# lijingzhu1/SKGHOI

Hardware: AMD Instinct MI355X
Metric: images/sec through interaction head (20x20 pairs) (higher is better)
Workload: dtype f32; 1 GPU; HICO-DET-shaped synthetic cached detections: 20 humans x 20 objects per image (G=800 grid rows, P=780 pairs, K=117 verbs), eval forward of InteractionHead from cached AdaMixer-R50 box features [40,256,7,7]/image; precision=fp32, batch_per_gpu=256, parallelism=dp1 (independent image shards, no data-path collective)

## Files before the change

include/skghoi.h:

```cpp
#ifndef SKGHOI_H
#define SKGHOI_H
#include <stdint.h>
#ifdef __cplusplus
extern "C" {
#endif

#define SKG_ABI_VERSION 19
#define SKG_E_ARG   (-1)
#define SKG_E_ALIGN (-2)
#define SKG_E_LIMIT (-3)
#define SKG_E_UNSUPPORTED (-4)
#define SKG_E_COMM  (-5)

#define SKG_MAX_DET_PER_IMAGE 1024
#define SKG_MAX_NODES         160
#define SKG_SPATIAL_LD        48
#define SKG_TRANSH_DIM        50
#define SKG_TRANSH_ENT        80

int         skg_abi_version(void);
const char* skg_build_info(void);

typedef struct {
    int32_t image;
// ... 175 lines not shown
                          const skg_image_meta* meta, int n_active, const int32_t* hum_img, const int32_t* node_img,
                          int sum_h, int sum_n, const float* T_os, const float* T_so, int64_t ldt, int cols,
                          void* U, void* V, int64_t ldu, float* adj_out, int out_dtype, void* stream);

int skg_layernorm_f32(const float* x, int64_t ldx, const float* gamma, const float* beta, int rows, int cols,
                      float eps, float* out, int64_t ldo, void* stream);
int skg_layernorm2_f32(const float* x0, int64_t ldx0, const float* gamma0, const float* beta0, int rows0, float* out0,
                       int64_t ldo0, const float* x1, int64_t ldx1, const float* gamma1, const float* beta1, int rows1,
                       float* out1, int64_t ldo1, int cols, float eps, void* stream);
int skg_layernorm2_x(const float* x0, int64_t ldx0, const float* gamma0, const float* beta0, int rows0, void* out0,
                     int64_t ldo0, const float* x1, int64_t ldx1, const float* gamma1, const float* beta1, int rows1,
                     void* out1, int64_t ldo1, int cols, float eps, int out_dtype, void* stream);

int skg_postprocess_f32(const float* logits, int64_t ld_logits, int K, const float* boxes, const float* scores,
                        const int64_t* labels, const skg_image_meta* meta, int n_active, const int64_t* x_keep,
                        const int64_t* y_keep, const int32_t* verb_off, const int32_t* verb_list, int num_obj_classes,
                        float prior_pow, int64_t L_total, const int32_t* L_total_dev, int max_pairs_per_image,
                        int64_t* out_index, int64_t* out_pred, float* out_scores, float* out_prior, float* out_weights,
                        int64_t* out_object, float* out_boxes_h, float* out_boxes_o, void* stream);

int skg_transh_draw_f32(void* torch_cpu_rng_state, int64_t state_bytes, int n_images, int K, int need_relations,
                        int fused_affine, float* ent, float* rel, float* nrm);

int skg_transh_draw_train_f32(void* torch_cpu_rng_state, int64_t state_bytes, int n_images, int K, int fused_affine,
                              const int64_t* n_neg, const int64_t* n_take, float* ent, float* rel, float* nrm,
                              int64_t* perm_out);

int skg_transh_scores_f32(const float* ent, const float* rel, const float* nrm, int K, int human_idx,
                          const skg_image_meta* meta, int n_active, float* scores, void* stream);

int skg_associate_f32(const float* boxes, const skg_image_meta* meta, int n_active, const int64_t* x_keep,
                      const int64_t* y_keep, const float* gt_h, const float* gt_o, const int64_t* gt_label,
                      const int32_t* gt_off, int K, float thresh, float* labels, int32_t* npos, void* stream);

typedef struct {
    const float* A; int64_t a_sm, a_sk;
    const float* B; int64_t b_sn, b_sk;
    int32_t b_kshift, b_nshift; int64_t b_kstride, b_nstride;
    float*  C; int64_t ldc; int32_t c_nshift, accumulate; int64_t c_nstride;
    int32_t M, N, K, relu;
    const float* bias;
    const float* mask; int64_t ldmask;
    float*  a_rowsum;
    int32_t split_k, reserved;
    float*  split_ws;
    const uint16_t* A16;
    const uint16_t* B16;
    uint16_t* C16;
    uint32_t* split_ctr;
    int64_t a16_ld, b16_ld;
} skg_gemmx_desc;
#define SKG_GEMMX_GROUP_MAX 8
int64_t skg_gemmx_ws_floats(const skg_gemmx_desc* desc_host);
int skg_gemmx_f32(const skg_gemmx_desc* descs_host, int n, void* stream);
int skg_gemmx_bf16(const skg_gemmx_desc* descs_host, int n, void* stream);
void skg_gemmx_path_counts(int64_t* out3_host, int reset);

int skg_graph_aggregate_train_f32(const float* dot_partial, int n_partial, int64_t partial_ld, float adj_bias,
                                  const skg_image_meta* meta, int n_active, const int32_t* hum_img,
                                  const int32_t* node_img, int sum_h, int sum_n, const float* T_os, const float* T_so,
                                  int64_t ldt, int cols, float* U, float* V, int64_t ldu, float* adj_out,
                                  float* alpha_out, float* beta_out, void* stream);
int skg_rowdot_f32(const float* X, int64_t ld, const float* w, int rows, int cols, float* out, void* stream);
int skg_add_layernorm_f32(const float* a, int64_t lda, const float* b, int64_t ldb, const float* gamma,
                          const float* beta, int rows, float eps, float* xsum, float* y, float* stats, void* stream);
int skg_layernorm_bwd_f32(const float* dy, int64_t lddy, const float* x, const float* stats, const float* gamma,
                          int rows, float* dx, const float* relu_src, float* dx_masked, float* dgamma, float* dbeta,
                          void* stream);
int skg_mul_bwd_f32(float* g, int64_t ldg, const float* F, const int32_t* f_idx, int64_t ldf, const float* P,
                    const int32_t* p_idx, int64_t ldp, const float* Q, const int32_t* q_idx, int64_t ldq,
                    const float* mbias, int rows, float* dF, int64_t lddf, int accumulate, void* stream);
int skg_segment_sum_f32(const float* src, int64_t ld, const skg_image_meta* meta, int n_active, const int32_t* hum_img,
                        const int32_t* node_img, int sum_h, int sum_n, int mode, float* outH, float* outN,
                        int accumulate, void* stream);
int skg_aggregate_bwd_f32(const float* dU, const float* dV, const float* Tos, const float* Tso, const float* alpha,
                          const float* beta, const int32_t* grid_h, const int32_t* grid_o, int sum_g,
                          const skg_image_meta* meta, const int32_t* hum_img, const int32_t* node_img, int sum_h,
                          int sum_n, float* dTos, float* dTso, float* da, float* db, float* dadj_h, float* dadj_n,
                          void* stream);
int skg_adjacency_bwd_f32(const float* dadj_h, const float* dadj_n, const float* w, const float* Wt, int rows,
                          float* dadj, float* dWt, void* stream);
int skg_entity_rows_bwd_f32(const float* dX, int64_t ldx, const int32_t* hum_of, const int32_t* node_of, int sum_h,
                            int n_enc, const float* enc, float* d_enc, void* stream);
#define SKG_LOSS_CHUNKS 64
int skg_hoi_loss_f32(const float* logits, int64_t ldl, int K, const skg_image_meta* meta, int n_active,
                     int64_t cells_total, const int64_t* index, const int64_t* pred, const float* scores,
                     const float* labels, float* cell_labels, float* unary, float* partial, float* dlogits,
                     void* stream);

int skg_count_positives_f32(const float* labels, int K, const float* det_scores, const int64_t* det_labels,
                            const skg_image_meta* meta, int n_active, const int64_t* x_keep, const int64_t* y_keep,
                            const int32_t* verb_off, const int32_t* verb_list, int num_obj_classes, float prior_pow,
                            float* counts, void* stream);

int skg_loss_finish_f32(const float* partial, int rows, const float* mpart, int n_img, int64_t m_pos, float margin,
                        float grad_share, const float* norm_in, float* losses, float* scale, float* counts_out,
                        void* stream);
int skg_scale_dlogits_f32(const float* dl, int64_t ld, int rows, int K, const float* scale, const float* g0,
                          const float* g1, float* out, void* stream);

int64_t skg_transh_sample_ws_ints(int n_active, int max_pos_per_image);
int skg_transh_sample_f32(const float* labels, const float* scores, int K, const skg_image_meta* meta, int n_active,
                          const int32_t* pos_off, int max_pos_per_image, const int64_t* perm, float margin, int32_t* ws,
                          int32_t* pos_cells, float* pos_scores, float* neg_scores, float* partial, void* stream);

int skg_eval_associate_f32(const float* boxes_h, const float* boxes_o, const int64_t* object, const int32_t* pair_off,
                           const int64_t* index, const int64_t* pred, const float* scores, const int32_t* cell_off,
                           int n_images, const int32_t* lut, int n_obj, int n_verb, const float* gt_h, const float* gt_o,
                           const int64_t* gt_hoi, const int32_t* gt_off, float min_iou, int32_t* hoi_out, float* labels,
                           int32_t* status, void* stream);
int skg_eval_ap11_f64(const float* labels_sorted, const int64_t* class_off, const int64_t* num_gt, int n_classes,
                      const double* thresholds11, double* ap, void* stream);

#define SKG_CHECKSUM_PARTIALS 1024
typedef struct {
    const void* ptr;
    uint32_t    count;
    uint32_t    first;
} skg_param_chunk;
int skg_param_checksum(const skg_param_chunk* chunks, int n_chunks, uint64_t* out, void* stream);

#define SKG_ADAMW_CHUNK 16384
typedef struct {
    float* p; const float* g; float* m; float* v;
    uint32_t count, reserved;
} skg_adamw_chunk;
int skg_adamw_f32(const skg_adamw_chunk* chunks, int n_chunks, double lr, double beta1, double beta2, double eps,
                  double weight_decay, double bias1, double bias2, float* steps, int n_steps, void* stream);

#define SKG_GRADNORM_PARTIALS 1024
typedef struct {
    float   total_norm;
    float   coef;
    int32_t applied;
    int32_t reserved;
    int64_t steps_applied;
    int64_t steps_skipped;
    int64_t steps_clipped;
    float   max_total_norm;
    int32_t reserved2;
    int64_t pending_skips[2];
} skg_step_status;
int skg_grad_sumsq_f32(const skg_adamw_chunk* chunks, int n_chunks, double* partials, void* stream);
int skg_adamw_guarded_f32(const skg_adamw_chunk* chunks, int n_chunks, double lr, double beta1, double beta2, double eps,
                          double weight_decay, double bias1, double bias2, int64_t t_host, double max_norm,
                          int skip_nonfinite, const double* partials, int n_partials, float* steps, int n_steps,
                          skg_step_status* status, void* stream);
int skg_sizeof_step_status(void);

enum {
    SKG_SEG_W1_0 = 0, SKG_SEG_W1_1, SKG_SEG_W1_2, SKG_SEG_W1_3, SKG_SEG_B1_0, SKG_SEG_B1_1, SKG_SEG_B1_2, SKG_SEG_B1_3,
    SKG_SEG_W3_0, SKG_SEG_W3_1, SKG_SEG_W3_2, SKG_SEG_W3_3, SKG_SEG_B3, SKG_SEG_W2, SKG_SEG_B2, SKG_SEG_CLS_W, SKG_SEG_CLS_B,
    SKG_SEG_NH_W, SKG_SEG_NH_B, SKG_SEG_NO_W, SKG_SEG_NO_B, SKG_SEG_ADJ_W, SKG_SEG_ADJ_B, SKG_SEG_SP0_W, SKG_SEG_SP0_B,
    SKG_SEG_SP2_W, SKG_SEG_SP2_B, SKG_SEG_SP4_W, SKG_SEG_SP4_B, SKG_SEG_FH_W, SKG_SEG_FH_B, SKG_SEG_FT_W, SKG_SEG_FT_B,
    SKG_SEG_BH3_W, SKG_SEG_BH3_B, SKG_SEG_BH1_W, SKG_SEG_BH1_B, SKG_TRAIN_SEGS
};
#define SKG_TRAIN_BWD_STAGES 12
typedef struct skg_train_timer skg_train_timer;
typedef struct {
    int32_t NA, Mg, Mp, Mh, Mn, A, K, Bf, Cf;
    int32_t x0_k;
    int32_t bf16;
    int32_t ld_logits;
    const float* params; float* grads;
    int64_t seg_off[SKG_TRAIN_SEGS];
    const float* x0;
// ... 80 lines not shown
```

skghoi_amd/_capi.py:

```python
import ctypes as C
import os

_HERE = os.path.dirname(os.path.abspath(__file__))
LIB_PATH = os.environ.get("SKG_LIB") or os.path.join(_HERE, "csrc", "libskghoi_hip.so")

EPI_BIAS, EPI_BIAS_RELU, EPI_MUL_RELU, EPI_RELU_DOT, EPI_BIAS_RES_RELU = range(5)
DTYPE_F32, DTYPE_F16, DTYPE_BF16 = range(3)
MAX_DET_PER_IMAGE = 1024
MAX_NODES = 160
SPATIAL_LD = 48
TRANSH_DIM = 50
TRANSH_ENT = 80
ABI_VERSION = 19
GEMM_GROUP_MAX = 4
CHECKSUM_PARTIALS = 1024
LOSS_CHUNKS = 64

_vp = C.c_void_p
_i32 = C.c_int32
_i64 = C.c_int64
_f32 = C.c_float


class GemmDesc(C.Structure):
    _fields_ = [("A", _vp), ("lda", _i64), ("W", _vp), ("ldw", _i64), ("bias", _vp), ("C", _vp), ("ldc", _i64),
                ("M", _i32), ("N", _i32), ("K", _i32), ("epilogue", _i32), ("a_rows", _vp), ("out_rows", _vp),
                ("P", _vp), ("p_idx", _vp), ("ldp", _i64), ("Q", _vp), ("q_idx", _vp), ("ldq", _i64),
                ("mbias", _vp), ("C_raw", _vp), ("ldc_raw", _i64), ("dot_w", _vp), ("dot_partial", _vp),
                ("res", _vp), ("ldres", _i64), ("split_k", _i32), ("w_scale", _f32), ("split_ws", _vp), ("w_split", _vp),
                ("a_exp", _vp)]


class GemmB16Io(C.Structure):
    _fields_ = [("w16", _vp), ("a16", _vp), ("c16", _vp), ("ldc16", _i64)]


class GemmXDesc(C.Structure):
    _fields_ = [("A", _vp), ("a_sm", _i64), ("a_sk", _i64), ("B", _vp), ("b_sn", _i64), ("b_sk", _i64),
                ("b_kshift", _i32), ("b_nshift", _i32), ("b_kstride", _i64), ("b_nstride", _i64),
                ("C", _vp), ("ldc", _i64), ("c_nshift", _i32), ("accumulate", _i32), ("c_nstride", _i64),
                ("M", _i32), ("N", _i32), ("K", _i32), ("relu", _i32), ("bias", _vp), ("mask", _vp), ("ldmask", _i64),
                ("a_rowsum", _vp), ("split_k", _i32), ("reserved", _i32), ("split_ws", _vp),
                ("A16", _vp), ("B16", _vp), ("C16", _vp), ("split_ctr", _vp),
                ("a16_ld", _i64), ("b16_ld", _i64)]


GEMMX_GROUP_MAX = 8
ADAMW_CHUNK = 16384


class GemmBf16Desc(C.Structure):
    _fields_ = [("A", _vp), ("lda", _i64), ("W", _vp), ("ldw", _i64), ("bias", _vp), ("C", _vp), ("ldc", _i64),
                ("M", _i32), ("N", _i32), ("K", _i32), ("relu", _i32), ("out_bf16", _i32), ("split_k", _i32),
                ("split_ws", _vp)]


TRAIN_SEGS = ("W1_0", "W1_1", "W1_2", "W1_3", "b1_0", "b1_1", "b1_2", "b1_3", "W3_0", "W3_1", "W3_2", "W3_3", "b3", "W2",
              "b2", "clsW", "clsb", "nh_w", "nh_b", "no_w", "no_b", "adj_w", "adj_b", "sp0_w", "sp0_b", "sp2_w", "sp2_b",
              "sp4_w", "sp4_b", "fh_w", "fh_b", "ft_w", "ft_b", "bh3_w", "bh3_b", "bh1_w", "bh1_b")
TRAIN_BWD_STAGES = 12
COMM_ID_BYTES = 128


class Exchange(C.Structure):
    _fields_ = [("comm", C.c_void_p), ("arena", C.c_void_p), ("n_chunks", C.c_int32),
                ("stage", C.c_int32 * TRAIN_BWD_STAGES), ("end", C.c_int64 * TRAIN_BWD_STAGES),
                ("adamw", C.c_void_p), ("adamw_first", C.c_int32 * (TRAIN_BWD_STAGES + 1)), ("adamw_n_steps", C.c_int32),
                ("adamw_steps", C.c_void_p)] + [(n, C.c_double) for n in ("lr", "beta1", "beta2", "eps", "weight_decay",
                                                                          "bias1", "bias2")]


GRADNORM_PARTIALS = 1024


class StepStatus(C.Structure):
    _fields_ = [("total_norm", _f32), ("coef", _f32), ("applied", _i32), ("reserved", _i32),
                ("steps_applied", _i64), ("steps_skipped", _i64), ("steps_clipped", _i64),
                ("max_total_norm", _f32), ("reserved2", _i32), ("pending_skips", _i64 * 2)]


class Tuning(C.Structure):
    _fields_ = [(n, _i32) for n in ("small_mode", "small_tiles", "route_tiles", "khalves_blocks")]


class TrainPlan(C.Structure):
    _fields_ = [(n, _i32) for n in ("NA", "Mg", "Mp", "Mh", "Mn", "A", "K", "Bf", "Cf", "x0_k", "bf16", "ld_logits")] + \
               [("params", _vp), ("grads", _vp), ("seg_off", _i64 * len(TRAIN_SEGS)),
                ("x0", _vp), ("gfeat", _vp), ("sp48", _vp), ("ent", _vp), ("meta", _vp)] + \
               [(n, _vp) for n in ("enc_row_hn", "img_hn", "ent_row_hn", "hum_img", "node_img", "grid_h", "grid_o",
                                   "grid_pair", "grid_img", "pair_grid", "pair_h", "pair_o", "pair_img", "hum_of",
                                   "node_of")] + \
               [("ws", _vp), ("ws_floats", _i64), ("pair_features", _vp), ("logits", _vp), ("dlogits", _vp),
                ("dx0", _vp), ("dgfeat", _vp), ("timer", _vp), ("ws16", _vp), ("params16", _vp), ("pf16", _vp),
                ("params_floats", _i64), ("counters", _vp), ("n_counters", _i64), ("split_target", _i32), ("split_max", _i32),
                ("two_branch", _i32), ("reserved2", _i32)]


LAYOUT_SLICES = ("meta", "node_img", "hum_img", "node_enc_row", "hum_enc_row", "node_ent_row", "hum_ent_row", "enc_row_hn",
                 "img_hn", "ent_row_hn", "hum_of", "node_of", "pair_img", "gt_off", "active")


class LayoutInfo(C.Structure):
    _fields_ = [(n, _i32) for n in ("B", "n_visit", "n_active", "index_error")] + \
               [(n, _i64) for n in ("sum_all", "sum_n", "sum_h", "sum_g", "sum_p", "sum_l", "ints")] + \
               [("off", _i32 * len(LAYOUT_SLICES)), ("len", _i32 * len(LAYOUT_SLICES))]


META_FIELDS = [("image", "i4"), ("n_h", "i4"), ("n", "i4"), ("box_off", "i4"), ("enc_off", "i4"), ("node_off", "i4"),
               ("hum_off", "i4"), ("grid_off", "i4"), ("pair_off", "i4"), ("out_off", "i4"), ("img_h", "f4"),
               ("img_w", "f4")]

PROTOTYPES = {
    "skg_abi_version": (C.c_int, []),
    "skg_build_info": (C.c_char_p, []),
    "skg_preprocess_f32": (C.c_int, [_vp, _vp, _vp, _vp, C.c_int, C.c_int, _f32, _f32, C.c_int, C.c_int, _vp, C.c_int,
                                     _f32, _vp, _vp, _vp]),
    "skg_pack_detections_f32": (C.c_int, [_vp, _vp, _vp, _vp, _vp, C.c_int, _vp, C.c_int, _vp, _vp, _vp, _vp]),
    "skg_pairs_spatial_f32": (C.c_int, [_vp, _vp, C.c_int, _vp, _vp, _vp, _vp, _vp, _vp, _vp, _vp, _vp, _vp, C.c_int,
                                        _vp]),
    "skg_pairs_spatial_padded_f32": (C.c_int, [_vp, _vp, C.c_int, _vp, _vp, _vp, _vp, _vp, _vp, _vp, _vp, _vp, _vp,
                                               C.c_int, C.c_int, C.c_int, _vp]),
    "skg_roi_align_f32": (C.c_int, [_vp, _vp, _vp, _vp, C.c_int, C.c_int, C.c_int, C.c_int, _f32, C.c_int, _vp, _vp,
                                    C.c_int, C.c_int, C.c_int, _vp, _vp]),
    "skg_roi_align_bwd_f32": (C.c_int, [_vp, _vp, _vp, _vp, C.c_int, C.c_int, C.c_int, C.c_int, _f32, C.c_int, _vp, _vp,
                                    C.c_int, C.c_int, C.c_int, _vp, _vp]),
    "skg_roi_align_x": (C.c_int, [_vp, C.c_int, _vp, _vp, _vp, C.c_int, C.c_int, C.c_int, C.c_int, _f32, C.c_int, _vp,
                                  _vp, C.c_int, C.c_int, C.c_int, _vp, C.c_int, _vp]),
    "skg_roi_align_nhwc_x": (C.c_int, [_vp, C.c_int, _vp, _vp, _vp, C.c_int, C.c_int, C.c_int, C.c_int, _f32, C.c_int,
                                       _vp, _vp, C.c_int, C.c_int, C.c_int, _vp, C.c_int, _vp]),
    "skg_roi_align_bwd_nhwc_f32": (C.c_int, [_vp, _vp, _vp, _vp, C.c_int, C.c_int, C.c_int, C.c_int, _f32, C.c_int, _vp,
                                             _vp, C.c_int, C.c_int, C.c_int, _vp, _vp]),
    "skg_roi_align_layout_counts": (None, [C.POINTER(_i64), C.c_int]),
    "skg_roi_align_bwd_det_x": (C.c_int, [_vp, C.c_int, _vp, _vp, _vp, C.c_int, C.c_int, C.c_int, C.c_int, _f32, C.c_int,
                                          _vp, _vp, C.c_int, C.c_int, C.c_int, C.c_int, _vp, _vp]),
    "skg_roi_align_bwd_det_nhwc_x": (C.c_int, [_vp, C.c_int, _vp, _vp, _vp, C.c_int, C.c_int, C.c_int, C.c_int, _f32,
                                               C.c_int, _vp, _vp, C.c_int, C.c_int, C.c_int, C.c_int, _vp, _vp]),
    "skg_roi_align_det_counts": (None, [C.POINTER(_i64), C.c_int]),
    "skg_global_avgpool_f32": (C.c_int, [_vp, C.c_int, C.c_int, C.c_int, _vp, _vp]),
    "skg_gemm_f32": (C.c_int, [C.POINTER(GemmDesc), _vp]),
    "skg_transh_draw_f32": (C.c_int, [_vp, _i64, C.c_int, C.c_int, C.c_int, C.c_int, _vp, _vp, _vp]),
    "skg_transh_draw_train_f32": (C.c_int, [_vp, _i64, C.c_int, C.c_int, C.c_int, _vp, _vp, _vp, _vp, _vp, _vp]),
    "skg_gemm_dot_partials": (C.c_int, [C.POINTER(GemmDesc)]),
    "skg_split_weights_bytes": (C.c_int64, [C.c_int, C.c_int]),
    "skg_split_weights_f16x2": (C.c_int, [_vp, C.c_int, C.c_int, _i64, _f32, _vp, _vp]),
    "skg_gemm_group_f32": (C.c_int, [C.POINTER(GemmDesc), C.c_int, _vp]),
    "skg_gemm_group_tile": (C.c_int, [C.POINTER(GemmDesc), C.c_int]),
    "skg_gemm_b16_f32": (C.c_int, [C.POINTER(GemmDesc), _vp, _vp]),
    "skg_gemm_group_b16_f32": (C.c_int, [C.POINTER(GemmDesc), C.POINTER(_vp), C.c_int, _vp]),
    "skg_gemm_path_counts": (None, [C.POINTER(_i64), C.c_int]),
    "skg_gemm_b16_a16_f32": (C.c_int, [C.POINTER(GemmDesc), _vp, _vp, _vp]),
    "skg_gemm_b16_a16_launches": (None, [C.POINTER(_i64), C.c_int]),
    "skg_gemm_b16_x": (C.c_int, [C.POINTER(GemmDesc), C.POINTER(GemmB16Io), _vp]),
    "skg_gemm_group_b16_x": (C.c_int, [C.POINTER(GemmDesc), C.POINTER(GemmB16Io), C.c_int, _vp]),
    "skg_gemm_b16_x_counts": (None, [C.POINTER(_i64), C.c_int]),
    "skg_row_exponents_f32": (C.c_int, [_vp, C.c_int64, _vp, C.c_int, C.c_int, _vp, _vp]),
    "skg_adamw_f32": (C.c_int, [_vp, C.c_int] + [C.c_double] * 7 + [_vp, C.c_int, _vp]),
    "skg_grad_sumsq_f32": (C.c_int, [_vp, C.c_int, _vp, _vp]),
    "skg_adamw_guarded_f32": (C.c_int, [_vp, C.c_int] + [C.c_double] * 7 + [_i64, C.c_double, C.c_int, _vp, C.c_int, _vp,
                                                                          C.c_int, _vp, _vp]),
    "skg_sizeof_step_status": (C.c_int, []),
    "skg_ctx_set_tuning": (C.c_int, [_vp, C.POINTER(Tuning)]),
    "skg_ctx_get_tuning": (C.c_int, [_vp, C.POINTER(Tuning)]),
    "skg_ctx_make_current": (_vp, [_vp]),
    "skg_gemmx_ws_floats": (C.c_int64, [C.POINTER(GemmXDesc)]),
    "skg_gemmx_f32": (C.c_int, [C.POINTER(GemmXDesc), C.c_int, _vp]),
    "skg_gemmx_bf16": (C.c_int, [C.POINTER(GemmXDesc), C.c_int, _vp]),
    "skg_gemmx_path_counts": (None, [C.POINTER(_i64), C.c_int]),
    "skg_gemm_bf16": (C.c_int, [C.POINTER(GemmBf16Desc), _vp]),
    "skg_transpose_bf16": (C.c_int, [_vp, _i64, C.c_int, C.c_int, _vp, _i64, _vp]),
    "skg_transpose_f32": (C.c_int, [_vp, _i64, C.c_int, C.c_int, _vp, _i64, _vp]),
    "skg_concat_entity_f32": (C.c_int, [_vp, _i64, _vp, _vp, _vp, _vp, C.c_int, _vp, _i64, _vp]),
    "skg_concat_entity_x": (C.c_int, [_vp, _i64, _vp, _vp, _vp, _vp, C.c_int, _vp, _i64, C.c_int, _vp]),
    "skg_rows_mul_relu_x": (C.c_int, [_vp, _vp, _i64, _vp, _vp, _i64, _vp, _vp, _vp, _i64, C.c_int, C.c_int, _vp,
                                      _i64, C.c_int, _vp]),
    "skg_graph_aggregate_x": (C.c_int, [_vp, C.c_int, _i64, _f32, _vp, C.c_int, _vp, _vp, C.c_int, C.c_int, _vp,
                                        _vp, _i64, C.c_int, _vp, _vp, _i64, _vp, C.c_int, _vp]),
    "skg_layernorm2_x": (C.c_int, [_vp, _i64, _vp, _vp, C.c_int, _vp, _i64, _vp, _i64, _vp, _vp, C.c_int, _vp, _i64,
                                   C.c_int, _f32, C.c_int, _vp]),
    "skg_rows_mul_relu_f32": (C.c_int, [_vp, _vp, _i64, _vp, _vp, _i64, _vp, _vp, _vp, _i64, C.c_int, C.c_int, _vp,
                                        _i64, _vp]),
    "skg_graph_aggregate_f32": (C.c_int, [_vp, C.c_int, _i64, _f32, _vp, C.c_int, _vp, _vp, C.c_int, C.c_int, _vp,
                                          _vp, _i64, C.c_int, _vp, _vp, _i64, _vp, _vp]),
    "skg_layernorm_f32": (C.c_int, [_vp, _i64, _vp, _vp, C.c_int, C.c_int, _f32, _vp, _i64, _vp]),
    "skg_layernorm2_f32": (C.c_int, [_vp, _i64, _vp, _vp, C.c_int, _vp, _i64, _vp, _i64, _vp, _vp, C.c_int, _vp, _i64,
                                     C.c_int, _f32, _vp]),
    "skg_postprocess_f32": (C.c_int, [_vp, _i64, C.c_int, _vp, _vp, _vp, _vp, C.c_int, _vp, _vp, _vp, _vp, C.c_int,
                                      _f32, _i64, _vp, C.c_int, _vp, _vp, _vp, _vp, _vp, _vp, _vp, _vp, _vp]),
    "skg_associate_f32": (C.c_int, [_vp, _vp, C.c_int, _vp, _vp, _vp, _vp, _vp, _vp, C.c_int, _f32, _vp, _vp, _vp]),
    "skg_transh_scores_f32": (C.c_int, [_vp, _vp, _vp, C.c_int, C.c_int, _vp, C.c_int, _vp, _vp]),
    "skg_param_checksum": (C.c_int, [_vp, C.c_int, _vp, _vp]),
    "skg_graph_aggregate_train_f32": (C.c_int, [_vp, C.c_int, _i64, _f32, _vp, C.c_int, _vp, _vp, C.c_int, C.c_int, _vp,
                                                _vp, _i64, C.c_int, _vp, _vp, _i64, _vp, _vp, _vp, _vp]),
    "skg_rowdot_f32": (C.c_int, [_vp, _i64, _vp, C.c_int, C.c_int, _vp, _vp]),
    "skg_add_layernorm_f32": (C.c_int, [_vp, _i64, _vp, _i64, _vp, _vp, C.c_int, _f32, _vp, _vp, _vp, _vp]),
    "skg_layernorm_bwd_f32": (C.c_int, [_vp, _i64, _vp, _vp, _vp, C.c_int, _vp, _vp, _vp, _vp, _vp, _vp]),
    "skg_mul_bwd_f32": (C.c_int, [_vp, _i64, _vp, _vp, _i64, _vp, _vp, _i64, _vp, _vp, _i64, _vp, C.c_int, _vp, _i64,
                                  C.c_int, _vp]),
    "skg_segment_sum_f32": (C.c_int, [_vp, _i64, _vp, C.c_int, _vp, _vp, C.c_int, C.c_int, C.c_int, _vp, _vp, C.c_int,
                                      _vp]),
    "skg_aggregate_bwd_f32": (C.c_int, [_vp, _vp, _vp, _vp, _vp, _vp, _vp, _vp, C.c_int, _vp, _vp, _vp, C.c_int, C.c_int,
                                        _vp, _vp, _vp, _vp, _vp, _vp, _vp]),
    "skg_adjacency_bwd_f32": (C.c_int, [_vp, _vp, _vp, _vp, C.c_int, _vp, _vp, _vp]),
    "skg_entity_rows_bwd_f32": (C.c_int, [_vp, _i64, _vp, _vp, C.c_int, C.c_int, _vp, _vp, _vp]),
    "skg_eval_associate_f32": (C.c_int, [_vp, _vp, _vp, _vp, _vp, _vp, _vp, _vp, C.c_int, _vp, C.c_int, C.c_int, _vp, _vp,
                                         _vp, _vp, _f32, _vp, _vp, _vp, _vp]),
    "skg_eval_ap11_f64": (C.c_int, [_vp, _vp, _vp, C.c_int, _vp, _vp, _vp]),
    "skg_transh_sample_ws_ints": (C.c_int64, [C.c_int, C.c_int]),
    "skg_transh_sample_f32": (C.c_int, [_vp, _vp, C.c_int, _vp, C.c_int, _vp, C.c_int, _vp, _f32, _vp, _vp, _vp, _vp, _vp,
                                        _vp]),
    "skg_hoi_loss_f32": (C.c_int, [_vp, _i64, C.c_int, _vp, C.c_int, _i64, _vp, _vp, _vp, _vp, _vp, _vp, _vp, _vp, _vp]),
    "skg_count_positives_f32": (C.c_int, [_vp, C.c_int, _vp, _vp, _vp, C.c_int, _vp, _vp, _vp, _vp, C.c_int, _f32, _vp, _vp]),
    "skg_loss_finish_f32": (C.c_int, [_vp, C.c_int, _vp, C.c_int, _i64, _f32, _f32, _vp, _vp, _vp, _vp, _vp]),
    "skg_scale_dlogits_f32": (C.c_int, [_vp, _i64, C.c_int, C.c_int, _vp, _vp, _vp, _vp, _vp]),
    "skg_train_ws_floats": (C.c_int64, [C.POINTER(TrainPlan)]),
    "skg_train_forward_f32": (C.c_int, [C.POINTER(TrainPlan), C.c_int, _vp]),
    "skg_train_backward_f32": (C.c_int, [C.POINTER(TrainPlan), C.c_int, C.c_int, _vp]),
    "skg_train_backward_async_f32": (C.c_int, [C.POINTER(TrainPlan), C.c_int, C.c_int, _vp]),
    "skg_train_backward_join": (C.c_int, []),
    "skg_twin_bf16": (C.c_int, [_vp, _vp, _i64, _vp]),
    "skg_layout_pack_train": (C.c_int, [_vp, _vp, _vp, C.c_int, _vp, C.c_int, C.c_int, C.c_int, _vp, _vp, _i64,
                                        C.POINTER(LayoutInfo)]),
    "skg_train_timer_create": (_vp, [C.c_int]),
    "skg_train_timer_destroy": (None, [_vp]),
    "skg_train_timer_read": (C.c_int, [_vp, C.POINTER(C.c_double)]),
    "skg_context_create": (_vp, []),
    "skg_context_destroy": (None, [_vp]),
    "skg_ctx_train_backward_async_f32": (C.c_int, [_vp, C.POINTER(TrainPlan), C.c_int, C.c_int, _vp, _vp, C.c_uint32]),
    "skg_ctx_train_forward_f32": (C.c_int, [_vp, C.POINTER(TrainPlan), C.c_int, _vp]),
    "skg_ctx_train_backward_exchange_f32": (C.c_int, [_vp, C.POINTER(TrainPlan), C.c_int, C.c_int, _vp, _vp, C.POINTER(Exchange)]),
    "skg_sizeof_exchange": (C.c_int, []),
    "skg_comm_load": (C.c_int, [C.c_char_p]),
    "skg_comm_unique_id": (C.c_int, [_vp]),
    "skg_comm_create": (C.c_int, [_vp, C.c_int, C.c_int, C.POINTER(_vp)]),
    "skg_comm_destroy": (None, [_vp]),
    "skg_comm_abort": (C.c_int, [_vp]),
    "skg_comm_dead": (C.c_int, [_vp]),
    "skg_comm_world": (C.c_int, [_vp]),
    "skg_comm_rank": (C.c_int, [_vp]),
    "skg_comm_collectives": (_i64, [_vp]),
    "skg_comm_last_error": (C.c_char_p, []),
    "skg_comm_all_reduce_chunks_f32": (C.c_int, [_vp, _vp, C.POINTER(_i64), C.c_int, _vp]),
    "skg_comm_all_reduce_begin_f32": (C.c_int, [_vp, _vp, _i64, _vp]),
    "skg_comm_all_reduce_end": (C.c_int, [_vp, _vp]),
    "skg_comm_exposed_ms": (C.c_int, [_vp, _vp, C.POINTER(C.c_float)]),
    "skg_ctx_stream_wait_stage": (C.c_int, [_vp, C.c_int, _vp]),
    "skg_ctx_train_backward_stage_wait": (C.c_int, [_vp, C.c_int]),
    "skg_ctx_train_backward_join": (C.c_int, [_vp]),
    "skg_ctx_train_backward_progress": (C.c_int, [_vp]),
    "skg_train_ws_offset": (C.c_int64, [C.POINTER(TrainPlan), C.c_int]),
    "skg_train_flops": (C.c_double, [C.POINTER(TrainPlan), C.c_int]),
}

_LIB = None


class SkgError(RuntimeError):
    pass


def lib():
    global _LIB
    if _LIB is not None:
        return _LIB
    if not os.path.isfile(LIB_PATH):
        raise SkgError("libskghoi_hip.so not built at %s -- run `python __graft_entry__.py` or "
                       "`make -C skghoi_amd/csrc` (there is no CPU fallback)" % LIB_PATH)
    l = C.CDLL(LIB_PATH)
    for name, (res, args) in PROTOTYPES.items():
        fn = getattr(l, name)
        fn.restype = res
        fn.argtypes = args
    if l.skg_abi_version() == ABI_VERSION and l.skg_sizeof_exchange() != C.sizeof(Exchange):
        raise SkgError("skg_exchange is %d bytes in libskghoi_hip.so, %d in the binding" % (l.skg_sizeof_exchange(), C.sizeof(Exchange)))
    if l.skg_abi_version() == ABI_VERSION and l.skg_sizeof_step_status() != C.sizeof(StepStatus):
        raise SkgError("skg_step_status is %d bytes in libskghoi_hip.so, %d in the binding" % (l.skg_sizeof_step_status(), C.sizeof(StepStatus)))
    if l.skg_abi_version() != ABI_VERSION:
        raise SkgError("libskghoi_hip.so ABI %d != binding ABI %d" % (l.skg_abi_version(), ABI_VERSION))
    _LIB = l
    env = {k: int(os.environ[e]) for k, e in (("small_mode", "SKG_SMALL_MODE"), ("small_tiles", "SKG_SMALL_TILES"),
                                              ("route_tiles", "SKG_ROUTE_TILES"), ("khalves_blocks", "SKG_KHALVES_BLOCKS"))
           if os.environ.get(e)}
    if env:
        set_tuning(**env)
    return l


# ... 34 lines not shown
```

skghoi_amd/csrc/skg_common.h:

```cpp
#pragma once
#include <hip/hip_runtime.h>
#include <stdint.h>
#include "skghoi.h"

#define SKG_WAVE 64

typedef float f32x16 __attribute__((ext_vector_type(16)));
typedef float f32x4 __attribute__((ext_vector_type(4)));

static inline int skg_launch_status() {
    hipError_t e = hipGetLastError();
    return e == hipSuccess ? 0 : (int)e;
}

static inline bool skg_aligned16(const void* p) { return (((uintptr_t)p) & 15u) == 0; }
__device__ __forceinline__ bool skg_aligned16_dev(const void* p) { return (((uintptr_t)p) & 15u) == 0; }

__device__ __forceinline__ float skg_wave_sum(float v) {
#pragma unroll
    for (int off = 32; off > 0; off >>= 1) v += __shfl_xor(v, off, 64);
    return v;
}
__device__ __forceinline__ float skg_wave_max(float v) {
#pragma unroll
    for (int off = 32; off > 0; off >>= 1) v = fmaxf(v, __shfl_xor(v, off, 64));
    return v;
}

__device__ __forceinline__ float skg_block_sum256(float v, float* red) {
    v = skg_wave_sum(v);
    const int w = threadIdx.x >> 6;
    __syncthreads();
    if ((threadIdx.x & 63) == 0) red[w] = v;
    __syncthreads();
    return (red[0] + red[1]) + (red[2] + red[3]);
}

extern thread_local const skg_tuning* skg_tls_tuning;
static inline int skg_tune_small_mode() { const skg_tuning* t = skg_tls_tuning; return t && t->small_mode > 0 ? t->small_mode : 3; }
static inline int skg_tune_small_tiles() { const skg_tuning* t = skg_tls_tuning; return t && t->small_tiles > 0 ? t->small_tiles : 384; }
static inline int skg_tune_route_tiles() { const skg_tuning* t = skg_tls_tuning; return t && t->route_tiles > 0 ? t->route_tiles : 200; }
static inline int skg_tune_khalves_blocks() { const skg_tuning* t = skg_tls_tuning; return t && t->khalves_blocks > 0 ? t->khalves_blocks : 320; }

struct skg_twin_map { const float* base[2]; uint16_t* base16[2]; int64_t n[2]; };
extern thread_local skg_twin_map skg_tls_twin;
static inline uint16_t* skg_twin(const float* p) {
    const skg_twin_map& m = skg_tls_twin;
    for (int i = 0; i < 2; ++i)
        if (m.base16[i] && p >= m.base[i] && p < m.base[i] + m.n[i]) return m.base16[i] + (p - m.base[i]);
    return nullptr;
}
typedef __bf16 skg_bf2 __attribute__((ext_vector_type(2)));
typedef float skg_f2 __attribute__((ext_vector_type(2)));
__device__ __forceinline__ uint32_t skg_pack_bf16(float a, float b) {
    const skg_f2 v = {a, b};
    return __builtin_bit_cast(uint32_t, __builtin_convertvector(v, skg_bf2));
}
__device__ __forceinline__ void skg_store_twin4(uint16_t* p, const float4 v) {
    *reinterpret_cast<uint2*>(p) = make_uint2(skg_pack_bf16(v.x, v.y), skg_pack_bf16(v.z, v.w));
}

struct skg_gemmx_fused {
    int kind;
    const float* P; const int32_t* p_idx; int64_t ldp;
    const float* Q; const int32_t* q_idx; int64_t ldq;
    const float* mbias;
    float* C_raw; int64_t ldc_raw;
    const int32_t* out_rows;
    const float* res; int64_t ldres;
};
int skg_gemmx_can_fuse(const skg_gemmx_desc* d, const skg_gemmx_fused* f);
int skg_gemmx_f32_fused(const skg_gemmx_desc* descs_host, const skg_gemmx_fused* fused_host, int n, void* stream);

#define SKG_MULTI_MAX 4
struct skg_rows_mul_args {
    const float* P; const int32_t* p_idx; int64_t ldp; const float* Q; const int32_t* q_idx; int64_t ldq; const float* mbias;
    const float* F; const int32_t* f_idx; int64_t ldf; int rows, cols; float* out; int64_t ldo;
    uint16_t* out16;
};
int skg_rows_mul_relu_multi(const skg_rows_mul_args* calls, int n, void* stream);
struct skg_mul_bwd_args {
    float* g; int64_t ldg; const float* F; const int32_t* f_idx; int64_t ldf; const float* P; const int32_t* p_idx; int64_t ldp;
    const float* Q; const int32_t* q_idx; int64_t ldq; const float* mbias; int rows; float* dF; int64_t lddf; int accumulate;
    uint16_t* dF16;
};
int skg_mul_bwd_multi(const skg_mul_bwd_args* calls, int n, void* stream);
struct skg_segment_sum_args {
    const float* src; int64_t ld; int mode; float* outH; float* outN; int accumulate;
    uint16_t* outH16; uint16_t* outN16;
};
int skg_segment_sum_multi(const skg_segment_sum_args* calls, int n, const skg_image_meta* meta, const int32_t* hum_img,
                          const int32_t* node_img, int sum_h, int sum_n, void* stream);
struct skg_add_layernorm_args {
    const float* a; int64_t lda; const float* b; int64_t ldb; const float* gamma; const float* beta; int rows;
    float* xsum; float* y; float* stats;
    uint16_t* y16;
};
int skg_add_layernorm_multi(const skg_add_layernorm_args* calls, int n, float eps, void* stream);
struct skg_layernorm_bwd_args {
    const float* dy; int64_t lddy; const float* x; const float* stats; const float* gamma; int rows; float* dx;
    const float* relu_src; float* dx_masked; float* dgamma; float* dbeta;
    uint16_t* dx16; uint16_t* dx_masked16;
};
int skg_layernorm_bwd_multi(const skg_layernorm_bwd_args* calls, int n, void* stream);

int skg_comm_chunk(skg_comm* c, hipEvent_t after, float* p, int64_t n);
int skg_comm_close_step(skg_comm* c, hipStream_t stream);
int skg_comm_chunk_in_stream(skg_comm* c, hipStream_t stream, float* p, int64_t n);
hipStream_t skg_comm_stream(skg_comm* c);
int skg_adamw_slice(const skg_adamw_chunk* chunks, int first, int last, const skg_exchange& x, bool with_steps, hipStream_t stream);
```

skghoi_amd/csrc/skg_gemm_x.hip:

```cpp
#include "skg_common.h"
#include <stdlib.h>
#include <string.h>
#include <type_traits>
#include <atomic>

#define XBM 128
#define XBN 128
#define XBK 16
#define XLD 130
#define XTILE (XBK * XLD)
#ifndef SKG_XXCD
#define SKG_XXCD 1
#endif

struct skg_gemmx_group {
    skg_gemmx_desc d[SKG_GEMMX_GROUP_MAX];
    int start[SKG_GEMMX_GROUP_MAX + 1];
    skg_gemmx_fused f[SKG_GEMMX_GROUP_MAX];
    int vec[SKG_GEMMX_GROUP_MAX];
    int n;
};

__device__ __forceinline__ int64_t xoff(int idx, int shift, int64_t bstride, int64_t estride) {
    if (shift <= 0) return (int64_t)idx * estride;
// ... 49 lines not shown
    return t;
}

template <bool KC>
__device__ __forceinline__ float4 xgen(const XOperand& op, int row, int k, int kend) {
    if (row >= op.rows || k >= kend) return xzero4();
    if (KC)
        return xquad(op.base + xoff(row, op.rshift, op.rstride, op.s_row) + xoff(k, op.kshift, op.kstride, 1), k, kend,
                     op.vec);
    return xquad(op.base + xoff(k, op.kshift, op.kstride, op.s_k) + xoff(row, op.rshift, op.rstride, 1), row, op.rows,
                 op.vec);
}

template <bool KC>
__device__ __forceinline__ bool xfast_ok(const XOperand& op, int row0) {
    return op.vec && (KC || (op.rows & 3) == 0 || row0 + 128 <= op.rows);
}

struct XTileId { int tm, tn, slice; };
__device__ __forceinline__ XTileId xtile_of(int b, int nb, int nbm, int nbn, int S, int K) {
#if SKG_XXCD
    {
        const int q = nb >> 3, r = nb & 7, x = b & 7;
        b = (x < r ? x * (q + 1) : r * (q + 1) + (x - r) * q) + (b >> 3);
    }
    int g = (int)((2 << 20) / ((int64_t)XBN * 4 * max(K, 1)));
    g = max(1, min(g, nbn));
    const int per_group = nbm * g * S;
    const int grp = min(b / per_group, (nbn - 1) / g);
    const int w = min(g, nbn - grp * g);
    const int rr = b - grp * per_group;
    XTileId t;
    t.slice = rr % S;
    t.tn = grp * g + (rr / S) % w;
    t.tm = rr / (S * w);
    return t;
#else
    XTileId t;
    t.slice = b % S; b /= S;
    t.tn = b % nbn; t.tm = b / nbn;
    return t;
#endif
}

typedef __bf16 xbf2 __attribute__((ext_vector_type(2)));
typedef float xf2 __attribute__((ext_vector_type(2)));
__device__ __forceinline__ uint32_t ypack(float a, float b) {
    const xf2 v = {a, b};
    return __builtin_bit_cast(uint32_t, __builtin_convertvector(v, xbf2));
}

#define XEP_LD 72
#define XEP_WAVE (32 * XEP_LD)
#define XEP_FLOATS (4 * XEP_WAVE)

struct XRed { const float* ws; int64_t MN; int S, slice; };
typedef unsigned int xu4s __attribute__((__vector_size__(16)));
#define XSC1 16
__device__ __forceinline__ __amdgpu_buffer_rsrc_t xrsrc(const float* p) {
    return __builtin_amdgcn_make_buffer_rsrc(const_cast<float*>(p), 0, 0x7fffffff, 0x00020000);
}
__device__ __forceinline__ void xst_sc1(__amdgpu_buffer_rsrc_t r, uint32_t byte_off, const float4& v) {
    const xu4s u = {__float_as_uint(v.x), __float_as_uint(v.y), __float_as_uint(v.z), __float_as_uint(v.w)};
    __builtin_amdgcn_raw_buffer_store_b128(u, r, (int)byte_off, 0, XSC1);
}
__device__ __forceinline__ float4 xld_sc1(__amdgpu_buffer_rsrc_t r, uint32_t byte_off) {
    const xu4s u = __builtin_amdgcn_raw_buffer_load_b128(r, (int)byte_off, 0, XSC1);
    return make_float4(__uint_as_float(u[0]), __uint_as_float(u[1]), __uint_as_float(u[2]), __uint_as_float(u[3]));
}

__device__ __forceinline__ bool xsplit_last(uint32_t* ctr, int S, volatile uint32_t* flag) {
    asm volatile("s_waitcnt vmcnt(0)" ::: "memory");
    __syncthreads();
    if (threadIdx.x == 0) *flag = atomicInc(ctr, (uint32_t)(S - 1)) == (uint32_t)(S - 1) ? 1u : 0u;
    __syncthreads();
    return *flag != 0u;
}

__device__ __forceinline__ void xep_apply(const skg_gemmx_desc& d, const skg_gemmx_fused& f, float4 v, int row, int col,
                                          int64_t coff, bool hb, const float4& bv, const float4& mb) {
    if (hb) { v.x += bv.x; v.y += bv.y; v.z += bv.z; v.w += bv.w; }
    if (f.kind | (f.out_rows != nullptr)) {
        const int orow = f.out_rows ? f.out_rows[row] : row;
        if (f.kind == SKG_EPI_MUL_RELU) {
            if (f.C_raw) *reinterpret_cast<float4*>(f.C_raw + (int64_t)row * f.ldc_raw + col) = v;
            if (orow < 0) return;
            float4 m = mb;
            if (f.P) {
                const float4 t = xld4(f.P + (int64_t)(f.p_idx ? f.p_idx[row] : row) * f.ldp + col);
                m.x += t.x; m.y += t.y; m.z += t.z; m.w += t.w;
            }
            if (f.Q) {
                const float4 t = xld4(f.Q + (int64_t)(f.q_idx ? f.q_idx[row] : row) * f.ldq + col);
                m.x += t.x; m.y += t.y; m.z += t.z; m.w += t.w;
            }
            *reinterpret_cast<float4*>(d.C + coff + (int64_t)orow * d.ldc) =
                make_float4(fmaxf(v.x * m.x, 0.f), fmaxf(v.y * m.y, 0.f), fmaxf(v.z * m.z, 0.f), fmaxf(v.w * m.w, 0.f));
            return;
        }
        if (orow < 0) return;
        if (d.relu || f.kind == SKG_EPI_BIAS_RES_RELU) {
            v.x = fmaxf(v.x, 0.f); v.y = fmaxf(v.y, 0.f); v.z = fmaxf(v.z, 0.f); v.w = fmaxf(v.w, 0.f);
        }
        if (f.kind == SKG_EPI_BIAS_RES_RELU) {
            const float4 t = xld4(f.res + (int64_t)row * f.ldres + col);
            v.x += t.x; v.y += t.y; v.z += t.z; v.w += t.w;
        }
        *reinterpret_cast<float4*>(d.C + coff + (int64_t)orow * d.ldc) = v;
        return;
    }
    if (d.relu) { v.x = fmaxf(v.x, 0.f); v.y = fmaxf(v.y, 0.f); v.z = fmaxf(v.z, 0.f); v.w = fmaxf(v.w, 0.f); }
    float* p = d.C + coff + (int64_t)row * d.ldc;
    if (d.accumulate) { const float4 o = xld4(p); v.x += o.x; v.y += o.y; v.z += o.z; v.w += o.w; }
    if (d.mask) {
        const float4 m = xld4(d.mask + (int64_t)row * d.ldmask + col);
        v.x = m.x > 0.f ? v.x : 0.f; v.y = m.y > 0.f ? v.y : 0.f; v.z = m.z > 0.f ? v.z : 0.f; v.w = m.w > 0.f ? v.w : 0.f;
    }
    *reinterpret_cast<float4*>(p) = v;
    if (d.C16)
        *reinterpret_cast<uint2*>(d.C16 + coff + (int64_t)row * d.ldc) = make_uint2(ypack(v.x, v.y), ypack(v.z, v.w));
}

template <bool WT = false>
__device__ __forceinline__ void xep_rows(const skg_gemmx_desc& d, const skg_gemmx_fused& f, const float* stage, int lane,
                                         int row0, int col0, float* ws) {
    const int c4 = 4 * (lane & 15), rr = lane >> 4, col = col0 + c4;
    if (col >= d.N) return;
    const bool hb = !ws && d.bias;
    float4 bv = xzero4(), mb = xzero4();
    if (hb) bv = xld4(d.bias + col);
    if (f.kind == SKG_EPI_MUL_RELU && f.mbias) mb = xld4(f.mbias + col);
    const int64_t coff = xoff(col, d.c_nshift, d.c_nstride, 1);
#pragma unroll
    for (int i = 0; i < 8; ++i) {
        const int row = row0 + 4 * i + rr;
        if (row >= d.M) continue;
        const float4 v = *reinterpret_cast<const float4*>(stage + (4 * i + rr) * XEP_LD + c4);
        if (WT) { xst_sc1(xrsrc(ws), ((uint32_t)row * (uint32_t)d.N + (uint32_t)col) * 4u, v); continue; }
        if (ws) { *reinterpret_cast<float4*>(ws + (int64_t)row * d.N + col) = v; continue; }
        xep_apply(d, f, v, row, col, coff, hb, bv, mb);
    }
}

template <bool OWN, int R>
__device__ __forceinline__ void xep_reduce(const skg_gemmx_desc& d, const skg_gemmx_fused& f, const float* stage, int lane,
                                           int row0, int col0, const XRed& red) {
    static_assert(R == 4 || R == 8, "rows per lane and pass");
    const int c4 = 4 * (lane & 15), rr = lane >> 4, col = col0 + c4;
    if (col >= d.N) return;
    const bool hb = d.bias != nullptr;
    float4 bv = xzero4(), mb = xzero4();
    if (hb) bv = xld4(d.bias + col);
    if (f.kind == SKG_EPI_MUL_RELU && f.mbias) mb = xld4(f.mbias + col);
    const int64_t coff = xoff(col, d.c_nshift, d.c_nstride, 1);
#pragma unroll 1
    for (int h = 0; h < 8 / R; ++h) {
        uint32_t ro[R];
        float4 sum[R];
#pragma unroll
        for (int i = 0; i < R; ++i) {
            ro[i] = ((uint32_t)min(row0 + 4 * (R * h + i) + rr, d.M - 1) * (uint32_t)d.N + (uint32_t)col) * 4u;
            sum[i] = xzero4();
        }
        auto add_slices = [&](int s0, int s1) {
            int s = s0;
            for (; s + 1 < s1; s += 2) {
                const __amdgpu_buffer_rsrc_t w0 = xrsrc(red.ws + (int64_t)s * red.MN);
                const __amdgpu_buffer_rsrc_t w1 = xrsrc(red.ws + (int64_t)(s + 1) * red.MN);
                float4 q0[R], q1[R];
#pragma unroll
                for (int i = 0; i < R; ++i) { q0[i] = xld_sc1(w0, ro[i]); q1[i] = xld_sc1(w1, ro[i]); }
#pragma unroll
                for (int i = 0; i < R; ++i) {
                    sum[i].x += q0[i].x; sum[i].y += q0[i].y; sum[i].z += q0[i].z; sum[i].w += q0[i].w;
                    sum[i].x += q1[i].x; sum[i].y += q1[i].y; sum[i].z += q1[i].z; sum[i].w += q1[i].w;
                }
            }
            if (s < s1) {
                const __amdgpu_buffer_rsrc_t w0 = xrsrc(red.ws + (int64_t)s * red.MN);
                float4 q0[R];
#pragma unroll
                for (int i = 0; i < R; ++i) q0[i] = xld_sc1(w0, ro[i]);
#pragma unroll
                for (int i = 0; i < R; ++i) { sum[i].x += q0[i].x; sum[i].y += q0[i].y; sum[i].z += q0[i].z; sum[i].w += q0[i].w; }
            }
        };
        if (OWN) {
            add_slices(0, red.slice);
#pragma unroll
            for (int i = 0; i < R; ++i) {
                const float4 q = *reinterpret_cast<const float4*>(stage + (4 * (R * h + i) + rr) * XEP_LD + c4);
                sum[i].x += q.x; sum[i].y += q.y; sum[i].z += q.z; sum[i].w += q.w;
            }
            add_slices(red.slice + 1, red.S);
        } else {
            add_slices(0, red.S);
        }
#pragma unroll
        for (int i = 0; i < R; ++i) {
            const int row = row0 + 4 * (R * h + i) + rr;
            if (row < d.M) xep_apply(d, f, sum[i], row, col, coff, hb, bv, mb);
        }
    }
}

__device__ __forceinline__ void xreduce_elem(const skg_gemmx_desc& d, int64_t MN, int row, int col) {
    const int64_t i = (int64_t)row * d.N + col;
    float v = 0.f;
    for (int s = 0; s < d.split_k; ++s) v += d.split_ws[(int64_t)s * MN + i];
    if (d.bias) v += d.bias[col];
    if (d.relu) v = fmaxf(v, 0.f);
    float* p = d.C + xoff(col, d.c_nshift, d.c_nstride, 1) + (int64_t)row * d.ldc;
    if (d.accumulate) v += *p;
    if (d.mask && !(d.mask[(int64_t)row * d.ldmask + col] > 0.f)) v = 0.f;
    *p = v;
    if (d.C16) d.C16[p - d.C] = (uint16_t)ypack(v, 0.f);
}
__device__ __forceinline__ void xreduce_rowsum(const skg_gemmx_desc& d, int64_t MN, int row) {
    float v = 0.f;
    for (int s = 0; s < d.split_k; ++s) v += d.split_ws[(int64_t)d.split_k * MN + (int64_t)s * d.M + row];
    d.a_rowsum[row] = d.accumulate ? d.a_rowsum[row] + v : v;
}
__device__ __forceinline__ void xreduce_rowsum_sc1(const skg_gemmx_desc& d, int64_t MN, int row) {
    float v = 0.f;
    for (int s = 0; s < d.split_k; ++s)
        v += __hip_atomic_load(d.split_ws + (int64_t)d.split_k * MN + (int64_t)s * d.M + row, __ATOMIC_RELAXED,
                               __HIP_MEMORY_SCOPE_AGENT);
    d.a_rowsum[row] = d.accumulate ? d.a_rowsum[row] + v : v;
}
__device__ __forceinline__ void xstore_rowsum_part(float* p, float v, bool wt) {
    if (wt) __hip_atomic_store(p, v, __ATOMIC_RELAXED, __HIP_MEMORY_SCOPE_AGENT);
    else *p = v;
}

template <bool KC>
__device__ __forceinline__ void xprep(const XOperand& op, int row0, int tid, XFast& F) {
// ... 1082 lines not shown
    const int64_t w = (int64_t)(blockIdx.x - g.start[gi]) * 256 + threadIdx.x;
    const bool quads = g.vec[gi] & 8;
    const int64_t nmat = quads ? MN / 4 : MN;
    if (w >= nmat) {
        const int64_t m = w - nmat;
        if (m >= d.M || !d.a_rowsum) return;
        xreduce_rowsum(d, MN, (int)m);
        return;
    }
    if (quads) {
        const int64_t i = 4 * w;
        float4 v = xzero4();
        for (int s = 0; s < d.split_k; ++s) {
            const float4 q = xld4(d.split_ws + (int64_t)s * MN + i);
            v.x += q.x; v.y += q.y; v.z += q.z; v.w += q.w;
        }
        const int row = (int)(i / d.N), col = (int)(i % d.N);
        if (d.bias) { const float4 bv = xld4(d.bias + col); v.x += bv.x; v.y += bv.y; v.z += bv.z; v.w += bv.w; }
        if (d.relu) { v.x = fmaxf(v.x, 0.f); v.y = fmaxf(v.y, 0.f); v.z = fmaxf(v.z, 0.f); v.w = fmaxf(v.w, 0.f); }
        float* p = d.C + xoff(col, d.c_nshift, d.c_nstride, 1) + (int64_t)row * d.ldc;
        if (d.accumulate) { const float4 o = xld4(p); v.x += o.x; v.y += o.y; v.z += o.z; v.w += o.w; }
        if (d.mask) {
            const float4 m = xld4(d.mask + (int64_t)row * d.ldmask + col);
            v.x = m.x > 0.f ? v.x : 0.f; v.y = m.y > 0.f ? v.y : 0.f; v.z = m.z > 0.f ? v.z : 0.f; v.w = m.w > 0.f ? v.w : 0.f;
        }
        *reinterpret_cast<float4*>(p) = v;
        if (d.C16) *reinterpret_cast<uint2*>(d.C16 + (p - d.C)) = make_uint2(ypack(v.x, v.y), ypack(v.z, v.w));
        return;
    }
    xreduce_elem(d, MN, (int)(w / d.N), (int)(w % d.N));
}

static int skg_gemmx_validate(const skg_gemmx_desc& d) {
    if (d.M < 0 || d.N < 0 || d.K < 0) return SKG_E_ARG;
    if (d.M == 0 || d.N == 0) return 0;
    if (!d.C || d.ldc < 1) return SKG_E_ARG;
    if (d.K > 0 && (!d.A || !d.B)) return SKG_E_ARG;
    if (d.a_sm != 1 && d.a_sk != 1) return SKG_E_ARG;
    if (d.b_sn != 1 && d.b_sk != 1) return SKG_E_ARG;
    if (d.b_kshift < 0 || d.b_kshift > 30 || d.b_nshift < 0 || d.b_nshift > 30 || d.c_nshift < 0 || d.c_nshift > 30)
        return SKG_E_ARG;
    if ((d.b_kshift == 1) || (d.b_nshift == 1)) return SKG_E_ARG;
    if (d.mask && d.ldmask < d.N) return SKG_E_ARG;
    if (d.split_k > 1 && (!d.split_ws || d.split_k > 256)) return SKG_E_ARG;
    if ((((uintptr_t)d.C16) & 1u) || (((uintptr_t)d.A16) & 1u) || (((uintptr_t)d.B16) & 1u)) return SKG_E_ALIGN;
    if (((uintptr_t)d.split_ctr) & 3u) return SKG_E_ALIGN;
    if (d.a16_ld < 0 || d.b16_ld < 0 || (d.b16_ld && (d.b_kshift || d.b_nshift))) return SKG_E_ARG;
    if (d.a16_ld && d.a16_ld < (d.a_sk == 1 ? d.K : d.M)) return SKG_E_ARG;
    if (d.b16_ld && d.b16_ld < (d.b_sk == 1 ? d.K : d.N)) return SKG_E_ARG;
    return 0;
}

static bool xmul4(int64_t v) { return (v & 3) == 0; }
static bool xmul8(int64_t v) { return (v & 7) == 0; }

static int64_t xspan(int64_t idx, int shift, int64_t bstride, int64_t estride) {
    if (idx <= 0) return 0;
    if (shift <= 0) return idx * estride;
    return (idx >> shift) * bstride + (idx & ((1LL << shift) - 1)) * estride;
}
static bool xfits32(int64_t elems) { return elems >= 0 && elems < (1LL << 29); }

extern "C" int64_t skg_gemmx_ws_floats(const skg_gemmx_desc* d) {
    if (!d) return SKG_E_ARG;
    return d->split_k > 1 ? (int64_t)d->split_k * ((int64_t)d->M * d->N + d->M) : 0;
}

static bool xfused_ptrs_ok(const skg_gemmx_fused& f) {
    return skg_aligned16(f.P) && skg_aligned16(f.Q) && skg_aligned16(f.mbias) && skg_aligned16(f.C_raw) &&
           skg_aligned16(f.res) && xmul4(f.ldp) && xmul4(f.ldq) && xmul4(f.ldc_raw) && xmul4(f.ldres);
}

static std::atomic<long long> g_path_launches[3];
extern "C" void skg_gemmx_path_counts(int64_t* out3_host, int reset) {
    for (int i = 0; i < 3; ++i) {
        if (out3_host) out3_host[i] = g_path_launches[i].load(std::memory_order_relaxed);
        if (reset) g_path_launches[i].store(0, std::memory_order_relaxed);
    }
}

static bool g_t16_enabled = getenv("SKG_GEMMX_T16") == nullptr || atoi(getenv("SKG_GEMMX_T16")) != 0;

static int skg_gemmx_launch(const skg_gemmx_desc* descs_host, int n, void* stream, bool bf16,
                            const skg_gemmx_fused* fused_host = nullptr) {
    if (!descs_host || n < 1 || n > SKG_GEMMX_GROUP_MAX) return SKG_E_ARG;
    skg_gemmx_group g, r;
    memset(g.f, 0, sizeof(g.f)); memset(r.f, 0, sizeof(r.f));
    g.n = r.n = 0;
    int64_t blocks = 0, rblocks = 0;
    for (int i = 0; i < n; ++i) {
        const skg_gemmx_desc& d = descs_host[i];
        const int rc = skg_gemmx_validate(d);
        if (rc) return rc;
        if (d.M == 0 || d.N == 0) continue;
        const int S = d.split_k > 1 ? d.split_k : 1;
        const int64_t nb = (int64_t)((d.M + XBM - 1) / XBM) * ((d.N + XBN - 1) / XBN) * S;
        if (blocks + nb > 0x7fffffffLL) return SKG_E_LIMIT;
        int vec = 0;
        if (skg_aligned16(d.A) && (d.a_sk == 1 ? xmul4(d.a_sm) : xmul4(d.a_sk)) &&
            xfits32((int64_t)(d.M - 1) * d.a_sm + (int64_t)(d.K - 1) * d.a_sk + 4))
            vec |= 1;
        if (skg_aligned16(d.B) && (d.b_sk == 1 ? xmul4(d.b_sn) : xmul4(d.b_sk)) &&
            (d.b_kshift == 0 || (xmul4(d.b_kstride) && d.b_kshift >= 5)) && (d.b_nshift == 0 || xmul4(d.b_nstride)) &&
            xfits32(xspan(d.N - 1, d.b_nshift, d.b_nstride, d.b_sn) + xspan(d.K - 1, d.b_kshift, d.b_kstride, d.b_sk) + 4))
            vec |= 2;
        if ((((uintptr_t)d.C) & 7u) == 0 && (d.ldc & 1) == 0 && (d.c_nshift == 0 || (d.c_nstride & 1) == 0)) vec |= 4;
        if ((d.N & 3) == 0 && skg_aligned16(d.C) && xmul4(d.ldc) &&
            (d.c_nshift == 0 || (d.c_nshift >= 2 && xmul4(d.c_nstride))) && skg_aligned16(d.bias) &&
            skg_aligned16(d.mask) && (!d.mask || xmul4(d.ldmask)) && (S == 1 || skg_aligned16(d.split_ws)) &&
            (((uintptr_t)d.C16) & 7u) == 0)
            vec |= 8;
        const int64_t lda16 = d.a16_ld ? d.a16_ld : (d.a_sk == 1 ? d.a_sm : d.a_sk);
        const int64_t ldb16 = d.b16_ld ? d.b16_ld : (d.b_sk == 1 ? d.b_sn : d.b_sk);
        if (bf16 && d.A16 && ((vec & 1) || d.a16_ld) && skg_aligned16(d.A16) && xmul8(lda16) &&
            xfits32((int64_t)(d.a_sk == 1 ? d.M : d.K) * lda16 + 8))
            vec |= 16;
        if (bf16 && d.B16 && ((vec & 2) || d.b16_ld) && skg_aligned16(d.B16) && xmul8(ldb16) &&
            (d.b_kshift == 0 || xmul8(d.b_kstride)) && (d.b_nshift == 0 || (d.b_nshift >= 3 && xmul8(d.b_nstride))) &&
            (!d.b16_ld || xfits32((int64_t)(d.b_sk == 1 ? d.N : d.K) * ldb16 + 8)))
            vec |= 32;
        if (fused_host && (fused_host[i].kind || fused_host[i].out_rows)) {
            if (!(vec & 8) || (S > 1 && !(d.split_ctr && (int64_t)d.M * d.N < (1LL << 29))) || d.c_nshift || d.accumulate || d.mask || d.C16 ||
                !xfused_ptrs_ok(fused_host[i]))
                return SKG_E_ARG;
            g.f[g.n] = fused_host[i];
        }
        g.d[g.n] = d; g.vec[g.n] = vec; g.start[g.n] = (int)blocks;
        const bool inlaunch = S > 1 && d.split_ctr && (vec & 8) && (int64_t)d.M * d.N < (1LL << 29);
        if (!inlaunch) g.d[g.n].split_ctr = nullptr;
        ++g.n;
        blocks += nb;
        if (S > 1 && !inlaunch) {
            const int64_t MN = (int64_t)d.M * d.N;
            const int64_t total = ((vec & 8) ? MN / 4 : MN) + (d.a_rowsum ? d.M : 0);
            const int64_t nr = (total + 255) / 256;
            if (rblocks + nr > 0x7fffffffLL) return SKG_E_LIMIT;
            r.d[r.n] = d; r.vec[r.n] = vec; r.start[r.n] = (int)rblocks; ++r.n;
            rblocks += nr;
        }
    }
    if (g.n == 0) return 0;
    for (int i = g.n; i <= SKG_GEMMX_GROUP_MAX; ++i) g.start[i] = (int)blocks;
    bool t16 = bf16 && g_t16_enabled;
    for (int i = 0; i < g.n && t16; ++i) {
        const skg_gemmx_desc& d = g.d[i];
        const int64_t lda16 = d.a16_ld ? d.a16_ld : d.a_sk, ldb16 = d.b16_ld ? d.b16_ld : d.b_sk;
        t16 = (g.vec[i] & 48) == 48 && d.K > 0 && (d.a_sk == 1 || (d.M & 7) == 0 || lda16 >= ((d.M + 7) & ~7)) &&
              (d.b_sk == 1 || (d.b_nshift == 0 ? ((d.N & 7) == 0 || ldb16 >= ((d.N + 7) & ~7)) : (d.N & 7) == 0)) &&
              (d.b_kshift == 0 || d.b_kshift >= 6);
    }
    if (!t16)
        for (int i = 0; i < g.n; ++i) {
            if (g.d[i].a16_ld) g.vec[i] &= ~16;
            if (g.d[i].b16_ld) g.vec[i] &= ~32;
        }
    g_path_launches[t16 ? 2 : (bf16 ? 1 : 0)].fetch_add(1, std::memory_order_relaxed);
    if (t16) hipLaunchKernelGGL(skg_gemmx_t16_kernel, dim3((unsigned)blocks), dim3(256), 0, (hipStream_t)stream, g);
    else if (bf16) hipLaunchKernelGGL(skg_gemmx_bf16_kernel, dim3((unsigned)blocks), dim3(256), 0, (hipStream_t)stream, g);
    else hipLaunchKernelGGL(skg_gemmx_kernel, dim3((unsigned)blocks), dim3(256), 0, (hipStream_t)stream, g);
    if (r.n) {
        for (int i = r.n; i <= SKG_GEMMX_GROUP_MAX; ++i) r.start[i] = (int)rblocks;
        hipLaunchKernelGGL(skg_gemmx_reduce_kernel, dim3((unsigned)rblocks), dim3(256), 0, (hipStream_t)stream, r);
    }
    return skg_launch_status();
}

extern "C" int skg_gemmx_f32(const skg_gemmx_desc* descs_host, int n, void* stream) {
    return skg_gemmx_launch(descs_host, n, stream, false);
}

int skg_gemmx_f32_fused(const skg_gemmx_desc* descs_host, const skg_gemmx_fused* fused_host, int n, void* stream) {
    return skg_gemmx_launch(descs_host, n, stream, false, fused_host);
}

int skg_gemmx_can_fuse(const skg_gemmx_desc* dp, const skg_gemmx_fused* f) {
    const skg_gemmx_desc& d = *dp;
    if (skg_gemmx_validate(d)) return 0;
    const bool staged = (d.N & 3) == 0 && skg_aligned16(d.C) && xmul4(d.ldc) && d.c_nshift == 0 && skg_aligned16(d.bias);
    if (!f || !(f->kind || f->out_rows)) return 1;
    return staged && (d.split_k <= 1 || d.split_ctr) && !d.accumulate && !d.mask && xfused_ptrs_ok(*f);
}

extern "C" int skg_gemmx_bf16(const skg_gemmx_desc* descs_host, int n, void* stream) {
    return skg_gemmx_launch(descs_host, n, stream, true);
}
```

skghoi_amd/csrc/skg_graph.hip:

```cpp
#include "skg_common.h"

__global__ __launch_bounds__(256) void skg_graph_aggregate_kernel(
    const float* __restrict__ dot_partial, int n_partial, int64_t partial_ld, float adj_bias,
    const skg_image_meta* __restrict__ meta, const int32_t* __restrict__ hum_img, const int32_t* __restrict__ node_img,
    int sum_h, const float* __restrict__ T_os, const float* __restrict__ T_so, int64_t ldt, int cols,
    float* __restrict__ U, float* __restrict__ V, int64_t ldu, float* __restrict__ adj_out,
    float* __restrict__ alpha_out, float* __restrict__ beta_out, uint16_t* __restrict__ U16, uint16_t* __restrict__ V16) {
    __shared__ float sw[SKG_MAX_NODES];
    __shared__ float sred[4];
    const int tid = threadIdx.x;
    const bool to_human = (int)blockIdx.x < sum_h;
    const int dst = to_human ? blockIdx.x : blockIdx.x - sum_h;
    const int a = to_human ? hum_img[dst] : node_img[dst];
    const skg_image_meta mt = meta[a];
    const int local = to_human ? dst - mt.hum_off : dst - mt.node_off;
    if (local >= (to_human ? mt.n_h : mt.n)) return;
    const int cnt = to_human ? mt.n : mt.n_h;
    const int64_t row0 = to_human ? (int64_t)mt.grid_off + (int64_t)local * mt.n : (int64_t)mt.grid_off + local;
    const int64_t rstep = to_human ? 1 : mt.n;

    for (int t = tid; t < cnt; t += 256) {
        const int64_t gr = row0 + t * rstep;
        float s = 0.f;
        for (int k = 0; k < n_partial; ++k) s += dot_partial[(int64_t)k * partial_ld + gr];
        s += adj_bias;
        sw[t] = s;
        if (to_human && adj_out) adj_out[gr] = s;
    }
    __syncthreads();
    float mx = -INFINITY;
    for (int t = tid; t < cnt; t += 256) mx = fmaxf(mx, sw[t]);
    mx = skg_wave_max(mx);
    if ((tid & 63) == 0) sred[tid >> 6] = mx;
    __syncthreads();
    mx = fmaxf(fmaxf(sred[0], sred[1]), fmaxf(sred[2], sred[3]));
    float se = 0.f;
    for (int t = tid; t < cnt; t += 256) {
        const float e = expf(sw[t] - mx);
        sw[t] = e;
        se += e;
    }
    se = skg_block_sum256(se, sred);
    const float inv = 1.f / se;
    float* wout = to_human ? alpha_out : beta_out;
    if (wout)
        for (int t = tid; t < cnt; t += 256) wout[row0 + t * rstep] = sw[t] * inv;

    const float* T = to_human ? T_os : T_so;
    float* out = to_human ? U : V;
    if (out) out += (int64_t)dst * ldu;
    uint16_t* out16 = to_human ? U16 : V16;
    if (out16) out16 += (int64_t)dst * ldu;
    for (int c = tid * 4; c < cols; c += 1024) {
        float4 acc = make_float4(0.f, 0.f, 0.f, 0.f);
        const float* p = T + row0 * ldt + c;
        for (int t = 0; t < cnt; ++t) {
            const float wt = sw[t] * inv;
            const float4 v = *reinterpret_cast<const float4*>(p + (int64_t)t * rstep * ldt);
            acc.x += wt * v.x; acc.y += wt * v.y; acc.z += wt * v.z; acc.w += wt * v.w;
        }
        if (out) *reinterpret_cast<float4*>(out + c) = acc;
        if (out16) skg_store_twin4(out16 + c, acc);
    }
}

extern "C" int skg_graph_aggregate_x(const float* dot_partial, int n_partial, int64_t partial_ld, float adj_bias,
                                     const skg_image_meta* meta, int n_active, const int32_t* hum_img,
                                     const int32_t* node_img, int sum_h, int sum_n, const float* T_os, const float* T_so,
                                     int64_t ldt, int cols, void* U, void* V, int64_t ldu, float* adj_out, int out_dtype,
                                     void* stream) {
    if (n_active < 0 || sum_h < 0 || sum_n < 0 || n_partial <= 0 || cols <= 0 || (cols & 3)) return SKG_E_ARG;
    if (out_dtype != SKG_DTYPE_F32 && out_dtype != SKG_DTYPE_BF16) return SKG_E_ARG;
    if (sum_h + sum_n == 0) return 0;
    if (!dot_partial || !meta || !hum_img || !node_img || !T_os || !T_so || !U || !V) return SKG_E_ARG;
    const bool half = out_dtype == SKG_DTYPE_BF16;
    const uintptr_t amask = half ? 7u : 15u;
    if ((ldt & 3) || (ldu & 3) || !skg_aligned16(T_os) || !skg_aligned16(T_so) || (((uintptr_t)U) & amask) ||
        (((uintptr_t)V) & amask))
        return SKG_E_ALIGN;
    hipLaunchKernelGGL(skg_graph_aggregate_kernel, dim3(sum_h + sum_n), dim3(256), 0, (hipStream_t)stream, dot_partial,
                       n_partial, partial_ld, adj_bias, meta, hum_img, node_img, sum_h, T_os, T_so, ldt, cols,
                       half ? (float*)nullptr : (float*)U, half ? (float*)nullptr : (float*)V, ldu, adj_out,
                       (float*)nullptr, (float*)nullptr, half ? (uint16_t*)U : (uint16_t*)nullptr,
                       half ? (uint16_t*)V : (uint16_t*)nullptr);
    return skg_launch_status();
}

extern "C" int skg_graph_aggregate_f32(const float* dot_partial, int n_partial, int64_t partial_ld, float adj_bias,
                                       const skg_image_meta* meta, int n_active, const int32_t* hum_img,
                                       const int32_t* node_img, int sum_h, int sum_n, const float* T_os,
                                       const float* T_so, int64_t ldt, int cols, float* U, float* V, int64_t ldu,
                                       float* adj_out, void* stream) {
    return skg_graph_aggregate_x(dot_partial, n_partial, partial_ld, adj_bias, meta, n_active, hum_img, node_img, sum_h,
                                 sum_n, T_os, T_so, ldt, cols, U, V, ldu, adj_out, SKG_DTYPE_F32, stream);
}

extern "C" int skg_graph_aggregate_train_f32(const float* dot_partial, int n_partial, int64_t partial_ld, float adj_bias,
                                             const skg_image_meta* meta, int n_active, const int32_t* hum_img,
                                             const int32_t* node_img, int sum_h, int sum_n, const float* T_os,
                                             const float* T_so, int64_t ldt, int cols, float* U, float* V, int64_t ldu,
                                             float* adj_out, float* alpha_out, float* beta_out, void* stream) {
    if (n_active < 0 || sum_h < 0 || sum_n < 0 || n_partial <= 0 || cols <= 0 || (cols & 3)) return SKG_E_ARG;
    if (sum_h + sum_n == 0) return 0;
    if (!dot_partial || !meta || !hum_img || !node_img || !T_os || !T_so || !U || !V || !alpha_out || !beta_out)
        return SKG_E_ARG;
    if ((ldt & 3) || (ldu & 3) || !skg_aligned16(T_os) || !skg_aligned16(T_so) || !skg_aligned16(U) ||
        !skg_aligned16(V))
        return SKG_E_ALIGN;
    hipLaunchKernelGGL(skg_graph_aggregate_kernel, dim3(sum_h + sum_n), dim3(256), 0, (hipStream_t)stream, dot_partial,
                       n_partial, partial_ld, adj_bias, meta, hum_img, node_img, sum_h, T_os, T_so, ldt, cols, U, V,
                       ldu, adj_out, alpha_out, beta_out, skg_twin(U), skg_twin(V));
    return skg_launch_status();
}

__global__ __launch_bounds__(256) void skg_layernorm_kernel(const float* __restrict__ x, int64_t ldx,
                                                            const float* __restrict__ gamma,
                                                            const float* __restrict__ beta, int cols, float eps,
                                                            float* __restrict__ out, int64_t ldo) {
    __shared__ float sred[4];
    const int r = blockIdx.x;
    const int c = threadIdx.x * 4;
    const bool in = c < cols;
    float4 v = make_float4(0.f, 0.f, 0.f, 0.f);
    if (in) v = *reinterpret_cast<const float4*>(x + (int64_t)r * ldx + c);
    const float mean = skg_block_sum256((v.x + v.y) + (v.z + v.w), sred) / (float)cols;
    float4 dlt = make_float4(v.x - mean, v.y - mean, v.z - mean, v.w - mean);
    float sq = in ? (dlt.x * dlt.x + dlt.y * dlt.y) + (dlt.z * dlt.z + dlt.w * dlt.w) : 0.f;
    const float var = skg_block_sum256(sq, sred) / (float)cols;
    const float rstd = 1.f / sqrtf(var + eps);
    if (in) {
        const float4 g = *reinterpret_cast<const float4*>(gamma + c);
        const float4 bb = *reinterpret_cast<const float4*>(beta + c);
        *reinterpret_cast<float4*>(out + (int64_t)r * ldo + c) =
            make_float4(dlt.x * rstd * g.x + bb.x, dlt.y * rstd * g.y + bb.y, dlt.z * rstd * g.z + bb.z,
                        dlt.w * rstd * g.w + bb.w);
    }
}

struct skg_ln_seg { const float* x; int64_t ldx; const float* gamma; const float* beta; float* out; int64_t ldo; int rows; uint16_t* out16; };

__global__ __launch_bounds__(256) void skg_layernorm2_kernel(const skg_ln_seg a, const skg_ln_seg b, int cols, float eps) {
    __shared__ float sred[4];
    const bool first = (int)blockIdx.x < a.rows;
    const skg_ln_seg& g = first ? a : b;
    const int r = first ? (int)blockIdx.x : (int)blockIdx.x - a.rows;
    const int c = threadIdx.x * 4;
    const bool in = c < cols;
    float4 v = make_float4(0.f, 0.f, 0.f, 0.f);
    if (in) v = *reinterpret_cast<const float4*>(g.x + (int64_t)r * g.ldx + c);
    const float mean = skg_block_sum256((v.x + v.y) + (v.z + v.w), sred) / (float)cols;
    float4 dlt = make_float4(v.x - mean, v.y - mean, v.z - mean, v.w - mean);
    float sq = in ? (dlt.x * dlt.x + dlt.y * dlt.y) + (dlt.z * dlt.z + dlt.w * dlt.w) : 0.f;
    const float var = skg_block_sum256(sq, sred) / (float)cols;
    const float rstd = 1.f / sqrtf(var + eps);
    if (in) {
        const float4 gm = *reinterpret_cast<const float4*>(g.gamma + c);
        const float4 bb = *reinterpret_cast<const float4*>(g.beta + c);
        const float4 y = make_float4(dlt.x * rstd * gm.x + bb.x, dlt.y * rstd * gm.y + bb.y, dlt.z * rstd * gm.z + bb.z,
                                     dlt.w * rstd * gm.w + bb.w);
        if (g.out16) skg_store_twin4(g.out16 + (int64_t)r * g.ldo + c, y);
        else *reinterpret_cast<float4*>(g.out + (int64_t)r * g.ldo + c) = y;
    }
}

extern "C" int skg_layernorm2_x(const float* x0, int64_t ldx0, const float* gamma0, const float* beta0, int rows0,
                                void* out0, int64_t ldo0, const float* x1, int64_t ldx1, const float* gamma1,
                                const float* beta1, int rows1, void* out1, int64_t ldo1, int cols, float eps,
                                int out_dtype, void* stream) {
    if (rows0 < 0 || rows1 < 0 || cols <= 0 || cols > 1024 || (cols & 3)) return SKG_E_ARG;
    if (out_dtype != SKG_DTYPE_F32 && out_dtype != SKG_DTYPE_BF16) return SKG_E_ARG;
    if (rows0 + rows1 == 0) return 0;
    if ((rows0 && (!x0 || !gamma0 || !beta0 || !out0)) || (rows1 && (!x1 || !gamma1 || !beta1 || !out1))) return SKG_E_ARG;
    const bool half = out_dtype == SKG_DTYPE_BF16;
    const uintptr_t amask = half ? 7u : 15u;
    if ((ldx0 & 3) || (ldo0 & 3) || (ldx1 & 3) || (ldo1 & 3)) return SKG_E_ALIGN;
    if (rows0 && (!skg_aligned16(x0) || (((uintptr_t)out0) & amask) || !skg_aligned16(gamma0) || !skg_aligned16(beta0))) return SKG_E_ALIGN;
    if (rows1 && (!skg_aligned16(x1) || (((uintptr_t)out1) & amask) || !skg_aligned16(gamma1) || !skg_aligned16(beta1))) return SKG_E_ALIGN;
    const skg_ln_seg a{x0, ldx0, gamma0, beta0, half ? nullptr : (float*)out0, ldo0, rows0, half ? (uint16_t*)out0 : nullptr},
                     b{x1, ldx1, gamma1, beta1, half ? nullptr : (float*)out1, ldo1, rows1, half ? (uint16_t*)out1 : nullptr};
    hipLaunchKernelGGL(skg_layernorm2_kernel, dim3(rows0 + rows1), dim3(256), 0, (hipStream_t)stream, a, b, cols, eps);
    return skg_launch_status();
}

extern "C" int skg_layernorm2_f32(const float* x0, int64_t ldx0, const float* gamma0, const float* beta0, int rows0,
                                  float* out0, int64_t ldo0, const float* x1, int64_t ldx1, const float* gamma1,
                                  const float* beta1, int rows1, float* out1, int64_t ldo1, int cols, float eps,
                                  void* stream) {
    return skg_layernorm2_x(x0, ldx0, gamma0, beta0, rows0, out0, ldo0, x1, ldx1, gamma1, beta1, rows1, out1, ldo1, cols,
                            eps, SKG_DTYPE_F32, stream);
}

extern "C" int skg_layernorm_f32(const float* x, int64_t ldx, const float* gamma, const float* beta, int rows,
                                 int cols, float eps, float* out, int64_t ldo, void* stream) {
    if (rows < 0 || cols <= 0 || cols > 1024 || (cols & 3)) return SKG_E_ARG;
// ... 10 lines not shown
```

skghoi_amd/csrc/skg_train.hip:

```cpp
#include "skg_common.h"

#define TR_COLS 1024

__global__ __launch_bounds__(256) void skg_rowdot_kernel(const float* __restrict__ X, int64_t ld,
                                                         const float* __restrict__ w, int rows, int cols,
                                                         float* __restrict__ out) {
    const int r = blockIdx.x * 4 + (threadIdx.x >> 6);
    if (r >= rows) return;
    const int lane = threadIdx.x & 63;
    const float* x = X + (int64_t)r * ld;
    float s = 0.f;
    for (int c = lane * 4; c < cols; c += 256) {
        const float4 a = *reinterpret_cast<const float4*>(x + c);
        const float4 b = *reinterpret_cast<const float4*>(w + c);
        s += (a.x * b.x + a.y * b.y) + (a.z * b.z + a.w * b.w);
    }
    s = skg_wave_sum(s);
    if (lane == 0) out[r] = s;
}

extern "C" int skg_rowdot_f32(const float* X, int64_t ld, const float* w, int rows, int cols, float* out, void* stream) {
    if (rows < 0 || cols <= 0 || (cols & 3)) return SKG_E_ARG;
    if (rows == 0) return 0;
    if (!X || !w || !out) return SKG_E_ARG;
    if ((ld & 3) || !skg_aligned16(X) || !skg_aligned16(w)) return SKG_E_ALIGN;
    hipLaunchKernelGGL(skg_rowdot_kernel, dim3((rows + 3) / 4), dim3(256), 0, (hipStream_t)stream, X, ld, w, rows, cols, out);
    return skg_launch_status();
}

__device__ __forceinline__ void skg_add_layernorm_row(const float* __restrict__ a, int64_t lda,
                                                      const float* __restrict__ b, int64_t ldb,
                                                      const float* __restrict__ gamma, const float* __restrict__ beta,
                                                      float eps, float* __restrict__ xsum, float* __restrict__ y,
                                                      float* __restrict__ stats, int r, uint16_t* __restrict__ y16) {
    __shared__ float sred[4];
    const int c = threadIdx.x * 4;
    const float4 va = *reinterpret_cast<const float4*>(a + (int64_t)r * lda + c);
    const float4 vb = *reinterpret_cast<const float4*>(b + (int64_t)r * ldb + c);
    const float4 v = make_float4(va.x + vb.x, va.y + vb.y, va.z + vb.z, va.w + vb.w);
    const float mean = skg_block_sum256((v.x + v.y) + (v.z + v.w), sred) / (float)TR_COLS;
    const float4 d = make_float4(v.x - mean, v.y - mean, v.z - mean, v.w - mean);
    const float var = skg_block_sum256((d.x * d.x + d.y * d.y) + (d.z * d.z + d.w * d.w), sred) / (float)TR_COLS;
    const float rstd = 1.f / sqrtf(var + eps);
    const float4 g = *reinterpret_cast<const float4*>(gamma + c);
    const float4 bb = *reinterpret_cast<const float4*>(beta + c);
    *reinterpret_cast<float4*>(xsum + (int64_t)r * TR_COLS + c) = v;
    const float4 yo = make_float4(d.x * rstd * g.x + bb.x, d.y * rstd * g.y + bb.y, d.z * rstd * g.z + bb.z, d.w * rstd * g.w + bb.w);
    *reinterpret_cast<float4*>(y + (int64_t)r * TR_COLS + c) = yo;
    if (y16) skg_store_twin4(y16 + (int64_t)r * TR_COLS + c, yo);
    if (threadIdx.x == 0) { stats[2 * r] = mean; stats[2 * r + 1] = rstd; }
}

__global__ __launch_bounds__(256) void skg_add_layernorm_kernel(const float* __restrict__ a, int64_t lda,
                                                                const float* __restrict__ b, int64_t ldb,
                                                                const float* __restrict__ gamma,
                                                                const float* __restrict__ beta, float eps,
                                                                float* __restrict__ xsum, float* __restrict__ y,
                                                                float* __restrict__ stats, uint16_t* __restrict__ y16) {
    skg_add_layernorm_row(a, lda, b, ldb, gamma, beta, eps, xsum, y, stats, (int)blockIdx.x, y16);
}

struct skg_add_layernorm_pack { skg_add_layernorm_args a[SKG_MULTI_MAX]; };
__global__ __launch_bounds__(256) void skg_add_layernorm_multi_kernel(const skg_add_layernorm_pack pk, float eps) {
    const skg_add_layernorm_args& a = pk.a[blockIdx.y];
    if ((int)blockIdx.x >= a.rows) return;
    skg_add_layernorm_row(a.a, a.lda, a.b, a.ldb, a.gamma, a.beta, eps, a.xsum, a.y, a.stats, (int)blockIdx.x, a.y16);
}

int skg_add_layernorm_multi(const skg_add_layernorm_args* calls, int n, float eps, void* stream) {
    if (!calls || n < 1 || n > SKG_MULTI_MAX) return SKG_E_ARG;
    skg_add_layernorm_pack pk;
    int m = 0, rows = 0;
    for (int i = 0; i < n; ++i) {
        const skg_add_layernorm_args& a = calls[i];
        if (a.rows < 0) return SKG_E_ARG;
        if (a.rows == 0) continue;
        if (!a.a || !a.b || !a.gamma || !a.beta || !a.xsum || !a.y || !a.stats) return SKG_E_ARG;
        if ((a.lda & 3) || (a.ldb & 3) || !skg_aligned16(a.a) || !skg_aligned16(a.b) || !skg_aligned16(a.gamma) ||
            !skg_aligned16(a.beta) || !skg_aligned16(a.xsum) || !skg_aligned16(a.y))
            return SKG_E_ALIGN;
        pk.a[m] = a;
        pk.a[m++].y16 = skg_twin(a.y);
        rows = a.rows > rows ? a.rows : rows;
    }
    if (m == 0) return 0;
    hipLaunchKernelGGL(skg_add_layernorm_multi_kernel, dim3(rows, m), dim3(256), 0, (hipStream_t)stream, pk, eps);
    return skg_launch_status();
}

extern "C" int skg_add_layernorm_f32(const float* a, int64_t lda, const float* b, int64_t ldb, const float* gamma,
                                     const float* beta, int rows, float eps, float* xsum, float* y, float* stats,
                                     void* stream) {
    if (rows < 0) return SKG_E_ARG;
    if (rows == 0) return 0;
    if (!a || !b || !gamma || !beta || !xsum || !y || !stats) return SKG_E_ARG;
    if ((lda & 3) || (ldb & 3) || !skg_aligned16(a) || !skg_aligned16(b) || !skg_aligned16(gamma) ||
        !skg_aligned16(beta) || !skg_aligned16(xsum) || !skg_aligned16(y))
        return SKG_E_ALIGN;
    hipLaunchKernelGGL(skg_add_layernorm_kernel, dim3(rows), dim3(256), 0, (hipStream_t)stream, a, lda, b, ldb, gamma,
                       beta, eps, xsum, y, stats, skg_twin(y));
    return skg_launch_status();
}

__device__ __forceinline__ void skg_layernorm_bwd_row(const float* __restrict__ dy, int64_t lddy,
                                                      const float* __restrict__ x, const float* __restrict__ stats,
                                                      const float* __restrict__ gamma, float* __restrict__ dx,
                                                      const float* __restrict__ relu_src, float* __restrict__ dx_masked,
                                                      int r, uint16_t* __restrict__ dx16, uint16_t* __restrict__ dxm16) {
    __shared__ float sred[4];
    const int c = threadIdx.x * 4;
    const float mean = stats[2 * r], rstd = stats[2 * r + 1];
    const float4 vx = *reinterpret_cast<const float4*>(x + (int64_t)r * TR_COLS + c);
    const float4 vd = *reinterpret_cast<const float4*>(dy + (int64_t)r * lddy + c);
    const float4 gm = *reinterpret_cast<const float4*>(gamma + c);
    const float4 xh = make_float4((vx.x - mean) * rstd, (vx.y - mean) * rstd, (vx.z - mean) * rstd, (vx.w - mean) * rstd);
    const float4 g = make_float4(vd.x * gm.x, vd.y * gm.y, vd.z * gm.z, vd.w * gm.w);
    const float c1 = skg_block_sum256((g.x + g.y) + (g.z + g.w), sred) / (float)TR_COLS;
    const float c2 = skg_block_sum256((g.x * xh.x + g.y * xh.y) + (g.z * xh.z + g.w * xh.w), sred) / (float)TR_COLS;
    const float4 o = make_float4(rstd * (g.x - c1 - xh.x * c2), rstd * (g.y - c1 - xh.y * c2),
                                 rstd * (g.z - c1 - xh.z * c2), rstd * (g.w - c1 - xh.w * c2));
    *reinterpret_cast<float4*>(dx + (int64_t)r * TR_COLS + c) = o;
    if (dx16) skg_store_twin4(dx16 + (int64_t)r * TR_COLS + c, o);
    if (dx_masked) {
        const float4 m = *reinterpret_cast<const float4*>(relu_src + (int64_t)r * TR_COLS + c);
        const float4 om = make_float4(m.x > 0.f ? o.x : 0.f, m.y > 0.f ? o.y : 0.f, m.z > 0.f ? o.z : 0.f, m.w > 0.f ? o.w : 0.f);
        *reinterpret_cast<float4*>(dx_masked + (int64_t)r * TR_COLS + c) = om;
        if (dxm16) skg_store_twin4(dxm16 + (int64_t)r * TR_COLS + c, om);
    }
}

__global__ __launch_bounds__(256) void skg_layernorm_bwd_kernel(const float* __restrict__ dy, int64_t lddy,
                                                                const float* __restrict__ x,
                                                                const float* __restrict__ stats,
                                                                const float* __restrict__ gamma,
                                                                float* __restrict__ dx,
                                                                const float* __restrict__ relu_src,
                                                                float* __restrict__ dx_masked,
                                                                uint16_t* __restrict__ dx16, uint16_t* __restrict__ dxm16) {
    skg_layernorm_bwd_row(dy, lddy, x, stats, gamma, dx, relu_src, dx_masked, (int)blockIdx.x, dx16, dxm16);
}

#define TR_RG 16
__device__ __forceinline__ void skg_layernorm_param_grad_cols(const float* __restrict__ dy, int64_t lddy,
                                                              const float* __restrict__ x,
                                                              const float* __restrict__ stats, int rows,
                                                              float* __restrict__ dgamma, float* __restrict__ dbeta,
                                                              int blk) {
    __shared__ float sg_s[TR_RG][64], sb_s[TR_RG][64];
    const int cl = threadIdx.x & 63, g = threadIdx.x >> 6;
    const int c = blk * 64 + cl;
    float sg = 0.f, sb = 0.f;
    for (int r = g; r < rows; r += TR_RG) {
        const float d = dy[(int64_t)r * lddy + c];
        sg += d * ((x[(int64_t)r * TR_COLS + c] - stats[2 * r]) * stats[2 * r + 1]);
        sb += d;
    }
    sg_s[g][cl] = sg; sb_s[g][cl] = sb;
    __syncthreads();
    if (g == 0) {
        float a = 0.f, b = 0.f;
#pragma unroll
        for (int q = 0; q < TR_RG; q += 4) {
            a += (sg_s[q][cl] + sg_s[q + 1][cl]) + (sg_s[q + 2][cl] + sg_s[q + 3][cl]);
            b += (sb_s[q][cl] + sb_s[q + 1][cl]) + (sb_s[q + 2][cl] + sb_s[q + 3][cl]);
        }
        dgamma[c] = a;
        dbeta[c] = b;
    }
}
// ... 163 lines not shown
    uint16_t* out16 = to_h ? outH16 : outN16;
    if (!out) return;
    const int a = mode == 2 ? dst : (to_h ? hum_img[dst] : node_img[dst]);
    const skg_image_meta mt = meta[a];
    const int c = threadIdx.x * 4;
    float4 acc = make_float4(0.f, 0.f, 0.f, 0.f);
    auto add = [&](int64_t row) {
        const float4 v = *reinterpret_cast<const float4*>(src + row * ld + c);
        acc.x += v.x; acc.y += v.y; acc.z += v.z; acc.w += v.w;
    };
    if (mode == 0) {
        if (to_h) { const int i = dst - mt.hum_off; for (int j = 0; j < mt.n; ++j) add((int64_t)mt.grid_off + (int64_t)i * mt.n + j); }
        else { const int j = dst - mt.node_off; for (int i = 0; i < mt.n_h; ++i) add((int64_t)mt.grid_off + (int64_t)i * mt.n + j); }
    } else if (mode == 1) {
        if (to_h) { const int i = dst - mt.hum_off; for (int jj = 0; jj < mt.n - 1; ++jj) add((int64_t)mt.pair_off + (int64_t)i * (mt.n - 1) + jj); }
        else {
            const int j = dst - mt.node_off;
            for (int i = 0; i < mt.n_h; ++i) if (i != j) add((int64_t)mt.pair_off + (int64_t)i * (mt.n - 1) + (j < i ? j : j - 1));
        }
    } else {
        const int P = mt.n_h * (mt.n - 1);
        float4 a1 = make_float4(0.f, 0.f, 0.f, 0.f), a2 = a1, a3 = a1;
        const float* base = src + (int64_t)mt.pair_off * ld + c;
        int p = 0;
        for (; p + 3 < P; p += 4) {
            const float4 v0 = *reinterpret_cast<const float4*>(base + (int64_t)p * ld);
            const float4 v1 = *reinterpret_cast<const float4*>(base + (int64_t)(p + 1) * ld);
            const float4 v2 = *reinterpret_cast<const float4*>(base + (int64_t)(p + 2) * ld);
            const float4 v3 = *reinterpret_cast<const float4*>(base + (int64_t)(p + 3) * ld);
            acc.x += v0.x; acc.y += v0.y; acc.z += v0.z; acc.w += v0.w;
            a1.x += v1.x; a1.y += v1.y; a1.z += v1.z; a1.w += v1.w;
            a2.x += v2.x; a2.y += v2.y; a2.z += v2.z; a2.w += v2.w;
            a3.x += v3.x; a3.y += v3.y; a3.z += v3.z; a3.w += v3.w;
        }
        for (; p < P; ++p) add((int64_t)mt.pair_off + p);
        acc.x = (acc.x + a1.x) + (a2.x + a3.x); acc.y = (acc.y + a1.y) + (a2.y + a3.y);
        acc.z = (acc.z + a1.z) + (a2.z + a3.z); acc.w = (acc.w + a1.w) + (a2.w + a3.w);
    }
    float4* o = reinterpret_cast<float4*>(out + (int64_t)(mode == 2 ? mt.image : dst) * TR_COLS + c);
    if (accumulate) { const float4 t = *o; acc.x += t.x; acc.y += t.y; acc.z += t.z; acc.w += t.w; }
    *o = acc;
    if (out16) skg_store_twin4(out16 + (int64_t)(mode == 2 ? mt.image : dst) * TR_COLS + c, acc);
}

__global__ __launch_bounds__(256) void skg_segment_sum_kernel(const float* __restrict__ src, int64_t ld,
                                                              const skg_image_meta* __restrict__ meta,
                                                              const int32_t* __restrict__ hum_img,
                                                              const int32_t* __restrict__ node_img, int n_dst_h, int mode,
                                                              float* __restrict__ outH, float* __restrict__ outN,
                                                              int accumulate, uint16_t* __restrict__ outH16,
                                                              uint16_t* __restrict__ outN16) {
    skg_segment_sum_body(src, ld, meta, hum_img, node_img, n_dst_h, mode, outH, outN, accumulate, (int)blockIdx.x, outH16, outN16);
}

struct skg_segment_sum_pack { skg_segment_sum_args a[SKG_MULTI_MAX]; };
__global__ __launch_bounds__(256) void skg_segment_sum_multi_kernel(const skg_segment_sum_pack pk,
                                                                    const skg_image_meta* __restrict__ meta,
                                                                    const int32_t* __restrict__ hum_img,
                                                                    const int32_t* __restrict__ node_img, int n_dst_h) {
    const skg_segment_sum_args& a = pk.a[blockIdx.y];
    skg_segment_sum_body(a.src, a.ld, meta, hum_img, node_img, n_dst_h, a.mode, a.outH, a.outN, a.accumulate, (int)blockIdx.x,
                         a.outH16, a.outN16);
}

int skg_segment_sum_multi(const skg_segment_sum_args* calls, int n, const skg_image_meta* meta, const int32_t* hum_img,
                          const int32_t* node_img, int sum_h, int sum_n, void* stream) {
    if (!calls || n < 1 || n > SKG_MULTI_MAX || sum_h < 0 || sum_n < 0) return SKG_E_ARG;
    if (sum_h + sum_n == 0) return 0;
    if (!meta || !hum_img || !node_img) return SKG_E_ARG;
    skg_segment_sum_pack pk;
    for (int i = 0; i < n; ++i) {
        const skg_segment_sum_args& a = calls[i];
        if (a.mode < 0 || a.mode > 1 || !a.src || (!a.outH && !a.outN)) return SKG_E_ARG;
        if ((a.ld & 3) || !skg_aligned16(a.src) || !skg_aligned16(a.outH) || !skg_aligned16(a.outN)) return SKG_E_ALIGN;
        pk.a[i] = a;
        pk.a[i].outH16 = a.outH ? skg_twin(a.outH) : nullptr;
        pk.a[i].outN16 = a.outN ? skg_twin(a.outN) : nullptr;
    }
    hipLaunchKernelGGL(skg_segment_sum_multi_kernel, dim3(sum_h + sum_n, n), dim3(256), 0, (hipStream_t)stream, pk, meta,
                       hum_img, node_img, sum_h);
    return skg_launch_status();
}

__global__ __launch_bounds__(256) void skg_segment_sum_image_kernel(const float* __restrict__ src, int64_t ld,
                                                                    const skg_image_meta* __restrict__ meta,
                                                                    float* __restrict__ out, int accumulate,
                                                                    uint16_t* __restrict__ out16) {
    __shared__ float4 red[16][16];
    const skg_image_meta mt = meta[blockIdx.x];
    const int q = threadIdx.x & 15, g = threadIdx.x >> 4;
    const int c = blockIdx.y * 64 + 4 * q;
    const int P = mt.n_h * (mt.n - 1);
    const float* base = src + (int64_t)mt.pair_off * ld + c;
    float4 a0 = make_float4(0.f, 0.f, 0.f, 0.f), a1 = a0;
    int p = g;
    for (; p + 16 < P; p += 32) {
        const float4 v0 = *reinterpret_cast<const float4*>(base + (int64_t)p * ld);
        const float4 v1 = *reinterpret_cast<const float4*>(base + (int64_t)(p + 16) * ld);
        a0.x += v0.x; a0.y += v0.y; a0.z += v0.z; a0.w += v0.w;
        a1.x += v1.x; a1.y += v1.y; a1.z += v1.z; a1.w += v1.w;
    }
    if (p < P) {
        const float4 v0 = *reinterpret_cast<const float4*>(base + (int64_t)p * ld);
        a0.x += v0.x; a0.y += v0.y; a0.z += v0.z; a0.w += v0.w;
    }
    red[g][q] = make_float4(a0.x + a1.x, a0.y + a1.y, a0.z + a1.z, a0.w + a1.w);
    __syncthreads();
    if (g == 0) {
        float4 s = red[0][q];
#pragma unroll
        for (int k = 1; k < 16; ++k) { const float4 t = red[k][q]; s.x += t.x; s.y += t.y; s.z += t.z; s.w += t.w; }
        float4* o = reinterpret_cast<float4*>(out + (int64_t)mt.image * TR_COLS + c);
        if (accumulate) { const float4 t = *o; s.x += t.x; s.y += t.y; s.z += t.z; s.w += t.w; }
        *o = s;
        if (out16) skg_store_twin4(out16 + (int64_t)mt.image * TR_COLS + c, s);
    }
}

extern "C" int skg_segment_sum_f32(const float* src, int64_t ld, const skg_image_meta* meta, int n_active,
                                   const int32_t* hum_img, const int32_t* node_img, int sum_h, int sum_n, int mode,
                                   float* outH, float* outN, int accumulate, void* stream) {
    if (n_active < 0 || sum_h < 0 || sum_n < 0 || mode < 0 || mode > 2) return SKG_E_ARG;
    const int nh = mode == 2 ? n_active : sum_h, nn = mode == 2 ? 0 : sum_n;
    if (nh + nn == 0) return 0;
    if (!src || !meta || (mode != 2 && (!hum_img || !node_img)) || (!outH && !outN)) return SKG_E_ARG;
    if ((ld & 3) || !skg_aligned16(src) || !skg_aligned16(outH) || !skg_aligned16(outN)) return SKG_E_ALIGN;
    if (mode == 2) {
        if (!outH) return SKG_E_ARG;
        hipLaunchKernelGGL(skg_segment_sum_image_kernel, dim3(n_active, TR_COLS / 64), dim3(256), 0, (hipStream_t)stream, src,
                           ld, meta, outH, accumulate, skg_twin(outH));
        return skg_launch_status();
    }
    hipLaunchKernelGGL(skg_segment_sum_kernel, dim3(nh + nn), dim3(256), 0, (hipStream_t)stream, src, ld, meta, hum_img,
                       node_img, nh, mode, outH, outN, accumulate, outH ? skg_twin(outH) : (uint16_t*)nullptr,
                       outN ? skg_twin(outN) : (uint16_t*)nullptr);
    return skg_launch_status();
}

__global__ __launch_bounds__(256) void skg_aggregate_bwd_rows_kernel(
    const float* __restrict__ dU, const float* __restrict__ dV, const float* __restrict__ Tos,
    const float* __restrict__ Tso, const float* __restrict__ alpha, const float* __restrict__ beta,
    const int32_t* __restrict__ grid_h, const int32_t* __restrict__ grid_o, int rows, float* __restrict__ dTos,
    float* __restrict__ dTso, float* __restrict__ da, float* __restrict__ db) {
    const int r = blockIdx.x * 4 + (threadIdx.x >> 6);
    if (r >= rows) return;
    const int lane = threadIdx.x & 63;
    const float al = alpha[r], be = beta[r];
    const float* u = dU + (int64_t)grid_h[r] * TR_COLS;
    const float* v = dV + (int64_t)grid_o[r] * TR_COLS;
    const float* ts = Tos + (int64_t)r * TR_COLS;
    const float* tv = Tso + (int64_t)r * TR_COLS;
    float sa = 0.f, sb = 0.f;
    for (int c = lane * 4; c < TR_COLS; c += 256) {
        const float4 a = *reinterpret_cast<const float4*>(u + c), t = *reinterpret_cast<const float4*>(ts + c);
        const float4 b = *reinterpret_cast<const float4*>(v + c), s = *reinterpret_cast<const float4*>(tv + c);
        sa += (a.x * t.x + a.y * t.y) + (a.z * t.z + a.w * t.w);
        sb += (b.x * s.x + b.y * s.y) + (b.z * s.z + b.w * s.w);
        *reinterpret_cast<float4*>(dTos + (int64_t)r * TR_COLS + c) =
            make_float4(t.x > 0.f ? al * a.x : 0.f, t.y > 0.f ? al * a.y : 0.f, t.z > 0.f ? al * a.z : 0.f, t.w > 0.f ? al * a.w : 0.f);
        *reinterpret_cast<float4*>(dTso + (int64_t)r * TR_COLS + c) =
            make_float4(s.x > 0.f ? be * b.x : 0.f, s.y > 0.f ? be * b.y : 0.f, s.z > 0.f ? be * b.z : 0.f, s.w > 0.f ? be * b.w : 0.f);
    }
    sa = skg_wave_sum(sa); sb = skg_wave_sum(sb);
    if (lane == 0) { da[r] = sa; db[r] = sb; }
}

__global__ __launch_bounds__(64) void skg_aggregate_bwd_softmax_kernel(
    const skg_image_meta* __restrict__ meta, const int32_t* __restrict__ hum_img, const int32_t* __restrict__ node_img,
    int sum_h, const float* __restrict__ alpha, const float* __restrict__ beta, const float* __restrict__ da,
    const float* __restrict__ db, float* __restrict__ dadj_h, float* __restrict__ dadj_n) {
    const bool to_h = (int)blockIdx.x < sum_h;
    const int dst = to_h ? blockIdx.x : blockIdx.x - sum_h;
    const skg_image_meta mt = meta[to_h ? hum_img[dst] : node_img[dst]];
    const int local = to_h ? dst - mt.hum_off : dst - mt.node_off;
    const int cnt = to_h ? mt.n : mt.n_h;
    const int64_t row0 = to_h ? (int64_t)mt.grid_off + (int64_t)local * mt.n : (int64_t)mt.grid_off + local;
    const int64_t step = to_h ? 1 : mt.n;
    const float* w = to_h ? alpha : beta;
    const float* d = to_h ? da : db;
    float* out = to_h ? dadj_h : dadj_n;
    float s = 0.f;
    for (int t = threadIdx.x; t < cnt; t += 64) s += w[row0 + t * step] * d[row0 + t * step];
    s = skg_wave_sum(s);
    for (int t = threadIdx.x; t < cnt; t += 64) {
        const int64_t r = row0 + t * step;
        out[r] = w[r] * (d[r] - s);
    }
}

extern "C" int skg_aggregate_bwd_f32(const float* dU, const float* dV, const float* Tos, const float* Tso,
                                     const float* alpha, const float* beta, const int32_t* grid_h, const int32_t* grid_o,
                                     int sum_g, const skg_image_meta* meta, const int32_t* hum_img,
                                     const int32_t* node_img, int sum_h, int sum_n, float* dTos, float* dTso,
                                     float* da, float* db, float* dadj_h, float* dadj_n, void* stream) {
    if (sum_g < 0 || sum_h < 0 || sum_n < 0) return SKG_E_ARG;
    if (sum_g == 0) return 0;
    if (!dU || !dV || !Tos || !Tso || !alpha || !beta || !grid_h || !grid_o || !meta || !hum_img || !node_img || !dTos ||
        !dTso || !da || !db || !dadj_h || !dadj_n)
        return SKG_E_ARG;
// ... 352 lines not shown
```

skghoi_amd/csrc/skg_train_plan.hip:

```cpp
#include <hip/hip_runtime.h>
#include <string.h>
#include <stdlib.h>
#include <pthread.h>
#include <condition_variable>
#include <mutex>
#include <new>
#include <thread>
#include "skghoi.h"
#include "skg_common.h"

struct skg_train_timer {
    std::mutex m;
    int cap = 0, n = 0;
    hipEvent_t* ev = nullptr;
    double* flops = nullptr;
};

namespace {

struct Mat {
    float* p; int64_t ld; int rows, cols;
    Mat() : p(nullptr), ld(0), rows(0), cols(0) {}
    Mat(float* p_, int r, int c) : p(p_), ld(c), rows(r), cols(c) {}
    Mat(float* p_, int r, int c, int64_t ld_) : p(p_), ld(ld_), rows(r), cols(c) {}
// ... 16 lines not shown
    double flops;
    const float* no_twin;
    const struct Ws* w;
    struct skg_branch* br;
};
struct skg_branch {
    hipStream_t stream;
    hipEvent_t fork, join;
    bool forked;
};
struct OnBranch {
    Ctx& c; hipStream_t s0; float* sc0;
    OnBranch(Ctx& c_, float* scratch2) : c(c_), s0(c_.stream), sc0(c_.scratch) { c.stream = c.br->stream; c.scratch = scratch2; }
    ~OnBranch() { c.stream = s0; c.scratch = sc0; }
};

static uint16_t* twin_of(const Ctx& c, const float* p, int64_t* ld);

struct TwinScope {
    skg_twin_map saved;
    explicit TwinScope(const skg_train_plan* P) : saved(skg_tls_twin) {
        skg_twin_map m = {{nullptr, nullptr}, {nullptr, nullptr}, {0, 0}};
        if (P->bf16 && P->ws16) {
            m.base[0] = P->ws; m.base16[0] = P->ws16; m.n[0] = P->ws_floats;
            if (P->pf16) { m.base[1] = P->pair_features; m.base16[1] = P->pf16; m.n[1] = (int64_t)(P->Mp > 0 ? P->Mp : 1) * 2048; }
        }
        skg_tls_twin = m;
    }
    ~TwinScope() { skg_tls_twin = saved; }
};

static skg_gemmx_desc op_zero() { skg_gemmx_desc d; memset(&d, 0, sizeof(d)); return d; }

static skg_gemmx_desc FWD(const Mat& x, const Mat& W, const Mat& out, const float* bias, bool relu, int M = -1, int K = -1,
                          int N = -1, bool blocks = false) {
    skg_gemmx_desc d = op_zero();
    d.A = x.p; d.a_sm = x.ld; d.a_sk = 1;
    d.B = W.p; d.b_sk = 1;
    d.C = out.p; d.ldc = out.ld;
    d.M = M < 0 ? x.rows : M; d.K = K < 0 ? x.cols : K; d.N = N < 0 ? out.cols : N;
    d.bias = bias; d.relu = relu ? 1 : 0;
    if (!blocks) d.b_sn = W.ld;
    else { d.b_kshift = BLK_SHIFT; d.b_kstride = BLK_STRIDE; d.b_sn = 1 << BLK_SHIFT; }
    return d;
}
static skg_gemmx_desc IG(const Mat& dz, const Mat& W, const Mat& dx, const Mat* mask, bool accumulate, int M = -1,
                         int N_in = -1, int K_out = -1, bool blocks = false) {
    skg_gemmx_desc d = op_zero();
    d.A = dz.p; d.a_sm = dz.ld; d.a_sk = 1;
    d.B = W.p; d.b_sn = 1;
    d.C = dx.p; d.ldc = dx.ld;
    d.M = M < 0 ? dz.rows : M; d.N = N_in < 0 ? dx.cols : N_in; d.K = K_out < 0 ? dz.cols : K_out;
    if (mask) { d.mask = mask->p; d.ldmask = mask->ld; }
    d.accumulate = accumulate ? 1 : 0;
    if (!blocks) d.b_sk = W.ld;
    else { d.b_nshift = BLK_SHIFT; d.b_nstride = BLK_STRIDE; d.b_sk = 1 << BLK_SHIFT; }
    return d;
}
static skg_gemmx_desc WG(const Mat& dz, const Mat& x, const Mat& dW, float* db, bool accumulate, int rows = -1,
                         int n_out = -1, int k_in = -1, bool blocks = false) {
    skg_gemmx_desc d = op_zero();
    d.A = dz.p; d.a_sm = 1; d.a_sk = dz.ld;
    d.B = x.p; d.b_sn = 1; d.b_sk = x.ld;
    d.C = dW.p;
    d.M = n_out < 0 ? dz.cols : n_out; d.N = k_in < 0 ? x.cols : k_in; d.K = rows < 0 ? dz.rows : rows;
    d.a_rowsum = db; d.accumulate = accumulate ? 1 : 0;
    if (!blocks) d.ldc = dW.ld;
    else { d.c_nshift = BLK_SHIFT; d.c_nstride = BLK_STRIDE; d.ldc = 1 << BLK_SHIFT; }
    return d;
}

static int pick_split(const skg_train_plan* P, const skg_gemmx_desc& o, int bk) {
    int64_t tiles = (int64_t)((o.M + 127) / 128) * ((o.N + 127) / 128);
    int kt = (o.K + bk - 1) / bk;
    const int target = P->split_target > 0 ? P->split_target : (bk == 16 ? 500 : 160);
    const int smax = P->split_max > 0 ? P->split_max : 64;
    int cap = kt * bk / 128; if (cap > smax) cap = smax;
    if (tiles == 0 || cap < 2) return 1;
    int sk = (int)((double)target / (double)tiles + 0.5);
    if (sk > cap) sk = cap;
    return sk < 1 ? 1 : sk;
}

static void launch(Ctx& c, skg_gemmx_desc* ops, int n) {
    if (c.rc) return;
    const bool bf16 = c.P->bf16 != 0;
    const int bk = bf16 ? 32 : 16;
    skg_gemmx_desc live[16];
    int m = 0;
    for (int i = 0; i < n; ++i)
        if (ops[i].M > 0 && ops[i].N > 0) live[m++] = ops[i];
    for (int i0 = 0; i0 < m; i0 += SKG_GEMMX_GROUP_MAX) {
        int cnt = m - i0 < SKG_GEMMX_GROUP_MAX ? m - i0 : SKG_GEMMX_GROUP_MAX;
        int64_t used = 0, used_ctr = 0;
        for (int i = 0; i < cnt; ++i) {
            skg_gemmx_desc& d = live[i0 + i];
            int sk = pick_split(c.P, d, bk);
            d.split_k = sk > 1 ? sk : 0;
            d.split_ctr = nullptr;
            if (sk > 1 && c.P->counters) {
                const int64_t tiles = (int64_t)((d.M + 127) / 128) * ((d.N + 127) / 128);
                if (used_ctr + tiles <= c.P->n_counters) { d.split_ctr = c.P->counters + used_ctr; used_ctr += tiles; }
            }
            if (bf16 && !c.dry) {
                d.A16 = twin_of(c, d.A, &d.a16_ld); d.B16 = twin_of(c, d.B, &d.b16_ld);
                int64_t ldc16 = 0;
                uint16_t* c16 = twin_of(c, d.C, &ldc16);
                d.C16 = (c16 && !ldc16 && (d.C < c.P->params || d.C >= c.P->params + c.P->params_floats)) ? c16 : nullptr;
            }
            if (sk > 1) {
                int64_t need = (int64_t)sk * ((int64_t)d.M * d.N + d.M);
                need = (need + 7) & ~(int64_t)7;
                d.split_ws = c.scratch ? c.scratch + used : nullptr;
                used += need;
            }
        }
        if (used > c.scratch_need) c.scratch_need = used;
        for (int i = 0; i < cnt; ++i) c.flops += 2.0 * live[i0 + i].M * (double)live[i0 + i].N * live[i0 + i].K;
        if (c.dry) continue;
        skg_train_timer* tm = c.P->timer;
        int slot = -1;
        double fl = 0.0;
        if (tm) {
            for (int i = 0; i < cnt; ++i) fl += 2.0 * live[i0 + i].M * (double)live[i0 + i].N * live[i0 + i].K;
            std::lock_guard<std::mutex> g(tm->m);
            if (tm->n < tm->cap) { slot = tm->n++; tm->flops[slot] = fl; }
        }
        if (slot >= 0) (void)hipEventRecord(tm->ev[2 * slot], c.stream);
        int rc = bf16 ? skg_gemmx_bf16(live + i0, cnt, c.stream) : skg_gemmx_f32(live + i0, cnt, c.stream);
        if (slot >= 0) (void)hipEventRecord(tm->ev[2 * slot + 1], c.stream);
        if (rc) { c.rc = rc; return; }
    }
}
#define CK(call) do { if (!c.rc && !c.dry) { int rc__ = (call); if (rc__) c.rc = rc__; } } while (0)

__global__ void b3sum_kernel(const float* __restrict__ b3, float* __restrict__ out) {
    int i = blockIdx.x * blockDim.x + threadIdx.x;
    if (i >= 4 * 1024) return;
    int m = i >> 10, col = i & 1023;
    float s = 0.f;
    for (int b = 0; b < 16; ++b) s += b3[((int64_t)m * 16 + b) * 1024 + col];
    out[i] = s;
}
__global__ void b3bcast_kernel(const float* __restrict__ db3, float* __restrict__ out) {
    int i = blockIdx.x * blockDim.x + threadIdx.x;
    if (i >= 4 * 16 * 1024) return;
    int m = i >> 14, col = i & 1023;
    out[i] = db3[m * 1024 + col];
}
__global__ __launch_bounds__(1024) void colsum2_kernel(const float* __restrict__ X, int rx, const float* __restrict__ Y, int ry,
                                                       float* __restrict__ out) {
    __shared__ float red[16][64];
    const int lane = threadIdx.x & 63, col = blockIdx.x * 64 + lane;
    const int part = threadIdx.x >> 6;
    float s = 0.f, t = 0.f;
    for (int r = part; r < rx; r += 16) s += X[(int64_t)r * 1024 + col];
    for (int r = part; r < ry; r += 16) t += Y[(int64_t)r * 1024 + col];
    red[part][lane] = s + t;
    __syncthreads();
    if (part == 0) {
        float a = 0.f;
#pragma unroll
        for (int q = 0; q < 16; q += 4) a += (red[q][lane] + red[q + 1][lane]) + (red[q + 2][lane] + red[q + 3][lane]);
        out[col] = a;
    }
}

#define ADJW_ROWS 16
__global__ __launch_bounds__(256) void adjw_partial_kernel(const float* __restrict__ dadj, const float* __restrict__ Wt,
                                                           int rows, float* __restrict__ part) {
    const int col = (blockIdx.x & 3) * 256 + threadIdx.x, chunk = blockIdx.x >> 2;
    const int r0 = chunk * ADJW_ROWS;
    float s = 0.f, sb = 0.f;
    if (r0 + ADJW_ROWS <= rows) {
        float d[ADJW_ROWS], v[ADJW_ROWS];
#pragma unroll
        for (int i = 0; i < ADJW_ROWS; ++i) { d[i] = dadj[r0 + i]; v[i] = Wt[(int64_t)(r0 + i) * 1024 + col]; }
#pragma unroll
        for (int i = 0; i < ADJW_ROWS; ++i) { s += d[i] * v[i]; sb += d[i]; }
    } else {
        for (int r = r0; r < rows; ++r) {
            const float d = dadj[r];
            s += d * Wt[(int64_t)r * 1024 + col];
            sb += d;
        }
    }
    part[(int64_t)chunk * 1028 + col] = s;
    if (col == 0) part[(int64_t)chunk * 1028 + 1024] = sb;
}
__global__ __launch_bounds__(1024) void adjw_finish_kernel(const float* __restrict__ part, int chunks, float* __restrict__ dw,
                                                           float* __restrict__ db) {
    __shared__ float red[16][64];
    const int lane = threadIdx.x & 63, g = threadIdx.x >> 6, col = blockIdx.x * 64 + lane;
    float s = 0.f;
    if (col <= 1024)
        for (int k = g; k < chunks; k += 16) s += part[(int64_t)k * 1028 + col];
    red[g][lane] = s;
    __syncthreads();
    if (g == 0 && col <= 1024) {
        float a = 0.f;
#pragma unroll
        for (int q = 0; q < 16; q += 4) a += (red[q][lane] + red[q + 1][lane]) + (red[q + 2][lane] + red[q + 3][lane]);
        if (col < 1024) dw[col] = a; else db[0] = a;
    }
}

__global__ __launch_bounds__(256) void zero_selfpair_rows_kernel(float* __restrict__ dF, uint16_t* __restrict__ dF16,
                                                                 const int32_t* __restrict__ grid_pair, int Mg) {
    const int g = blockIdx.x;
    if (grid_pair[g] >= 0) return;
    const int c = threadIdx.x * 4;
    const float4 z = make_float4(0.f, 0.f, 0.f, 0.f);
// ... 61 lines not shown
    w.total = off;
    w.scratch = base ? base + off : nullptr;
    w.scratch2 = nullptr;
}

static uint16_t* twin_of(const Ctx& c, const float* p, int64_t* ld) {
    const skg_train_plan* P = c.P;
    *ld = 0;
    if (!P->ws16 || !p) return nullptr;
    if (p >= P->ws && p < P->ws + P->ws_floats) return (c.no_twin && p == c.no_twin) ? nullptr : P->ws16 + (p - P->ws);
    const int64_t npf = (int64_t)(P->Mp > 0 ? P->Mp : 1) * 2048;
    if (P->pf16 && p >= P->pair_features && p < P->pair_features + npf) return P->pf16 + (p - P->pair_features);
    const Ws* w = c.w;
    if (w && w->side && w->x0t) {
        auto side = [&](const float* region) { return P->ws16 + (region - P->ws); };
        const float* fh = P->params + P->seg_off[SKG_SEG_FH_W];
        const float* ft = P->params + P->seg_off[SKG_SEG_FT_W];
        const float* s0 = P->params + P->seg_off[SKG_SEG_SP0_W];
        if (p == fh) { *ld = FH_PITCH; return side(w->fhw_t); }
        if (p == ft) { *ld = FH_PITCH; return side(w->ftw_t); }
        if (p == s0) { *ld = SP0_PITCH; return side(w->sp0w_t); }
        if (p >= P->x0 && p < P->x0 + (int64_t)P->NA * P->x0_k) return side(w->x0t) + (p - P->x0);
        if (p >= P->sp48 && p < P->sp48 + (int64_t)P->Mg * SKG_SPATIAL_LD) return side(w->sp48t) + (p - P->sp48);
        if (p >= P->gfeat && p < P->gfeat + (int64_t)P->Bf * P->Cf) return side(w->gft) + (p - P->gfeat);
        if (P->dlogits && P->Mp > 0 && p == P->dlogits) { *ld = (P->ld_logits + 7) & ~7; return side(w->dlog_t); }
    }
    if (P->params16 && p >= P->params && p < P->params + P->params_floats) return P->params16 + (p - P->params);
    return nullptr;
}

struct TwinSeg { const float* src; uint16_t* dst; int64_t ld_src, ld_dst; int rows, cols; int64_t first; };
struct TwinSegs { TwinSeg s[8]; int n; int64_t total; };
__global__ __launch_bounds__(256) void twin_segments_kernel(const TwinSegs g) {
    for (int64_t i = (int64_t)blockIdx.x * 256 + threadIdx.x; i < g.total; i += (int64_t)gridDim.x * 256) {
        int k = 0;
#pragma unroll
        for (int t = 1; t < 8; ++t)
            if (t < g.n && i >= g.s[t].first) k = t;
        const TwinSeg& sg = g.s[k];
        const int64_t local = i - sg.first, qpr = sg.ld_dst >> 2;
        const int64_t row = local / qpr;
        const int col = (int)(local - row * qpr) * 4;
        const float* sp = sg.src + row * sg.ld_src + col;
        float4 v = make_float4(0.f, 0.f, 0.f, 0.f);
        if (col + 3 < sg.cols && (sg.ld_src & 3) == 0 && skg_aligned16_dev(sg.src)) v = *reinterpret_cast<const float4*>(sp);
        else {
            if (col < sg.cols) v.x = sp[0];
            if (col + 1 < sg.cols) v.y = sp[1];
            if (col + 2 < sg.cols) v.z = sp[2];
            if (col + 3 < sg.cols) v.w = sp[3];
        }
        skg_store_twin4(sg.dst + row * sg.ld_dst + col, v);
    }
}
static void twin_segments(Ctx& c, TwinSeg* segs, int n) {
    if (c.rc || c.dry || n == 0) return;
    TwinSegs g; g.n = 0; g.total = 0;
    for (int i = 0; i < n; ++i) {
        if (segs[i].rows <= 0 || !segs[i].src || !segs[i].dst) continue;
        segs[i].first = g.total;
        g.total += (int64_t)segs[i].rows * (segs[i].ld_dst >> 2);
        g.s[g.n++] = segs[i];
    }
    if (!g.n) return;
    int64_t blocks = (g.total + 255) / 256;
    if (blocks > 8192) blocks = 8192;
    hipLaunchKernelGGL(twin_segments_kernel, dim3((unsigned)blocks), dim3(256), 0, c.stream, g);
}

struct Seg {
    const skg_train_plan* P; float* base;
    float* at(int s) const { return base + P->seg_off[s]; }
};

static int check_plan(const skg_train_plan* P) {
    if (!P || !P->params || !P->meta) return SKG_E_ARG;
    if (P->NA <= 0 || P->Mg <= 0 || P->Mh <= 0 || P->Mn <= 0 || P->A <= 0 || P->K <= 0 || P->Bf <= 0 || P->Cf <= 0 ||
        P->x0_k <= 0 || P->Mp < 0)
        return SKG_E_ARG;
    if (P->ld_logits < P->K + 1 || (P->ld_logits & 3)) return SKG_E_ARG;
    return 0;
}

static void forward(Ctx& c, const Ws& w, int part) {
    const skg_train_plan* P = c.P;
    Seg W{P, const_cast<float*>(P->params)};
    const int NA = P->NA, Mg = P->Mg, Mp = P->Mp, Mh = P->Mh, Mn = P->Mn, A = P->A, K = P->K, Bf = P->Bf, Cf = P->Cf;
    const int kx = P->x0_k;
    Mat x0 = cm(P->x0, NA, kx), gfeat = cm(P->gfeat, Bf, Cf), sp48 = cm(P->sp48, Mg, SKG_SPATIAL_LD);
    Mat E1(w.E1, NA, 1024), enc(w.enc, NA, 1024), G1(w.G1, Bf, 1024), s1(w.s1, Mg, 128), s2(w.s2, Mg, 256);
    Mat bh1_w(W.at(SKG_SEG_BH1_W), 1024, kx), bh3_w(W.at(SKG_SEG_BH3_W), 1024, 1024);
    Mat sp0_w(W.at(SKG_SEG_SP0_W), 128, 46), sp2_w(W.at(SKG_SEG_SP2_W), 256, 128), sp4_w(W.at(SKG_SEG_SP4_W), 1024, 256);
    Mat W1[4] = {Mat(W.at(SKG_SEG_W1_0), 1024, 2048), Mat(W.at(SKG_SEG_W1_1), 1024, 1024),
                 Mat(W.at(SKG_SEG_W1_2), 1024, 1024), Mat(W.at(SKG_SEG_W1_3), 1024, Cf)};
    float* b1[4] = {W.at(SKG_SEG_B1_0), W.at(SKG_SEG_B1_1), W.at(SKG_SEG_B1_2), W.at(SKG_SEG_B1_3)};
    Mat W3[4] = {Mat(W.at(SKG_SEG_W3_0), 1024, 1024), Mat(W.at(SKG_SEG_W3_1), 1024, 1024),
                 Mat(W.at(SKG_SEG_W3_2), 1024, 1024), Mat(W.at(SKG_SEG_W3_3), 1024, 1024)};
    enum { ATT = 0, OS = 1, SO = 2, GL = 3 };
    if (part == 0) {
        if (!c.dry)
            hipLaunchKernelGGL(b3sum_kernel, dim3(16), dim3(256), 0, c.stream, W.at(SKG_SEG_B3), w.b3sum);
        if (P->bf16 && P->params16 && P->params_floats > 0)
            CK(skg_twin_bf16(P->params, P->params16, P->params_floats & ~(int64_t)3, c.stream));
        if (w.side && P->ws16 && !c.dry) {
            auto side = [&](const float* region) { return P->ws16 + (region - P->ws); };
            TwinSeg sg[6] = {{P->x0, side(w.x0t), kx, kx, NA, kx, 0}, {P->sp48, side(w.sp48t), SKG_SPATIAL_LD, SKG_SPATIAL_LD, Mg, SKG_SPATIAL_LD, 0},
                             {P->gfeat, side(w.gft), Cf, Cf, Bf, Cf, 0},
                             {W.at(SKG_SEG_FH_W), side(w.fhw_t), 1074, FH_PITCH, 1024, 1074, 0},
                             {W.at(SKG_SEG_FT_W), side(w.ftw_t), 1074, FH_PITCH, 1024, 1074, 0},
                             {W.at(SKG_SEG_SP0_W), side(w.sp0w_t), 46, SP0_PITCH, 128, 46, 0}};
            twin_segments(c, sg, 6);
        }
        skg_gemmx_desc l1[2] = {FWD(x0, bh1_w, E1, W.at(SKG_SEG_BH1_B), true),
                                FWD(sp48, sp0_w, s1, W.at(SKG_SEG_SP0_B), true, -1, 46)};
        launch(c, l1, 2);
        skg_gemmx_desc l2[3] = {FWD(E1, bh3_w, enc, W.at(SKG_SEG_BH3_B), true), FWD(gfeat, W1[GL], G1, b1[GL], false),
                                FWD(s1, sp2_w, s2, W.at(SKG_SEG_SP2_B), true)};
        launch(c, l2, 3);
        return;
    }
    const float* b3 = w.b3sum;
    const int Mp1 = Mp > 0 ? Mp : 1;
    Mat Xhn(w.Xhn, Mh + Mn, 1088), GH(w.GH, Mh, 1024), GO(w.GO, Mn, 1024), Sp(w.Sp, Mg, 1024);
    Mat fh_w(W.at(SKG_SEG_FH_W), 1024, 1074), ft_w(W.at(SKG_SEG_FT_W), 1024, 1074);
    Mat A1h(w.A1h, Mh, 1024), A1o(w.A1o, Mn, 1024), C1o(w.C1o, Mn, 1024), C1h(w.C1h, Mh, 1024);
    Mat Wa1 = W1[ATT];
    Mat F(w.F, Mg, 4096), T(w.T, Mg, 1024), Tos(w.Tos, Mg, 1024), Tso(w.Tso, Mg, 1024), Tg(w.Tg, Mp1, 1024);
    const float* W2 = W.at(SKG_SEG_W2); const float* b2 = W.at(SKG_SEG_B2);
    auto node_chain = [&]() {
        CK(skg_concat_entity_f32(w.enc, 1024, P->enc_row_hn, P->ent, P->img_hn, P->ent_row_hn, Mh + Mn, w.Xhn, 1088, c.stream));
        skg_gemmx_desc l[2] = {FWD(Xhn.row_range(0, Mh), fh_w, GH, W.at(SKG_SEG_FH_B), true, -1, 1074),
                               FWD(Xhn.row_range(Mh, Mn), ft_w, GO, W.at(SKG_SEG_FT_B), true, -1, 1074)};
        launch(c, l, 2);
        skg_gemmx_desc l4[4] = {FWD(GH, Wa1, A1h, nullptr, false, -1, 1024), FWD(GO, Wa1.from_col(1024), A1o, nullptr, false, -1, 1024),
                                FWD(GO, W1[OS], C1o, b1[OS], false), FWD(GH, W1[SO], C1h, b1[SO], false)};
        launch(c, l4, 4);
    };
    const bool two = c.br != nullptr && P->bf16 && !c.dry;
    if (two) {
        CK((int)hipEventRecord(c.br->fork, c.stream));
        CK((int)hipStreamWaitEvent(c.br->stream, c.br->fork, 0));
        {
            OnBranch on(c, w.scratch2);
            node_chain();
            CK((int)hipEventRecord(c.br->join, c.stream));
        }
        skg_gemmx_desc l[1] = {FWD(s2, sp4_w, Sp, W.at(SKG_SEG_SP4_B), true)};
        launch(c, l, 1);
    } else {
        CK(skg_concat_entity_f32(w.enc, 1024, P->enc_row_hn, P->ent, P->img_hn, P->ent_row_hn, Mh + Mn, w.Xhn, 1088, c.stream));
        skg_gemmx_desc l[3] = {FWD(Xhn.row_range(0, Mh), fh_w, GH, W.at(SKG_SEG_FH_B), true, -1, 1074),
                               FWD(Xhn.row_range(Mh, Mn), ft_w, GO, W.at(SKG_SEG_FT_B), true, -1, 1074),
                               FWD(s2, sp4_w, Sp, W.at(SKG_SEG_SP4_B), true)};
        launch(c, l, 3);
        skg_gemmx_desc l4[4] = {FWD(GH, Wa1, A1h, nullptr, false, -1, 1024), FWD(GO, Wa1.from_col(1024), A1o, nullptr, false, -1, 1024),
                                FWD(GO, W1[OS], C1o, b1[OS], false), FWD(GH, W1[SO], C1h, b1[SO], false)};
        launch(c, l4, 4);
    }
    if (P->bf16) {
        skg_gemmx_desc l[1] = {FWD(Sp, cm(W2, 4096, 1024), F, b2, false)};
        launch(c, l, 1);
        if (two) CK((int)hipStreamWaitEvent(c.stream, c.br->join, 0));
        {
            skg_rows_mul_args m[4] = {
                {w.A1h, P->grid_h, 1024, w.A1o, P->grid_o, 1024, b1[ATT], w.F, nullptr, 4096, Mg, 1024, w.T, 1024},
                {w.C1o, P->grid_o, 1024, nullptr, nullptr, 1024, nullptr, w.F + 1024, nullptr, 4096, Mg, 1024, w.Tos, 1024},
                {w.C1h, P->grid_h, 1024, nullptr, nullptr, 1024, nullptr, w.F + 2048, nullptr, 4096, Mg, 1024, w.Tso, 1024},
                {w.G1, P->pair_img, 1024, nullptr, nullptr, 1024, nullptr, w.F + 3072, P->pair_grid, 4096, Mp, 1024, w.Tg, 1024}};
            CK(skg_rows_mul_relu_multi(m, Mp > 0 ? 4 : 3, c.stream));
        }
    } else {
        skg_gemm_desc ds[4];
        for (int i = 0; i < 4; ++i) {
            skg_gemm_desc& d = ds[i]; memset(&d, 0, sizeof(d));
            d.A = w.Sp; d.lda = 1024; d.W = W2 + (int64_t)1024 * 1024 * i; d.ldw = 1024; d.bias = b2 + 1024 * i;
            d.ldc = 1024; d.M = Mg; d.N = 1024; d.K = 1024; d.epilogue = SKG_EPI_MUL_RELU;
            d.C_raw = w.F + 1024 * i; d.ldc_raw = 4096;
            if (i == ATT) { d.C = w.T; d.P = w.A1h; d.p_idx = P->grid_h; d.ldp = 1024; d.Q = w.A1o; d.q_idx = P->grid_o;
                            d.ldq = 1024; d.mbias = b1[ATT]; }
            else if (i == OS) { d.C = w.Tos; d.P = w.C1o; d.p_idx = P->grid_o; d.ldp = 1024; }
            else if (i == SO) { d.C = w.Tso; d.P = w.C1h; d.p_idx = P->grid_h; d.ldp = 1024; }
            else { d.C = w.Tg; d.P = w.G1; d.p_idx = P->grid_img; d.ldp = 1024; d.out_rows = P->grid_pair; }
            c.flops += 2.0 * Mg * 1024.0 * 1024.0;
        }
        if ((int64_t)((Mg + 127) / 128) * 8 * 4 < 1536) {
            CK(skg_gemm_group_f32(ds, 4, c.stream));
        } else {
            for (int i = 0; i < 4; ++i) CK(skg_gemm_f32(&ds[i], c.stream));
        }
    }
    Mat Wt(w.Wt, Mg, 1024);
    {
        skg_gemmx_desc l[1] = {FWD(T, W3[ATT], Wt, b3 + 1024 * ATT, true, -1, -1, -1, true)};
        launch(c, l, 1);
    }
    CK(skg_rowdot_f32(w.Wt, 1024, W.at(SKG_SEG_ADJ_W), Mg, 1024, w.adj_raw, c.stream));
    CK(skg_graph_aggregate_train_f32(w.adj_raw, 1, Mg, 0.0f, P->meta, A, P->hum_img, P->node_img, Mh, Mn, w.Tos, w.Tso,
                                     1024, 1024, w.U, w.V, 1024, w.adj, w.alpha, w.beta, c.stream));
    Mat U(w.U, Mh, 1024), V(w.V, Mn, 1024), M1(w.M1, Mh, 1024), M2(w.M2, Mn, 1024);
    {
        skg_gemmx_desc l[2] = {FWD(U, W3[OS], M1, b3 + 1024 * OS, true, -1, -1, -1, true),
                               FWD(V, W3[SO], M2, b3 + 1024 * SO, true, -1, -1, -1, true)};
        launch(c, l, 2);
    }
    {
        skg_add_layernorm_args ln[2] = {
            {w.GH, 1024, w.M1, 1024, W.at(SKG_SEG_NH_W), W.at(SKG_SEG_NH_B), Mh, w.Hp, w.h_node, w.st_h},
            {w.GO, 1024, w.M2, 1024, W.at(SKG_SEG_NO_W), W.at(SKG_SEG_NO_B), Mn, w.Op, w.node, w.st_o}};
        CK(skg_add_layernorm_multi(ln, 2, 1e-5f, c.stream));
    }
    Mat h_node(w.h_node, Mh, 1024), node(w.node, Mn, 1024), B1h(w.B1h, Mh, 1024), B1o(w.B1o, Mn, 1024);
    {
        skg_gemmx_desc l[2] = {FWD(h_node, Wa1, B1h, nullptr, false, -1, 1024),
                               FWD(node, Wa1.from_col(1024), B1o, nullptr, false, -1, 1024)};
        launch(c, l, 2);
    }
    if (Mp > 0)
        CK(skg_rows_mul_relu_f32(w.B1h, P->pair_h, 1024, w.B1o, P->pair_o, 1024, b1[ATT], w.F, P->pair_grid, 4096, Mp,
                                 1024, w.Tp, 1024, c.stream));
    Mat Tp(w.Tp, Mp1, 1024), PF(P->pair_features, Mp1, 2048);
    {
        skg_gemmx_desc l[2] = {FWD(Tp, W3[ATT], PF, b3 + 1024 * ATT, true, Mp, -1, 1024, true),
                               FWD(Tg, W3[GL], PF.from_col(1024), b3 + 1024 * GL, true, Mp, -1, 1024, true)};
        launch(c, l, 2);
    }
    {
        Mat logits(P->logits, Mp1, P->ld_logits);
        skg_gemmx_desc l[1] = {FWD(PF, Mat(W.at(SKG_SEG_CLS_W), K + 1, 2048), logits, W.at(SKG_SEG_CLS_B), false, Mp, -1, K + 1)};
        launch(c, l, 1);
    }
}

static void backward(Ctx& c, const Ws& w, int first, int last) {
    const skg_train_plan* P = c.P;
    Seg W{P, const_cast<float*>(P->params)}, G{P, P->grads};
    const int NA = P->NA, Mg = P->Mg, Mp = P->Mp, Mh = P->Mh, Mn = P->Mn, A = P->A, K = P->K, Bf = P->Bf, Cf = P->Cf;
    const int kx = P->x0_k, Mp1 = Mp > 0 ? Mp : 1;
    enum { ATT = 0, OS = 1, SO = 2, GL = 3 };
    Mat W1[4] = {Mat(W.at(SKG_SEG_W1_0), 1024, 2048), Mat(W.at(SKG_SEG_W1_1), 1024, 1024),
                 Mat(W.at(SKG_SEG_W1_2), 1024, 1024), Mat(W.at(SKG_SEG_W1_3), 1024, Cf)};
    Mat dW1[4] = {Mat(G.at(SKG_SEG_W1_0), 1024, 2048), Mat(G.at(SKG_SEG_W1_1), 1024, 1024),
                  Mat(G.at(SKG_SEG_W1_2), 1024, 1024), Mat(G.at(SKG_SEG_W1_3), 1024, Cf)};
    float* b1[4] = {W.at(SKG_SEG_B1_0), W.at(SKG_SEG_B1_1), W.at(SKG_SEG_B1_2), W.at(SKG_SEG_B1_3)};
    float* db1[4] = {G.at(SKG_SEG_B1_0), G.at(SKG_SEG_B1_1), G.at(SKG_SEG_B1_2), G.at(SKG_SEG_B1_3)};
    Mat W3[4] = {Mat(W.at(SKG_SEG_W3_0), 1024, 1024), Mat(W.at(SKG_SEG_W3_1), 1024, 1024),
                 Mat(W.at(SKG_SEG_W3_2), 1024, 1024), Mat(W.at(SKG_SEG_W3_3), 1024, 1024)};
    Mat dW3[4] = {Mat(G.at(SKG_SEG_W3_0), 1024, 1024), Mat(G.at(SKG_SEG_W3_1), 1024, 1024),
                  Mat(G.at(SKG_SEG_W3_2), 1024, 1024), Mat(G.at(SKG_SEG_W3_3), 1024, 1024)};
    float* db3 = w.db3;
    Mat dlogits = cm(P->dlogits, Mp1, P->ld_logits);
    Mat PF(P->pair_features, Mp1, 2048), Tp(w.Tp, Mp1, 1024), Tg(w.Tg, Mp1, 1024);
    Mat dPF(w.dPF, Mp1, 2048), dTp(w.dTp, Mp1, 1024), dTg(w.dTg, Mp1, 1024);
    Mat Wa1 = W1[ATT], dWa1 = dW1[ATT];
    Mat dB1h(w.dB1h, Mh, 1024), dB1o(w.dB1o, Mn, 1024), dG1(w.dG1, Bf, 1024);
    Mat dh_node(w.dh_node, Mh, 1024), dnode(w.dnode, Mn, 1024), h_node(w.h_node, Mh, 1024), node(w.node, Mn, 1024);
    Mat dHp(w.dHp, Mh, 1024), dHm(w.dHm, Mh, 1024), dOp(w.dOp, Mn, 1024), dOm(w.dOm, Mn, 1024);
    Mat dU(w.dU, Mh, 1024), dV(w.dV, Mn, 1024), U(w.U, Mh, 1024), V(w.V, Mn, 1024);
    Mat dWt(w.dWt, Mg, 1024), dT(w.dT, Mg, 1024), T(w.T, Mg, 1024), Wt(w.Wt, Mg, 1024), dadj(w.dadj, Mg, 1);
    Mat dA1h(w.dA1h, Mh, 1024), dA1o(w.dA1o, Mn, 1024), dC1o(w.dC1o, Mn, 1024), dC1h(w.dC1h, Mh, 1024);
    Mat GH(w.GH, Mh, 1024), GO(w.GO, Mn, 1024), Sp(w.Sp, Mg, 1024), dS(w.dS, Mg, 1024), dF(w.dF, Mg, 4096);
    Mat s1(w.s1, Mg, 128), s2(w.s2, Mg, 256), ds1(w.ds1, Mg, 128), ds2(w.ds2, Mg, 256), sp48 = cm(P->sp48, Mg, SKG_SPATIAL_LD);
    Mat sp0_w(W.at(SKG_SEG_SP0_W), 128, 46), sp2_w(W.at(SKG_SEG_SP2_W), 256, 128), sp4_w(W.at(SKG_SEG_SP4_W), 1024, 256);
    Mat g_sp0(G.at(SKG_SEG_SP0_W), 128, 46), g_sp2(G.at(SKG_SEG_SP2_W), 256, 128), g_sp4(G.at(SKG_SEG_SP4_W), 1024, 256);
    Mat Xhn(w.Xhn, Mh + Mn, 1088), dXhn(w.dXhn, Mh + Mn, 1088);
    Mat fh_w(W.at(SKG_SEG_FH_W), 1024, 1074), ft_w(W.at(SKG_SEG_FT_W), 1024, 1074);
    Mat g_fh(G.at(SKG_SEG_FH_W), 1024, 1074), g_ft(G.at(SKG_SEG_FT_W), 1024, 1074);
    Mat gfeat = cm(P->gfeat, Bf, Cf), x0 = cm(P->x0, NA, kx);
    Mat E1(w.E1, NA, 1024), dE1(w.dE1, NA, 1024), d_enc(w.d_enc, NA, 1024);
    Mat bh1_w(W.at(SKG_SEG_BH1_W), 1024, kx), bh3_w(W.at(SKG_SEG_BH3_W), 1024, 1024);
    Mat g_bh1(G.at(SKG_SEG_BH1_W), 1024, kx), g_bh3(G.at(SKG_SEG_BH3_W), 1024, 1024);
    const bool two = c.br != nullptr && P->bf16 && !c.dry;
    bool no_branch = false;
    bool& forked = two ? c.br->forked : no_branch;
    auto on_node = [&](auto&& fn) {
        if (two && forked) { OnBranch on(c, w.scratch2); fn(); }
        else fn();
    };
    for (int st = first; st < last && !c.rc; ++st) switch (st) {
    case 0: {
        if (w.side && P->ws16 && Mp > 0 && !c.dry) {
            TwinSeg sg[1] = {{P->dlogits, P->ws16 + (w.dlog_t - P->ws), P->ld_logits, (P->ld_logits + 7) & ~7, Mp, P->ld_logits, 0}};
            twin_segments(c, sg, 1);
        }
        Mat clsW(W.at(SKG_SEG_CLS_W), K + 1, 2048), g_clsW(G.at(SKG_SEG_CLS_W), K + 1, 2048);
        skg_gemmx_desc l[2] = {IG(dlogits, clsW, dPF, &PF, false, Mp, 2048, K + 1),
                               WG(dlogits, PF, g_clsW, G.at(SKG_SEG_CLS_B), false, Mp, K + 1, 2048)};
        launch(c, l, 2);
    } break;
    case 1: {
        skg_gemmx_desc l[4] = {IG(dPF, W3[ATT], dTp, &Tp, false, Mp, 1024, 1024, true),
                               IG(dPF.from_col(1024), W3[GL], dTg, &Tg, false, Mp, 1024, 1024, true),
                               WG(dPF, Tp, dW3[ATT], db3 + 1024 * ATT, false, Mp, 1024, 1024, true),
                               WG(dPF.from_col(1024), Tg, dW3[GL], db3 + 1024 * GL, false, Mp, 1024, 1024, true)};
        launch(c, l, 4);
        if (!c.dry) {
            uint16_t* dF16 = (P->bf16 && P->ws16) ? P->ws16 + (w.dF - P->ws) : nullptr;
            if (Mp > 0) {
                hipLaunchKernelGGL(zero_selfpair_rows_kernel, dim3(Mg), dim3(256), 0, c.stream, w.dF, dF16, P->grid_pair, Mg);
                if (A < Bf) {
                    hipError_t e = hipMemsetAsync(w.dG1, 0, sizeof(float) * (size_t)Bf * 1024, c.stream);
                    if (e == hipSuccess && dF16)
                        e = hipMemsetAsync(P->ws16 + (w.dG1 - P->ws), 0, sizeof(uint16_t) * (size_t)Bf * 1024, c.stream);
                    if (e != hipSuccess) { c.rc = (int)e; break; }
                }
            } else {
                const size_t nz = (size_t)((w.dG1 - w.dF) + (int64_t)Bf * 1024);
                hipError_t e = hipMemsetAsync(w.dF, 0, sizeof(float) * nz, c.stream);
                if (e == hipSuccess && dF16) e = hipMemsetAsync(dF16, 0, sizeof(uint16_t) * nz, c.stream);
                if (e != hipSuccess) { c.rc = (int)e; break; }
            }
        }
        if (Mp > 0) {
            skg_mul_bwd_args m[2] = {
                {w.dTp, 1024, w.F, P->pair_grid, 4096, w.B1h, P->pair_h, 1024, w.B1o, P->pair_o, 1024, b1[ATT], Mp, w.dF, 4096, 0},
                {w.dTg, 1024, w.F + 3072, P->pair_grid, 4096, w.G1, P->pair_img, 1024, nullptr, nullptr, 0, nullptr, Mp,
                 w.dF + 3072, 4096, 0}};
            CK(skg_mul_bwd_multi(m, 2, c.stream));
        }
        CK(skg_segment_sum_f32(w.dTp, 1024, P->meta, A, P->hum_img, P->node_img, Mh, Mn, 1, w.dB1h, w.dB1o, 0, c.stream));
        CK(skg_segment_sum_f32(w.dTg, 1024, P->meta, A, nullptr, nullptr, 0, 0, 2, w.dG1, nullptr, 0, c.stream));
        skg_gemmx_desc l2[4] = {IG(dB1h, Wa1, dh_node, nullptr, false, -1, 1024), IG(dB1o, Wa1.from_col(1024), dnode, nullptr, false, -1, 1024),
                                WG(dB1h, h_node, dWa1, nullptr, false, -1, -1, 1024),
                                WG(dB1o, node, dWa1.from_col(1024), nullptr, false, -1, -1, 1024)};
        launch(c, l2, 4);
    } break;
    case 2: {
        skg_layernorm_bwd_args ln[2] = {
            {w.dh_node, 1024, w.Hp, w.st_h, W.at(SKG_SEG_NH_W), Mh, w.dHp, w.M1, w.dHm, G.at(SKG_SEG_NH_W), G.at(SKG_SEG_NH_B)},
            {w.dnode, 1024, w.Op, w.st_o, W.at(SKG_SEG_NO_W), Mn, w.dOp, w.M2, w.dOm, G.at(SKG_SEG_NO_W), G.at(SKG_SEG_NO_B)}};
        CK(skg_layernorm_bwd_multi(ln, 2, c.stream));
    } break;
    case 3: {
        skg_gemmx_desc l[4] = {IG(dHm, W3[OS], dU, nullptr, false, -1, 1024, -1, true), IG(dOm, W3[SO], dV, nullptr, false, -1, 1024, -1, true),
                               WG(dHm, U, dW3[OS], db3 + 1024 * OS, false, -1, -1, -1, true),
                               WG(dOm, V, dW3[SO], db3 + 1024 * SO, false, -1, -1, -1, true)};
        launch(c, l, 4);
    } break;
    case 4: {
        float* da = w.da;
        CK(skg_aggregate_bwd_f32(w.dU, w.dV, w.Tos, w.Tso, w.alpha, w.beta, P->grid_h, P->grid_o, Mg, P->meta, P->hum_img,
                                 P->node_img, Mh, Mn, w.dTos, w.dTso, da, da + Mg, da + 2 * (int64_t)Mg, da + 3 * (int64_t)Mg,
                                 c.stream));
        CK(skg_adjacency_bwd_f32(da + 2 * (int64_t)Mg, da + 3 * (int64_t)Mg, W.at(SKG_SEG_ADJ_W), w.Wt, Mg, w.dadj, w.dWt,
                                 c.stream));
        skg_gemmx_desc l[3] = {IG(dWt, W3[ATT], dT, &T, false, -1, 1024, -1, true),
                               WG(dWt, T, dW3[ATT], db3 + 1024 * ATT, true, -1, -1, -1, true),
                               WG(dadj, Wt, Mat(G.at(SKG_SEG_ADJ_W), 1, 1024), G.at(SKG_SEG_ADJ_B), false)};
        if (P->bf16 && w.side) {
            const int chunks = (Mg + ADJW_ROWS - 1) / ADJW_ROWS;
            const int64_t need = (int64_t)chunks * 1028;
            if (need > c.scratch_need) c.scratch_need = need;
            c.flops += 2.0 * Mg * 1024.0;
            if (!c.dry && !c.rc) {
                hipLaunchKernelGGL(adjw_partial_kernel, dim3(4 * chunks), dim3(256), 0, c.stream, w.dadj, w.Wt, Mg, c.scratch);
                hipLaunchKernelGGL(adjw_finish_kernel, dim3(17), dim3(1024), 0, c.stream, c.scratch, chunks,
                                   G.at(SKG_SEG_ADJ_W), G.at(SKG_SEG_ADJ_B));
            }
            launch(c, l, 2);
        } else {
            launch(c, l, 3);
        }
    } break;
    case 5: {
        {
            skg_mul_bwd_args m[3] = {
                {w.dT, 1024, w.F, nullptr, 4096, w.A1h, P->grid_h, 1024, w.A1o, P->grid_o, 1024, b1[ATT], Mg, w.dF, 4096, 1},
                {w.dTos, 1024, w.F + 1024, nullptr, 4096, w.C1o, P->grid_o, 1024, nullptr, nullptr, 0, nullptr, Mg, w.dF + 1024,
                 4096, 0},
                {w.dTso, 1024, w.F + 2048, nullptr, 4096, w.C1h, P->grid_h, 1024, nullptr, nullptr, 0, nullptr, Mg, w.dF + 2048,
                 4096, 0}};
            CK(skg_mul_bwd_multi(m, 3, c.stream));
            skg_segment_sum_args g[3] = {{w.dT, 1024, 0, w.dA1h, w.dA1o, 0}, {w.dTos, 1024, 0, nullptr, w.dC1o, 0},
                                         {w.dTso, 1024, 0, w.dC1h, nullptr, 0}};
            CK(skg_segment_sum_multi(g, 3, P->meta, P->hum_img, P->node_img, Mh, Mn, c.stream));
        }
        if (!c.dry)
            hipLaunchKernelGGL(colsum2_kernel, dim3(16), dim3(1024), 0, c.stream, w.dA1h, Mh, w.dB1h, Mh, db1[ATT]);
    } break;
    case 6: {
        if (two && !forked) {
            CK((int)hipEventRecord(c.br->fork, c.stream));
            CK((int)hipStreamWaitEvent(c.br->stream, c.br->fork, 0));
            forked = !c.rc;
        }
        Mat W2(W.at(SKG_SEG_W2), 4096, 1024), g_W2(G.at(SKG_SEG_W2), 4096, 1024);
        skg_gemmx_desc l[2] = {IG(dF, W2, dS, &Sp, false, -1, 1024), WG(dF, Sp, g_W2, G.at(SKG_SEG_B2), false)};
        launch(c, l, 2);
    } break;
    case 7: {
        skg_gemmx_desc l[6] = {IG(dA1h, Wa1, dHp, nullptr, true, -1, 1024), IG(dA1o, Wa1.from_col(1024), dOp, nullptr, true, -1, 1024),
                               WG(dA1h, GH, dWa1, nullptr, true, -1, -1, 1024),
                               WG(dA1o, GO, dWa1.from_col(1024), nullptr, true, -1, -1, 1024),
                               IG(dS, sp4_w, ds2, &s2, false), WG(dS, s2, g_sp4, G.at(SKG_SEG_SP4_B), false)};
        if (two && forked) { on_node([&] { launch(c, l, 4); }); launch(c, l + 4, 2); }
        else launch(c, l, 6);
    } break;
    case 8: {
        skg_gemmx_desc l[6] = {IG(dC1h, W1[SO], dHp, &GH, true), IG(dC1o, W1[OS], dOp, &GO, true),
                               WG(dC1h, GH, dW1[SO], db1[SO], false), WG(dC1o, GO, dW1[OS], db1[OS], false),
                               IG(ds2, sp2_w, ds1, &s1, false), WG(ds2, s1, g_sp2, G.at(SKG_SEG_SP2_B), false)};
        if (two && forked) { on_node([&] { launch(c, l, 4); }); launch(c, l + 4, 2); }
        else launch(c, l, 6);
    } break;
// ... 483 lines not shown
```

Measured before the change: 8321 images/s.

## Fuse gating, row-dot, split-K reduction and segment sums into neighbouring training kernels

Adds a gated GEMM epilogue so the bf16 W2 projection writes the gated ReLU products (T, Tos, Tso, Tg) directly. This replaces the separate rows-mul-relu pass. It also folds the adjacency row-dot into the graph aggregate kernel, and lets the split-K slices of the M1/M2 GEMMs be reduced inside the add-layernorm kernel instead of a separate reduction. The two backward segment-sum launches are merged into one. These changes cut kernel launches and intermediate memory traffic in the training plan, at the cost of more epilogue logic and new restrictions (the gated path rejects split-K). They live in the training forward/backward, so the eval benchmark path may not exercise them.

Result: slower. 8161 images/s (-1.9%).

```diff
diff --git a/include/skghoi.h b/include/skghoi.h
--- a/include/skghoi.h
+++ b/include/skghoi.h
@@ -281,6 +281,38 @@
                           float* dadj, float* dWt, void* stream);
 int skg_entity_rows_bwd_f32(const float* dX, int64_t ldx, const int32_t* hum_of, const int32_t* node_of, int sum_h,
                             int n_enc, const float* enc, float* d_enc, void* stream);
+
+int skg_graph_aggregate_rowdot_train_f32(const float* X, int64_t ldx, const float* w, float* adj_raw,
+                                         const skg_image_meta* meta, int n_active, const int32_t* hum_img,
+                                         const int32_t* node_img, int sum_h, int sum_n, const float* T_os,
+                                         const float* T_so, int64_t ldt, int cols, float* U, float* V, int64_t ldu,
+                                         float* adj_out, float* alpha_out, float* beta_out, void* stream);
+typedef struct {
+    const float* a; int64_t lda;
+    float* b; int64_t ldb;
+    const float* slices; int64_t slice_stride; int32_t S, relu;
+    const float* bias;
+    const float* gamma; const float* beta;
+    int32_t rows, reserved;
+    float* xsum; float* y; float* stats;
+} skg_add_layernorm_slices_args;
+int skg_add_layernorm_slices_f32(const skg_add_layernorm_slices_args* calls_host, int n, float eps, void* stream);
+int skg_gemmx_slices(const skg_gemmx_desc* descs_host, int n, int bf16, void* stream);
+typedef struct {
+    const float* src; int64_t ld; int32_t mode, accumulate; float* outH; float* outN;
+} skg_segment_sum_entry;
+int skg_segment_sum_modes_f32(const skg_segment_sum_entry* calls_host, int n, const skg_image_meta* meta, int n_active,
+                              const int32_t* hum_img, const int32_t* node_img, int sum_h, int sum_n, void* stream);
+typedef struct {
+    const float* P; const int32_t* p_idx; int64_t ldp;
+    const float* Q; const int32_t* q_idx; int64_t ldq;
+    const float* mbias;
+    float* out; uint16_t* out16; int64_t ldo;
+    const int32_t* out_rows;
+} skg_gemmx_gate_block;
+typedef struct { int32_t n_blocks, block_cols; skg_gemmx_gate_block b[4]; } skg_gemmx_gate;
+int skg_gemmx_gated(const skg_gemmx_desc* desc_host, const skg_gemmx_gate* gate_host, int bf16, void* stream);
+
 #define SKG_LOSS_CHUNKS 64
 int skg_hoi_loss_f32(const float* logits, int64_t ldl, int K, const skg_image_meta* meta, int n_active,
                      int64_t cells_total, const int64_t* index, const int64_t* pred, const float* scores,
diff --git a/skghoi_amd/_capi.py b/skghoi_amd/_capi.py
--- a/skghoi_amd/_capi.py
+++ b/skghoi_amd/_capi.py
@@ -53,6 +53,25 @@
     _fields_ = [("A", _vp), ("lda", _i64), ("W", _vp), ("ldw", _i64), ("bias", _vp), ("C", _vp), ("ldc", _i64),
                 ("M", _i32), ("N", _i32), ("K", _i32), ("relu", _i32), ("out_bf16", _i32), ("split_k", _i32),
                 ("split_ws", _vp)]
+
+
+class AddLayerNormSlicesArgs(C.Structure):
+    _fields_ = [("a", _vp), ("lda", _i64), ("b", _vp), ("ldb", _i64), ("slices", _vp), ("slice_stride", _i64),
+                ("S", _i32), ("relu", _i32), ("bias", _vp), ("gamma", _vp), ("beta", _vp), ("rows", _i32),
+                ("reserved", _i32), ("xsum", _vp), ("y", _vp), ("stats", _vp)]
+
+
+class SegmentSumEntry(C.Structure):
+    _fields_ = [("src", _vp), ("ld", _i64), ("mode", _i32), ("accumulate", _i32), ("outH", _vp), ("outN", _vp)]
+
+
+class GemmXGateBlock(C.Structure):
+    _fields_ = [("P", _vp), ("p_idx", _vp), ("ldp", _i64), ("Q", _vp), ("q_idx", _vp), ("ldq", _i64), ("mbias", _vp),
+                ("out", _vp), ("out16", _vp), ("ldo", _i64), ("out_rows", _vp)]
+
+
+class GemmXGate(C.Structure):
+    _fields_ = [("n_blocks", _i32), ("block_cols", _i32), ("b", GemmXGateBlock * 4)]
 
 
 TRAIN_SEGS = ("W1_0", "W1_1", "W1_2", "W1_3", "b1_0", "b1_1", "b1_2", "b1_3", "W3_0", "W3_1", "W3_2", "W3_3", "b3", "W2",
@@ -202,6 +221,13 @@
                                         _vp, _vp, _vp, _vp, _vp, _vp, _vp]),
     "skg_adjacency_bwd_f32": (C.c_int, [_vp, _vp, _vp, _vp, C.c_int, _vp, _vp, _vp]),
     "skg_entity_rows_bwd_f32": (C.c_int, [_vp, _i64, _vp, _vp, C.c_int, C.c_int, _vp, _vp, _vp]),
+    "skg_graph_aggregate_rowdot_train_f32": (C.c_int, [_vp, _i64, _vp, _vp, _vp, C.c_int, _vp, _vp, C.c_int, C.c_int, _vp,
+                                                       _vp, _i64, C.c_int, _vp, _vp, _i64, _vp, _vp, _vp, _vp]),
+    "skg_add_layernorm_slices_f32": (C.c_int, [C.POINTER(AddLayerNormSlicesArgs), C.c_int, _f32, _vp]),
+    "skg_gemmx_slices": (C.c_int, [C.POINTER(GemmXDesc), C.c_int, C.c_int, _vp]),
+    "skg_segment_sum_modes_f32": (C.c_int, [C.POINTER(SegmentSumEntry), C.c_int, _vp, C.c_int, _vp, _vp, C.c_int, C.c_int,
+                                            _vp]),
+    "skg_gemmx_gated": (C.c_int, [C.POINTER(GemmXDesc), C.POINTER(GemmXGate), C.c_int, _vp]),
     "skg_eval_associate_f32": (C.c_int, [_vp, _vp, _vp, _vp, _vp, _vp, _vp, _vp, C.c_int, _vp, C.c_int, C.c_int, _vp, _vp,
                                          _vp, _vp, _f32, _vp, _vp, _vp, _vp]),
     "skg_eval_ap11_f64": (C.c_int, [_vp, _vp, _vp, C.c_int, _vp, _vp, _vp]),
diff --git a/skghoi_amd/csrc/skg_common.h b/skghoi_amd/csrc/skg_common.h
--- a/skghoi_amd/csrc/skg_common.h
+++ b/skghoi_amd/csrc/skg_common.h
@@ -68,7 +68,9 @@
     float* C_raw; int64_t ldc_raw;
     const int32_t* out_rows;
     const float* res; int64_t ldres;
+    uint16_t* C_raw16;
 };
+#define SKG_GEMMX_EPI_GATE 16
 int skg_gemmx_can_fuse(const skg_gemmx_desc* d, const skg_gemmx_fused* f);
 int skg_gemmx_f32_fused(const skg_gemmx_desc* descs_host, const skg_gemmx_fused* fused_host, int n, void* stream);
 
diff --git a/skghoi_amd/csrc/skg_gemm_x.hip b/skghoi_amd/csrc/skg_gemm_x.hip
--- a/skghoi_amd/csrc/skg_gemm_x.hip
+++ b/skghoi_amd/csrc/skg_gemm_x.hip
@@ -155,6 +155,23 @@
     if (hb) { v.x += bv.x; v.y += bv.y; v.z += bv.z; v.w += bv.w; }
     if (f.kind | (f.out_rows != nullptr)) {
         const int orow = f.out_rows ? f.out_rows[row] : row;
+        if (f.kind == SKG_GEMMX_EPI_GATE) {
+            *reinterpret_cast<float4*>(f.C_raw + (int64_t)row * f.ldc_raw + col) = v;
+            if (f.C_raw16)
+                *reinterpret_cast<uint2*>(f.C_raw16 + (int64_t)row * f.ldc_raw + col) = make_uint2(ypack(v.x, v.y), ypack(v.z, v.w));
+            if (orow < 0) return;
+            float4 m = xld4(f.P + (int64_t)(f.p_idx ? f.p_idx[row] : row) * f.ldp + col);
+            if (f.Q) {
+                const float4 t = xld4(f.Q + (int64_t)(f.q_idx ? f.q_idx[row] : row) * f.ldq + col);
+                m.x += t.x; m.y += t.y; m.z += t.z; m.w += t.w;
+            }
+            if (f.mbias) { m.x += mb.x; m.y += mb.y; m.z += mb.z; m.w += mb.w; }
+            const float4 res = make_float4(fmaxf(m.x * v.x, 0.f), fmaxf(m.y * v.y, 0.f), fmaxf(m.z * v.z, 0.f), fmaxf(m.w * v.w, 0.f));
+            float* p = d.C + coff + (int64_t)orow * d.ldc;
+            *reinterpret_cast<float4*>(p) = res;
+            if (d.C16) *reinterpret_cast<uint2*>(d.C16 + (p - d.C)) = make_uint2(ypack(res.x, res.y), ypack(res.z, res.w));
+            return;
+        }
         if (f.kind == SKG_EPI_MUL_RELU) {
             if (f.C_raw) *reinterpret_cast<float4*>(f.C_raw + (int64_t)row * f.ldc_raw + col) = v;
             if (orow < 0) return;
@@ -202,7 +219,7 @@
     const bool hb = !ws && d.bias;
     float4 bv = xzero4(), mb = xzero4();
     if (hb) bv = xld4(d.bias + col);
-    if (f.kind == SKG_EPI_MUL_RELU && f.mbias) mb = xld4(f.mbias + col);
+    if ((f.kind == SKG_EPI_MUL_RELU || f.kind == SKG_GEMMX_EPI_GATE) && f.mbias) mb = xld4(f.mbias + col);
     const int64_t coff = xoff(col, d.c_nshift, d.c_nstride, 1);
 #pragma unroll
     for (int i = 0; i < 8; ++i) {
@@ -224,7 +241,7 @@
     const bool hb = d.bias != nullptr;
     float4 bv = xzero4(), mb = xzero4();
     if (hb) bv = xld4(d.bias + col);
-    if (f.kind == SKG_EPI_MUL_RELU && f.mbias) mb = xld4(f.mbias + col);
+    if ((f.kind == SKG_EPI_MUL_RELU || f.kind == SKG_GEMMX_EPI_GATE) && f.mbias) mb = xld4(f.mbias + col);
     const int64_t coff = xoff(col, d.c_nshift, d.c_nstride, 1);
 #pragma unroll 1
     for (int h = 0; h < 8 / R; ++h) {
@@ -1473,7 +1490,7 @@
 static bool g_t16_enabled = getenv("SKG_GEMMX_T16") == nullptr || atoi(getenv("SKG_GEMMX_T16")) != 0;
 
 static int skg_gemmx_launch(const skg_gemmx_desc* descs_host, int n, void* stream, bool bf16,
-                            const skg_gemmx_fused* fused_host = nullptr) {
+                            const skg_gemmx_fused* fused_host = nullptr, bool keep_slices = false) {
     if (!descs_host || n < 1 || n > SKG_GEMMX_GROUP_MAX) return SKG_E_ARG;
     skg_gemmx_group g, r;
     memset(g.f, 0, sizeof(g.f)); memset(r.f, 0, sizeof(r.f));
@@ -1485,6 +1502,7 @@
         if (rc) return rc;
         if (d.M == 0 || d.N == 0) continue;
         const int S = d.split_k > 1 ? d.split_k : 1;
+        if (keep_slices && S > 1 && (d.a_rowsum || d.accumulate || d.mask)) return SKG_E_ARG;
         const int64_t nb = (int64_t)((d.M + XBM - 1) / XBM) * ((d.N + XBN - 1) / XBN) * S;
         if (blocks + nb > 0x7fffffffLL) return SKG_E_LIMIT;
         int vec = 0;
@@ -1511,17 +1529,18 @@
             (!d.b16_ld || xfits32((int64_t)(d.b_sk == 1 ? d.N : d.K) * ldb16 + 8)))
             vec |= 32;
         if (fused_host && (fused_host[i].kind || fused_host[i].out_rows)) {
-            if (!(vec & 8) || (S > 1 && !(d.split_ctr && (int64_t)d.M * d.N < (1LL << 29))) || d.c_nshift || d.accumulate || d.mask || d.C16 ||
-                !xfused_ptrs_ok(fused_host[i]))
+            const bool gate = fused_host[i].kind == SKG_GEMMX_EPI_GATE;
+            if (!(vec & 8) || (S > 1 && (gate || !(d.split_ctr && (int64_t)d.M * d.N < (1LL << 29)))) || d.c_nshift || d.accumulate ||
+                d.mask || (d.C16 && !gate) || !xfused_ptrs_ok(fused_host[i]))
                 return SKG_E_ARG;
             g.f[g.n] = fused_host[i];
         }
         g.d[g.n] = d; g.vec[g.n] = vec; g.start[g.n] = (int)blocks;
-        const bool inlaunch = S > 1 && d.split_ctr && (vec & 8) && (int64_t)d.M * d.N < (1LL << 29);
+        const bool inlaunch = !keep_slices && S > 1 && d.split_ctr && (vec & 8) && (int64_t)d.M * d.N < (1LL << 29);
         if (!inlaunch) g.d[g.n].split_ctr = nullptr;
         ++g.n;
         blocks += nb;
-        if (S > 1 && !inlaunch) {
+        if (S > 1 && !inlaunch && !keep_slices) {
             const int64_t MN = (int64_t)d.M * d.N;
             const int64_t total = ((vec & 8) ? MN / 4 : MN) + (d.a_rowsum ? d.M : 0);
             const int64_t nr = (total + 255) / 256;
@@ -1575,3 +1594,42 @@
 extern "C" int skg_gemmx_bf16(const skg_gemmx_desc* descs_host, int n, void* stream) {
     return skg_gemmx_launch(descs_host, n, stream, true);
 }
+
+extern "C" int skg_gemmx_slices(const skg_gemmx_desc* descs_host, int n, int bf16, void* stream) {
+    return skg_gemmx_launch(descs_host, n, stream, bf16 != 0, nullptr, true);
+}
+
+extern "C" int skg_gemmx_gated(const skg_gemmx_desc* dp, const skg_gemmx_gate* gp, int bf16, void* stream) {
+    if (!dp || !gp) return SKG_E_ARG;
+    const skg_gemmx_desc& d = *dp;
+    const skg_gemmx_gate& gt = *gp;
+    if (gt.n_blocks < 1 || gt.n_blocks > 4 || gt.block_cols <= 0 || (gt.block_cols % XBN) || d.N != gt.n_blocks * gt.block_cols)
+        return SKG_E_ARG;
+    if (d.M < 0 || !d.C || d.relu || d.accumulate || d.mask || d.a_rowsum || d.split_k > 1 || d.b_nshift || d.c_nshift)
+        return SKG_E_ARG;
+    if (d.M == 0) return 0;
+    skg_gemmx_desc xs[4];
+    skg_gemmx_fused fs[4];
+    for (int k = 0; k < gt.n_blocks; ++k) {
+        const skg_gemmx_gate_block& b = gt.b[k];
+        if (!b.P || !b.out || b.ldo < gt.block_cols) return SKG_E_ARG;
+        if ((((uintptr_t)b.out16) & 7u) || !skg_aligned16(b.out) || !xmul4(b.ldo)) return SKG_E_ALIGN;
+        const int64_t c0 = (int64_t)k * gt.block_cols;
+        skg_gemmx_desc& x = xs[k];
+        x = d;
+        x.N = gt.block_cols;
+        x.B = d.B + c0 * d.b_sn;
+        if (d.B16) x.B16 = d.B16 + c0 * ((d.b_sk == 1 && d.b16_ld) ? d.b16_ld : d.b_sn);
+        if (d.bias) x.bias = d.bias + c0;
+        x.C = b.out; x.ldc = b.ldo; x.C16 = b.out16;
+        x.split_k = 0; x.split_ws = nullptr; x.split_ctr = nullptr;
+        skg_gemmx_fused& f = fs[k];
+        memset(&f, 0, sizeof(f));
+        f.kind = SKG_GEMMX_EPI_GATE;
+        f.P = b.P; f.p_idx = b.p_idx; f.ldp = b.ldp; f.Q = b.Q; f.q_idx = b.q_idx; f.ldq = b.ldq; f.mbias = b.mbias;
+        f.C_raw = d.C + c0; f.ldc_raw = d.ldc; f.C_raw16 = d.C16 ? d.C16 + c0 : nullptr;
+        f.out_rows = b.out_rows;
+        if ((((uintptr_t)f.C_raw16) & 7u)) return SKG_E_ALIGN;
+    }
+    return skg_gemmx_launch(xs, gt.n_blocks, stream, bf16 != 0, fs);
+}
diff --git a/skghoi_amd/csrc/skg_graph.hip b/skghoi_amd/csrc/skg_graph.hip
--- a/skghoi_amd/csrc/skg_graph.hip
+++ b/skghoi_amd/csrc/skg_graph.hip
@@ -1,7 +1,9 @@
 #include "skg_common.h"
 
+template <bool DOT>
 __global__ __launch_bounds__(256) void skg_graph_aggregate_kernel(
     const float* __restrict__ dot_partial, int n_partial, int64_t partial_ld, float adj_bias,
+    const float* __restrict__ X, int64_t ldx, const float* __restrict__ w, float* __restrict__ raw_out,
     const skg_image_meta* __restrict__ meta, const int32_t* __restrict__ hum_img, const int32_t* __restrict__ node_img,
     int sum_h, const float* __restrict__ T_os, const float* __restrict__ T_so, int64_t ldt, int cols,
     float* __restrict__ U, float* __restrict__ V, int64_t ldu, float* __restrict__ adj_out,
@@ -19,7 +21,29 @@
     const int64_t row0 = to_human ? (int64_t)mt.grid_off + (int64_t)local * mt.n : (int64_t)mt.grid_off + local;
     const int64_t rstep = to_human ? 1 : mt.n;
 
-    for (int t = tid; t < cnt; t += 256) {
+    if (DOT) {
+        const int lane = tid & 63;
+        for (int t = tid >> 6; t < cnt; t += 4) {
+            const int64_t gr = row0 + t * rstep;
+            const float* x = X + gr * ldx;
+            float s = 0.f;
+            for (int c = lane * 4; c < cols; c += 256) {
+                const float4 a = *reinterpret_cast<const float4*>(x + c);
+                const float4 b = *reinterpret_cast<const float4*>(w + c);
+                s += (a.x * b.x + a.y * b.y) + (a.z * b.z + a.w * b.w);
+            }
+            s = skg_wave_sum(s);
+            if (lane == 0) {
+                if (to_human) raw_out[gr] = s;
+                float l = 0.f;
+                l += s;
+                l += adj_bias;
+                sw[t] = l;
+                if (to_human && adj_out) adj_out[gr] = l;
+            }
+        }
+    }
+    for (int t = tid; !DOT && t < cnt; t += 256) {
         const int64_t gr = row0 + t * rstep;
         float s = 0.f;
         for (int k = 0; k < n_partial; ++k) s += dot_partial[(int64_t)k * partial_ld + gr];
@@ -78,8 +102,8 @@
     if ((ldt & 3) || (ldu & 3) || !skg_aligned16(T_os) || !skg_aligned16(T_so) || (((uintptr_t)U) & amask) ||
         (((uintptr_t)V) & amask))
         return SKG_E_ALIGN;
-    hipLaunchKernelGGL(skg_graph_aggregate_kernel, dim3(sum_h + sum_n), dim3(256), 0, (hipStream_t)stream, dot_partial,
-                       n_partial, partial_ld, adj_bias, meta, hum_img, node_img, sum_h, T_os, T_so, ldt, cols,
+    hipLaunchKernelGGL(skg_graph_aggregate_kernel<false>, dim3(sum_h + sum_n), dim3(256), 0, (hipStream_t)stream, dot_partial,
+                       n_partial, partial_ld, adj_bias, (const float*)nullptr, (int64_t)0, (const float*)nullptr, (float*)nullptr, meta, hum_img, node_img, sum_h, T_os, T_so, ldt, cols,
                        half ? (float*)nullptr : (float*)U, half ? (float*)nullptr : (float*)V, ldu, adj_out,
                        (float*)nullptr, (float*)nullptr, half ? (uint16_t*)U : (uint16_t*)nullptr,
                        half ? (uint16_t*)V : (uint16_t*)nullptr);
@@ -107,9 +131,28 @@
     if ((ldt & 3) || (ldu & 3) || !skg_aligned16(T_os) || !skg_aligned16(T_so) || !skg_aligned16(U) ||
         !skg_aligned16(V))
         return SKG_E_ALIGN;
-    hipLaunchKernelGGL(skg_graph_aggregate_kernel, dim3(sum_h + sum_n), dim3(256), 0, (hipStream_t)stream, dot_partial,
-                       n_partial, partial_ld, adj_bias, meta, hum_img, node_img, sum_h, T_os, T_so, ldt, cols, U, V,
+    hipLaunchKernelGGL(skg_graph_aggregate_kernel<false>, dim3(sum_h + sum_n), dim3(256), 0, (hipStream_t)stream, dot_partial,
+                       n_partial, partial_ld, adj_bias, (const float*)nullptr, (int64_t)0, (const float*)nullptr, (float*)nullptr, meta, hum_img, node_img, sum_h, T_os, T_so, ldt, cols, U, V,
                        ldu, adj_out, alpha_out, beta_out, skg_twin(U), skg_twin(V));
+    return skg_launch_status();
+}
+
+extern "C" int skg_graph_aggregate_rowdot_train_f32(const float* X, int64_t ldx, const float* w, float* adj_raw,
+                                                    const skg_image_meta* meta, int n_active, const int32_t* hum_img,
+                                                    const int32_t* node_img, int sum_h, int sum_n, const float* T_os,
+                                                    const float* T_so, int64_t ldt, int cols, float* U, float* V,
+                                                    int64_t ldu, float* adj_out, float* alpha_out, float* beta_out,
+                                                    void* stream) {
+    if (n_active < 0 || sum_h < 0 || sum_n < 0 || cols <= 0 || (cols & 3)) return SKG_E_ARG;
+    if (sum_h + sum_n == 0) return 0;
+    if (!X || !w || !adj_raw || !meta || !hum_img || !node_img || !T_os || !T_so || !U || !V || !alpha_out || !beta_out)
+        return SKG_E_ARG;
+    if ((ldx & 3) || (ldt & 3) || (ldu & 3) || !skg_aligned16(X) || !skg_aligned16(w) || !skg_aligned16(T_os) ||
+        !skg_aligned16(T_so) || !skg_aligned16(U) || !skg_aligned16(V))
+        return SKG_E_ALIGN;
+    hipLaunchKernelGGL(skg_graph_aggregate_kernel<true>, dim3(sum_h + sum_n), dim3(256), 0, (hipStream_t)stream,
+                       (const float*)nullptr, 1, (int64_t)0, 0.0f, X, ldx, w, adj_raw, meta, hum_img, node_img, sum_h, T_os,
+                       T_so, ldt, cols, U, V, ldu, adj_out, alpha_out, beta_out, skg_twin(U), skg_twin(V));
     return skg_launch_status();
 }
 
diff --git a/skghoi_amd/csrc/skg_train.hip b/skghoi_amd/csrc/skg_train.hip
--- a/skghoi_amd/csrc/skg_train.hip
+++ b/skghoi_amd/csrc/skg_train.hip
@@ -85,6 +85,67 @@
     }
     if (m == 0) return 0;
     hipLaunchKernelGGL(skg_add_layernorm_multi_kernel, dim3(rows, m), dim3(256), 0, (hipStream_t)stream, pk, eps);
+    return skg_launch_status();
+}
+
+struct skg_add_layernorm_slices_item { skg_add_layernorm_slices_args a; uint16_t* y16; };
+struct skg_add_layernorm_slices_pack { skg_add_layernorm_slices_item a[SKG_MULTI_MAX]; };
+__global__ __launch_bounds__(256) void skg_add_layernorm_slices_kernel(const skg_add_layernorm_slices_pack pk, float eps) {
+    __shared__ float sred[4];
+    const skg_add_layernorm_slices_args& a = pk.a[blockIdx.y].a;
+    const int r = blockIdx.x;
+    if (r >= a.rows) return;
+    const int c = threadIdx.x * 4;
+    const float4 va = *reinterpret_cast<const float4*>(a.a + (int64_t)r * a.lda + c);
+    float4 vb;
+    if (a.S > 0) {
+        vb = make_float4(0.f, 0.f, 0.f, 0.f);
+        const float* sp = a.slices + (int64_t)r * TR_COLS + c;
+        for (int s = 0; s < a.S; ++s) {
+            const float4 q = *reinterpret_cast<const float4*>(sp + (int64_t)s * a.slice_stride);
+            vb.x += q.x; vb.y += q.y; vb.z += q.z; vb.w += q.w;
+        }
+        if (a.bias) { const float4 bv = *reinterpret_cast<const float4*>(a.bias + c); vb.x += bv.x; vb.y += bv.y; vb.z += bv.z; vb.w += bv.w; }
+        if (a.relu) { vb.x = fmaxf(vb.x, 0.f); vb.y = fmaxf(vb.y, 0.f); vb.z = fmaxf(vb.z, 0.f); vb.w = fmaxf(vb.w, 0.f); }
+        *reinterpret_cast<float4*>(a.b + (int64_t)r * a.ldb + c) = vb;
+    } else {
+        vb = *reinterpret_cast<const float4*>(a.b + (int64_t)r * a.ldb + c);
+    }
+    const float4 v = make_float4(va.x + vb.x, va.y + vb.y, va.z + vb.z, va.w + vb.w);
+    const float mean = skg_block_sum256((v.x + v.y) + (v.z + v.w), sred) / (float)TR_COLS;
+    const float4 d = make_float4(v.x - mean, v.y - mean, v.z - mean, v.w - mean);
+    const float var = skg_block_sum256((d.x * d.x + d.y * d.y) + (d.z * d.z + d.w * d.w), sred) / (float)TR_COLS;
+    const float rstd = 1.f / sqrtf(var + eps);
+    const float4 g = *reinterpret_cast<const float4*>(a.gamma + c);
+    const float4 bb = *reinterpret_cast<const float4*>(a.beta + c);
+    *reinterpret_cast<float4*>(a.xsum + (int64_t)r * TR_COLS + c) = v;
+    const float4 yo = make_float4(d.x * rstd * g.x + bb.x, d.y * rstd * g.y + bb.y, d.z * rstd * g.z + bb.z, d.w * rstd * g.w + bb.w);
+    *reinterpret_cast<float4*>(a.y + (int64_t)r * TR_COLS + c) = yo;
+    uint16_t* y16 = pk.a[blockIdx.y].y16;
+    if (y16) skg_store_twin4(y16 + (int64_t)r * TR_COLS + c, yo);
+    if (threadIdx.x == 0) { a.stats[2 * r] = mean; a.stats[2 * r + 1] = rstd; }
+}
+
+extern "C" int skg_add_layernorm_slices_f32(const skg_add_layernorm_slices_args* calls, int n, float eps, void* stream) {
+    if (!calls || n < 1 || n > SKG_MULTI_MAX) return SKG_E_ARG;
+    skg_add_layernorm_slices_pack pk;
+    int m = 0, rows = 0;
+    for (int i = 0; i < n; ++i) {
+        const skg_add_layernorm_slices_args& a = calls[i];
+        if (a.rows < 0 || a.S < 0 || a.S > 256) return SKG_E_ARG;
+        if (a.rows == 0) continue;
+        if (!a.a || !a.b || !a.gamma || !a.beta || !a.xsum || !a.y || !a.stats) return SKG_E_ARG;
+        if (a.S > 0 && (!a.slices || a.slice_stride < (int64_t)a.rows * TR_COLS)) return SKG_E_ARG;
+        if ((a.lda & 3) || (a.ldb & 3) || !skg_aligned16(a.a) || !skg_aligned16(a.b) || !skg_aligned16(a.gamma) ||
+            !skg_aligned16(a.beta) || !skg_aligned16(a.xsum) || !skg_aligned16(a.y))
+            return SKG_E_ALIGN;
+        if (a.S > 0 && ((a.slice_stride & 3) || !skg_aligned16(a.slices) || !skg_aligned16(a.bias))) return SKG_E_ALIGN;
+        pk.a[m].a = a;
+        pk.a[m++].y16 = skg_twin(a.y);
+        rows = a.rows > rows ? a.rows : rows;
+    }
+    if (m == 0) return 0;
+    hipLaunchKernelGGL(skg_add_layernorm_slices_kernel, dim3(rows, m), dim3(256), 0, (hipStream_t)stream, pk, eps);
     return skg_launch_status();
 }
 
@@ -414,14 +475,14 @@
     return skg_launch_status();
 }
 
-__global__ __launch_bounds__(256) void skg_segment_sum_image_kernel(const float* __restrict__ src, int64_t ld,
-                                                                    const skg_image_meta* __restrict__ meta,
-                                                                    float* __restrict__ out, int accumulate,
-                                                                    uint16_t* __restrict__ out16) {
+__device__ __forceinline__ void skg_segment_sum_image_body(const float* __restrict__ src, int64_t ld,
+                                                           const skg_image_meta* __restrict__ meta,
+                                                           float* __restrict__ out, int accumulate,
+                                                           uint16_t* __restrict__ out16, int img, int cblk) {
     __shared__ float4 red[16][16];
-    const skg_image_meta mt = meta[blockIdx.x];
+    const skg_image_meta mt = meta[img];
     const int q = threadIdx.x & 15, g = threadIdx.x >> 4;
-    const int c = blockIdx.y * 64 + 4 * q;
+    const int c = cblk * 64 + 4 * q;
     const int P = mt.n_h * (mt.n - 1);
     const float* base = src + (int64_t)mt.pair_off * ld + c;
     float4 a0 = make_float4(0.f, 0.f, 0.f, 0.f), a1 = a0;
@@ -447,6 +508,55 @@
         *o = s;
         if (out16) skg_store_twin4(out16 + (int64_t)mt.image * TR_COLS + c, s);
     }
+}
+__global__ __launch_bounds__(256) void skg_segment_sum_image_kernel(const float* __restrict__ src, int64_t ld,
+                                                                    const skg_image_meta* __restrict__ meta,
+                                                                    float* __restrict__ out, int accumulate,
+                                                                    uint16_t* __restrict__ out16) {
+    skg_segment_sum_image_body(src, ld, meta, out, accumulate, out16, (int)blockIdx.x, (int)blockIdx.y);
+}
+
+struct skg_segment_sum_modes_pack { skg_segment_sum_args a[SKG_MULTI_MAX]; };
+__global__ __launch_bounds__(256) void skg_segment_sum_modes_kernel(const skg_segment_sum_modes_pack pk,
+                                                                    const skg_image_meta* __restrict__ meta, int n_active,
+                                                                    const int32_t* __restrict__ hum_img,
+                                                                    const int32_t* __restrict__ node_img, int n_dst_h,
+                                                                    int n_dst) {
+    const skg_segment_sum_args& a = pk.a[blockIdx.y];
+    const int x = blockIdx.x;
+    if (a.mode == 2) {
+        if (x >= 16 * n_active) return;
+        skg_segment_sum_image_body(a.src, a.ld, meta, a.outH, a.accumulate, a.outH16, x >> 4, x & 15);
+        return;
+    }
+    if (x >= n_dst) return;
+    skg_segment_sum_body(a.src, a.ld, meta, hum_img, node_img, n_dst_h, a.mode, a.outH, a.outN, a.accumulate, x, a.outH16, a.outN16);
+}
+
+extern "C" int skg_segment_sum_modes_f32(const skg_segment_sum_entry* calls, int n, const skg_image_meta* meta, int n_active,
+                                         const int32_t* hum_img, const int32_t* node_img, int sum_h, int sum_n, void* stream) {
+    if (!calls || n < 1 || n > SKG_MULTI_MAX || n_active < 0 || sum_h < 0 || sum_n < 0) return SKG_E_ARG;
+    skg_segment_sum_modes_pack pk;
+    int m = 0, blocks = 0;
+    for (int i = 0; i < n; ++i) {
+        const skg_segment_sum_entry& e = calls[i];
+        if (e.mode < 0 || e.mode > 2) return SKG_E_ARG;
+        const int nb = e.mode == 2 ? 16 * n_active : sum_h + sum_n;
+        if (nb == 0) continue;
+        if (!e.src || !meta || (e.mode != 2 && (!hum_img || !node_img)) || (!e.outH && !e.outN) || (e.mode == 2 && !e.outH))
+            return SKG_E_ARG;
+        if ((e.ld & 3) || !skg_aligned16(e.src) || !skg_aligned16(e.outH) || !skg_aligned16(e.outN)) return SKG_E_ALIGN;
+        skg_segment_sum_args& a = pk.a[m++];
+        a.src = e.src; a.ld = e.ld; a.mode = e.mode; a.outH = e.outH; a.outN = e.mode == 2 ? nullptr : e.outN;
+        a.accumulate = e.accumulate;
+        a.outH16 = a.outH ? skg_twin(a.outH) : nullptr;
+        a.outN16 = a.outN ? skg_twin(a.outN) : nullptr;
+        blocks = nb > blocks ? nb : blocks;
+    }
+    if (m == 0) return 0;
+    hipLaunchKernelGGL(skg_segment_sum_modes_kernel, dim3(blocks, m), dim3(256), 0, (hipStream_t)stream, pk, meta, n_active,
+                       hum_img, node_img, sum_h, sum_h + sum_n);
+    return skg_launch_status();
 }
 
 extern "C" int skg_segment_sum_f32(const float* src, int64_t ld, const skg_image_meta* meta, int n_active,
diff --git a/skghoi_amd/csrc/skg_train_plan.hip b/skghoi_amd/csrc/skg_train_plan.hip
--- a/skghoi_amd/csrc/skg_train_plan.hip
+++ b/skghoi_amd/csrc/skg_train_plan.hip
@@ -122,14 +122,17 @@
     return sk < 1 ? 1 : sk;
 }
 
-static void launch(Ctx& c, skg_gemmx_desc* ops, int n) {
+struct SliceRef { const float* ws; int S; };
+static void launch(Ctx& c, skg_gemmx_desc* ops, int n, SliceRef* slices = nullptr) {
+    if (slices) for (int i = 0; i < n; ++i) slices[i] = SliceRef{nullptr, 0};
     if (c.rc) return;
     const bool bf16 = c.P->bf16 != 0;
     const int bk = bf16 ? 32 : 16;
     skg_gemmx_desc live[16];
+    int src[16];
     int m = 0;
     for (int i = 0; i < n; ++i)
-        if (ops[i].M > 0 && ops[i].N > 0) live[m++] = ops[i];
+        if (ops[i].M > 0 && ops[i].N > 0) { src[m] = i; live[m++] = ops[i]; }
     for (int i0 = 0; i0 < m; i0 += SKG_GEMMX_GROUP_MAX) {
         int cnt = m - i0 < SKG_GEMMX_GROUP_MAX ? m - i0 : SKG_GEMMX_GROUP_MAX;
         int64_t used = 0, used_ctr = 0;
@@ -138,7 +141,7 @@
             int sk = pick_split(c.P, d, bk);
             d.split_k = sk > 1 ? sk : 0;
             d.split_ctr = nullptr;
-            if (sk > 1 && c.P->counters) {
+            if (sk > 1 && c.P->counters && !slices) {
                 const int64_t tiles = (int64_t)((d.M + 127) / 128) * ((d.N + 127) / 128);
                 if (used_ctr + tiles <= c.P->n_counters) { d.split_ctr = c.P->counters + used_ctr; used_ctr += tiles; }
             }
@@ -152,6 +155,7 @@
                 int64_t need = (int64_t)sk * ((int64_t)d.M * d.N + d.M);
                 need = (need + 7) & ~(int64_t)7;
                 d.split_ws = c.scratch ? c.scratch + used : nullptr;
+                if (slices) slices[src[i0 + i]] = SliceRef{d.split_ws, sk};
                 used += need;
             }
         }
@@ -167,7 +171,8 @@
             if (tm->n < tm->cap) { slot = tm->n++; tm->flops[slot] = fl; }
         }
         if (slot >= 0) (void)hipEventRecord(tm->ev[2 * slot], c.stream);
-        int rc = bf16 ? skg_gemmx_bf16(live + i0, cnt, c.stream) : skg_gemmx_f32(live + i0, cnt, c.stream);
+        int rc = slices ? skg_gemmx_slices(live + i0, cnt, bf16 ? 1 : 0, c.stream)
+                        : (bf16 ? skg_gemmx_bf16(live + i0, cnt, c.stream) : skg_gemmx_f32(live + i0, cnt, c.stream));
         if (slot >= 0) (void)hipEventRecord(tm->ev[2 * slot + 1], c.stream);
         if (rc) { c.rc = rc; return; }
     }
@@ -395,6 +400,35 @@
     return 0;
 }
 
+static void gated(Ctx& c, skg_gemmx_desc& d, const Ws& w) {
+    if (c.rc) return;
+    const skg_train_plan* P = c.P;
+    c.flops += 2.0 * d.M * (double)d.N * d.K;
+    if (c.dry) return;
+    d.A16 = twin_of(c, d.A, &d.a16_ld); d.B16 = twin_of(c, d.B, &d.b16_ld);
+    int64_t ld16 = 0;
+    d.C16 = twin_of(c, d.C, &ld16);
+    auto t16 = [&](float* p) { int64_t ld = 0; return twin_of(c, p, &ld); };
+    const float* b1att = P->params + P->seg_off[SKG_SEG_B1_0];
+    skg_gemmx_gate g;
+    memset(&g, 0, sizeof(g));
+    g.n_blocks = 4; g.block_cols = 1024;
+    g.b[0] = skg_gemmx_gate_block{w.A1h, P->grid_h, 1024, w.A1o, P->grid_o, 1024, b1att, w.T, t16(w.T), 1024, nullptr};
+    g.b[1] = skg_gemmx_gate_block{w.C1o, P->grid_o, 1024, nullptr, nullptr, 1024, nullptr, w.Tos, t16(w.Tos), 1024, nullptr};
+    g.b[2] = skg_gemmx_gate_block{w.C1h, P->grid_h, 1024, nullptr, nullptr, 1024, nullptr, w.Tso, t16(w.Tso), 1024, nullptr};
+    g.b[3] = skg_gemmx_gate_block{w.G1, P->grid_img, 1024, nullptr, nullptr, 1024, nullptr, w.Tg, t16(w.Tg), 1024, P->grid_pair};
+    skg_train_timer* tm = P->timer;
+    int slot = -1;
+    if (tm) {
+        std::lock_guard<std::mutex> lk(tm->m);
+        if (tm->n < tm->cap) { slot = tm->n++; tm->flops[slot] = 2.0 * d.M * (double)d.N * d.K; }
+    }
+    if (slot >= 0) (void)hipEventRecord(tm->ev[2 * slot], c.stream);
+    int rc = skg_gemmx_gated(&d, &g, 1, c.stream);
+    if (slot >= 0) (void)hipEventRecord(tm->ev[2 * slot + 1], c.stream);
+    if (rc) c.rc = rc;
+}
+
 static void forward(Ctx& c, const Ws& w, int part) {
     const skg_train_plan* P = c.P;
     Seg W{P, const_cast<float*>(P->params)};
@@ -471,17 +505,9 @@
         launch(c, l4, 4);
     }
     if (P->bf16) {
+        if (two) CK((int)hipStreamWaitEvent(c.stream, c.br->join, 0));
         skg_gemmx_desc l[1] = {FWD(Sp, cm(W2, 4096, 1024), F, b2, false)};
-        launch(c, l, 1);
-        if (two) CK((int)hipStreamWaitEvent(c.stream, c.br->join, 0));
-        {
-            skg_rows_mul_args m[4] = {
-                {w.A1h, P->grid_h, 1024, w.A1o, P->grid_o, 1024, b1[ATT], w.F, nullptr, 4096, Mg, 1024, w.T, 1024},
-                {w.C1o, P->grid_o, 1024, nullptr, nullptr, 1024, nullptr, w.F + 1024, nullptr, 4096, Mg, 1024, w.Tos, 1024},
-                {w.C1h, P->grid_h, 1024, nullptr, nullptr, 1024, nullptr, w.F + 2048, nullptr, 4096, Mg, 1024, w.Tso, 1024},
-                {w.G1, P->pair_img, 1024, nullptr, nullptr, 1024, nullptr, w.F + 3072, P->pair_grid, 4096, Mp, 1024, w.Tg, 1024}};
-            CK(skg_rows_mul_relu_multi(m, Mp > 0 ? 4 : 3, c.stream));
-        }
+        gated(c, l[0], w);
     } else {
         skg_gemm_desc ds[4];
         for (int i = 0; i < 4; ++i) {
@@ -507,20 +533,21 @@
         skg_gemmx_desc l[1] = {FWD(T, W3[ATT], Wt, b3 + 1024 * ATT, true, -1, -1, -1, true)};
         launch(c, l, 1);
     }
-    CK(skg_rowdot_f32(w.Wt, 1024, W.at(SKG_SEG_ADJ_W), Mg, 1024, w.adj_raw, c.stream));
-    CK(skg_graph_aggregate_train_f32(w.adj_raw, 1, Mg, 0.0f, P->meta, A, P->hum_img, P->node_img, Mh, Mn, w.Tos, w.Tso,
-                                     1024, 1024, w.U, w.V, 1024, w.adj, w.alpha, w.beta, c.stream));
+    CK(skg_graph_aggregate_rowdot_train_f32(w.Wt, 1024, W.at(SKG_SEG_ADJ_W), w.adj_raw, P->meta, A, P->hum_img, P->node_img,
+                                            Mh, Mn, w.Tos, w.Tso, 1024, 1024, w.U, w.V, 1024, w.adj, w.alpha, w.beta,
+                                            c.stream));
     Mat U(w.U, Mh, 1024), V(w.V, Mn, 1024), M1(w.M1, Mh, 1024), M2(w.M2, Mn, 1024);
     {
         skg_gemmx_desc l[2] = {FWD(U, W3[OS], M1, b3 + 1024 * OS, true, -1, -1, -1, true),
                                FWD(V, W3[SO], M2, b3 + 1024 * SO, true, -1, -1, -1, true)};
-        launch(c, l, 2);
-    }
-    {
-        skg_add_layernorm_args ln[2] = {
-            {w.GH, 1024, w.M1, 1024, W.at(SKG_SEG_NH_W), W.at(SKG_SEG_NH_B), Mh, w.Hp, w.h_node, w.st_h},
-            {w.GO, 1024, w.M2, 1024, W.at(SKG_SEG_NO_W), W.at(SKG_SEG_NO_B), Mn, w.Op, w.node, w.st_o}};
-        CK(skg_add_layernorm_multi(ln, 2, 1e-5f, c.stream));
+        SliceRef sl[2];
+        launch(c, l, 2, sl);
+        skg_add_layernorm_slices_args ln[2] = {
+            {w.GH, 1024, w.M1, 1024, sl[0].ws, (int64_t)Mh * 1024, sl[0].S, 1, l[0].bias, W.at(SKG_SEG_NH_W), W.at(SKG_SEG_NH_B), Mh, 0,
+             w.Hp, w.h_node, w.st_h},
+            {w.GO, 1024, w.M2, 1024, sl[1].ws, (int64_t)Mn * 1024, sl[1].S, 1, l[1].bias, W.at(SKG_SEG_NO_W), W.at(SKG_SEG_NO_B), Mn, 0,
+             w.Op, w.node, w.st_o}};
+        CK(skg_add_layernorm_slices_f32(ln, 2, 1e-5f, c.stream));
     }
     Mat h_node(w.h_node, Mh, 1024), node(w.node, Mn, 1024), B1h(w.B1h, Mh, 1024), B1o(w.B1o, Mn, 1024);
     {
@@ -630,8 +657,10 @@
                  w.dF + 3072, 4096, 0}};
             CK(skg_mul_bwd_multi(m, 2, c.stream));
         }
-        CK(skg_segment_sum_f32(w.dTp, 1024, P->meta, A, P->hum_img, P->node_img, Mh, Mn, 1, w.dB1h, w.dB1o, 0, c.stream));
-        CK(skg_segment_sum_f32(w.dTg, 1024, P->meta, A, nullptr, nullptr, 0, 0, 2, w.dG1, nullptr, 0, c.stream));
+        {
+            skg_segment_sum_entry g[2] = {{w.dTp, 1024, 1, 0, w.dB1h, w.dB1o}, {w.dTg, 1024, 2, 0, w.dG1, nullptr}};
+            CK(skg_segment_sum_modes_f32(g, 2, P->meta, A, P->hum_img, P->node_img, Mh, Mn, c.stream));
+        }
         skg_gemmx_desc l2[4] = {IG(dB1h, Wa1, dh_node, nullptr, false, -1, 1024), IG(dB1o, Wa1.from_col(1024), dnode, nullptr, false, -1, 1024),
                                 WG(dB1h, h_node, dWa1, nullptr, false, -1, -1, 1024),
                                 WG(dB1o, node, dWa1.from_col(1024), nullptr, false, -1, -1, 1024)};
```
